# tum-vision/lsd_slam

Hardware: AMD Instinct MI355X
Metric: tracked frames/sec (full track+map loop) at 640x480, frames resident in HBM (8-bit upload excluded: value_pcie_inclusive has it) (higher is better)
Workload: dtype f32

## Files before the change

include/lsd_slam_hip.hpp:

```cpp
#ifndef LSD_SLAM_HIP_HPP
#define LSD_SLAM_HIP_HPP

#include <array>
#include <chrono>
#include <cmath>
#include <cstdint>
#include <cstring>
#include <deque>
#include <exception>
#include <functional>
#include <map>
#include <memory>
#include <mutex>
#include <stdexcept>
#include <string>
#include <tuple>
#include <utility>
#include <vector>

#include "lsdhip.h"
#include "lsd_slam_hip_pose.hpp"

namespace lsd_slam_hip {

// ... 279 lines not shown
    check(lsdhip_tracker_create(ctx_->handle(), &h_), "lsdhip_tracker_create");
  }
  SE3Tracker(const SE3Tracker&) = delete;
  SE3Tracker& operator=(const SE3Tracker&) = delete;
  ~SE3Tracker() { lsdhip_tracker_destroy(h_); }

  SE3 trackFrame(TrackingReference* reference, Frame* frame, const SE3& frameToReference_initialEstimate) {
    pushSettings();
    double init[7];
    frameToReference_initialEstimate.to7(init);
    lsdhip_track_result r;
    hookError_ = nullptr;
    if (!reference || !reference->keyframe || !frame) throw Error(LSDHIP_E_STATE, "SE3Tracker::trackFrame: the tracking reference holds no keyframe");
    check(lsdhip_tracker_track(h_, reference->keyframe->handle(), frame->handle(), init, &r), "lsdhip_tracker_track");
    publish(r);
    if (hookError_) std::rethrow_exception(hookError_);
    return SE3::from7(r.frameToReference);
  }
  std::vector<SE3> trackFrameBatch(const std::vector<TrackingReference*>& references, const std::vector<Frame*>& frames,
                                   const std::vector<SE3>& inits, std::vector<lsdhip_track_result>& results) {
    pushSettings();
    const int n = (int)frames.size();
    std::vector<lsdhip_frame*> kfs((size_t)n), frs((size_t)n);
    std::vector<double> init((size_t)n * 7);
    for (int j = 0; j < n; j++) {
      if (!references[j] || !references[j]->keyframe || !frames[j]) throw Error(LSDHIP_E_STATE, "SE3Tracker::trackFrameBatch: a tracking reference holds no keyframe");
      kfs[j] = references[j]->keyframe->handle();
      frs[j] = frames[j]->handle();
      inits[j].to7(&init[(size_t)j * 7]);
    }
    results.assign((size_t)n, lsdhip_track_result());
    hookError_ = nullptr;
    const int rc = lsdhip_tracker_track_batch(h_, n, kfs.data(), frs.data(), init.data(), results.data());
    if (rc != LSDHIP_OK && rc != LSDHIP_DIVERGED) check(rc, "lsdhip_tracker_track_batch");
    if (hookError_) std::rethrow_exception(hookError_);
    std::vector<SE3> out((size_t)n);
    for (int j = 0; j < n; j++) out[j] = SE3::from7(results[j].frameToReference);
    return out;
  }
  SE3 trackFrameOnPermaref(Frame* reference, Frame* frame, SE3 referenceToFrame) {
    pushSettings();
    double init[7];
    referenceToFrame.to7(init);
    lsdhip_track_result r;
    check(lsdhip_tracker_track_permaref(h_, reference->permaRef_posData.data(), reference->permaRef_colorAndVarData.data(),
                                        reference->permaRefNumPts, frame->handle(), init, &r), "lsdhip_tracker_track_permaref");
    publish(r);
    return SE3::from7(r.frameToReference);
  }
  void setEnqueueHook(std::function<void()> fn) {
    hook_ = std::move(fn);
    check(lsdhip_tracker_set_enqueue_hook(h_, hook_ ? &SE3Tracker::hookTrampoline : nullptr, this), "lsdhip_tracker_set_enqueue_hook");
  }
  float checkPermaRefOverlap(Frame* reference, SE3 referenceToFrame) {
    double init[7];
    referenceToFrame.to7(init);
    float usage = 0;
    check(lsdhip_tracker_check_overlap(h_, reference->permaRef_posData.data(), reference->permaRefNumPts, init, &usage), "lsdhip_tracker_check_overlap");
    pointUsage = usage;
    return usage;
  }

  float pointUsage = 0, lastGoodCount = 0, lastMeanRes = 0, lastBadCount = 0, lastResidual = 0;
  float affineEstimation_a = 1, affineEstimation_b = 0;
  bool diverged = false, trackingWasGood = false;
  int numEvaluations = 0, numWarpUpdates = 0;
  int levelEvaluations[LSDHIP_PYRAMID_LEVELS] = {0, 0, 0, 0, 0};
  int numLaunches = 0;
  void setSpeculation(int trials, int finestLevelWorkgroups = 0) { check(lsdhip_tracker_set_speculation(h_, trials, finestLevelWorkgroups), "lsdhip_tracker_set_speculation"); }
  void setBatchCoarseMinJobs(int minJobs) { check(lsdhip_tracker_set_batch_coarse_min_jobs(h_, minJobs), "lsdhip_tracker_set_batch_coarse_min_jobs"); }
  lsdhip_tracker* handle() const { return h_; }
  const std::shared_ptr<Context>& context() const { return ctx_; }

 private:
  void pushSettings() {
    lsdhip_tracker_settings st;
    st.lambdaSuccessFac = settings.lambdaSuccessFac; st.lambdaFailFac = settings.lambdaFailFac;
    for (int l = 0; l < LSDHIP_PYRAMID_LEVELS; l++) {
      st.lambdaInitial[l] = settings.lambdaInitial[l]; st.stepSizeMin[l] = settings.stepSizeMin[l];
      st.convergenceEps[l] = settings.convergenceEps[l]; st.maxItsPerLvl[l] = settings.maxItsPerLvl[l];
    }
    st.lambdaInitialTestTrack = settings.lambdaInitialTestTrack; st.stepSizeMinTestTrack = settings.stepSizeMinTestTrack;
    st.convergenceEpsTestTrack = settings.convergenceEpsTestTrack; st.maxItsTestTrack = settings.maxItsTestTrack;
    st.huber_d = settings.huber_d; st.var_weight = settings.var_weight;
    check(lsdhip_tracker_set_settings(h_, &st), "lsdhip_tracker_set_settings");
  }
  void publish(const lsdhip_track_result& r) {
    pointUsage = r.pointUsage; lastGoodCount = r.lastGoodCount; lastMeanRes = r.lastMeanRes; lastBadCount = r.lastBadCount;
    lastResidual = r.lastResidual; affineEstimation_a = r.affineEstimation_a; affineEstimation_b = r.affineEstimation_b;
    diverged = r.diverged != 0; trackingWasGood = r.trackingWasGood != 0;
    numEvaluations = r.numEvaluations; numWarpUpdates = r.numWarpUpdates;
    int st[8];
    if (lsdhip_tracker_exec_stats(h_, st) == 0) for (int l = 0; l < LSDHIP_PYRAMID_LEVELS; l++) levelEvaluations[l] = st[3 + l];
    int ls[2];
    if (lsdhip_tracker_launch_stats(h_, ls) == 0) numLaunches = ls[0];
  }
  static void hookTrampoline(void* self) {
    SE3Tracker* t = static_cast<SE3Tracker*>(self);
    try { if (t->hook_) t->hook_(); } catch (...) { t->hookError_ = std::current_exception(); }
  }
  std::function<void()> hook_;
  std::exception_ptr hookError_;
  std::shared_ptr<Context> ctx_;
  lsdhip_tracker* h_ = nullptr;
};

class KeyFrameBank {
 public:
  struct Info { int frameId, numPoints; float meanIdepth; Sim3 camToWorld; };
  KeyFrameBank(std::shared_ptr<Context> ctx, int maxKeyframes) : ctx_(std::move(ctx)) {
    check(lsdhip_kfbank_create(ctx_->handle(), maxKeyframes, &h_), "lsdhip_kfbank_create");
  }
  KeyFrameBank(const KeyFrameBank&) = delete;
  KeyFrameBank& operator=(const KeyFrameBank&) = delete;
  ~KeyFrameBank() { lsdhip_kfbank_destroy(h_); }
  int put(Frame& kf) {
    int slot = -1;
    check(lsdhip_kfbank_put(h_, kf.handle(), &slot), "lsdhip_kfbank_put");
    kf.idxInKeyframes = slot;
    return slot;
  }
  int put(Frame& kf, const Sim3& camToWorld, float meanIdepth = -1.0f) {
    const int slot = put(kf);
    setMeta(slot, camToWorld, meanIdepth);
    return slot;
  }
  void setMeta(int slot, const Sim3& camToWorld, float meanIdepth = -1.0f) {
    const double p[8] = {camToWorld.q[0], camToWorld.q[1], camToWorld.q[2], camToWorld.q[3], camToWorld.t[0], camToWorld.t[1], camToWorld.t[2], camToWorld.s};
    check(lsdhip_kfbank_set_meta(h_, slot, p, meanIdepth), "lsdhip_kfbank_set_meta");
  }
  int size() const { return check(lsdhip_kfbank_size(h_), "lsdhip_kfbank_size"); }
  Info info(int slot) const {
    Info o;
    double p[8];
    check(lsdhip_kfbank_info(h_, slot, &o.frameId, &o.numPoints, &o.meanIdepth, p), "lsdhip_kfbank_info");
    for (int i = 0; i < 4; i++) o.camToWorld.q[i] = p[i];
    for (int i = 0; i < 3; i++) o.camToWorld.t[i] = p[4 + i];
    o.camToWorld.s = p[7];
    return o;
  }
  int download(int slot, std::vector<float>* posData, std::vector<float>* colorAndVarData) const {
    const int n = info(slot).numPoints;
    std::vector<float> pos((size_t)n * 3 + 1), cv((size_t)n * 2 + 1);
    check(lsdhip_kfbank_download(h_, slot, pos.data(), cv.data()), "lsdhip_kfbank_download");
    if (posData) posData->assign(pos.begin(), pos.begin() + (size_t)n * 3);
    if (colorAndVarData) colorAndVarData->assign(cv.begin(), cv.begin() + (size_t)n * 2);
    return n;
  }
  lsdhip_kfbank* handle() const { return h_; }
  const std::shared_ptr<Context>& context() const { return ctx_; }

 private:
  std::shared_ptr<Context> ctx_;
  lsdhip_kfbank* h_ = nullptr;
// ... 164 lines not shown
    return v;
  }
  int debugPlotDepthMap(int debugDisplay = 0) {
    if (!isValid()) return 1;
    debugImageDepth.resize((size_t)ctx_->width() * ctx_->height() * 3);
    check(lsdhip_depth_debug_plot(h_, debugDisplay, debugImageDepth.data()), "lsdhip_depth_debug_plot");
    return 1;
  }
  void debugPlotDepthMapDevice(unsigned char* dev, int debugDisplay) { check(lsdhip_depth_debug_plot_dev(h_, debugDisplay, dev), "lsdhip_depth_debug_plot_dev"); }
  static void debugPlotDepthMapBatch(const std::vector<DepthMap*>& maps, const std::vector<unsigned char*>& devs, int debugDisplay) {
    if (maps.empty()) return;
    if (devs.size() != maps.size()) throw Error(LSDHIP_E_ARG, "DepthMap::debugPlotDepthMapBatch: one device buffer per map");
    std::vector<lsdhip_depthmap*> ms;
    for (DepthMap* m : maps) ms.push_back(m->h_);
    check(lsdhip_depth_debug_plot_batch((int)ms.size(), ms.data(), debugDisplay, devs.data()), "lsdhip_depth_debug_plot_batch");
  }
  std::vector<unsigned char> debugImageDepth;
  void copyPlanesToDevice(float* idepth_dev, float* idepthVar_dev) { check(lsdhip_depth_copy_planes_dev(h_, idepth_dev, idepthVar_dev), "lsdhip_depth_copy_planes_dev"); }

  float msUpdate = 0, msCreate = 0, msFinalize = 0, msObserve = 0, msRegularize = 0, msPropagate = 0, msFillHoles = 0, msSetDepth = 0;
  lsdhip_depthmap* handle() const { return h_; }

 private:
  void timings() {
    float t[8];
    if (lsdhip_depth_timings(h_, t) == 0) { msUpdate = t[0]; msCreate = t[1]; msFinalize = t[2]; msObserve = t[3]; msRegularize = t[4]; msPropagate = t[5]; msFillHoles = t[6]; msSetDepth = t[7]; }
  }
  std::shared_ptr<Context> ctx_;
  lsdhip_depthmap* h_ = nullptr;
};

class SlamLoop {
 public:
  SlamLoop(int w, int h, const Mat3f& K, const unsigned char* firstImage, bool imagesOnDevice, const float* gtDepth0, int kfEvery)
      : tracker(w, h, K), map(w, h, K), w_(w), h_(h), K_(K), onDevice_(imagesOnDevice), kfEvery_(kfEvery) {
    const int its[LSDHIP_PYRAMID_LEVELS] = {5, 20, 50, 100, 0};
    std::memcpy(tracker.settings.maxItsPerLvl, its, sizeof(its));
    keyframe = makeFrame(0, firstImage);
    if (gtDepth0) {
      keyframe->setDepthFromGroundTruth(gtDepth0);
      map.initializeFromGTDepth(keyframe.get());
    } else {
      map.initializeRandomly(keyframe.get());
    }
    trackKF_ = keyframe;
    reference.importFrame(keyframe.get());
    keyframe->clearDepthHasBeenUpdatedFlag();
    tracker.setEnqueueHook([this]() {
      flushDeferredMapping();
      if (!pendingNext_) return;
      prefetched_ = makeFrame(frameId_ + 1, pendingNext_, true);
      prefetchedSrc_ = pendingNext_;
    });
  }
  SlamLoop(const SlamLoop&) = delete;
  SlamLoop& operator=(const SlamLoop&) = delete;
  void setPipelined(bool on) {
    if (frameId_ != 0) throw Error(LSDHIP_E_STATE, "SlamLoop::setPipelined: switch before the first frame");
    Context::get(w_, h_, K_)->setPipeline(on);
    pipelined_ = on;
  }
  bool pipelined() const { return pipelined_; }
  void flushDeferredMapping() {
    if (!deferredMap_) return;
    std::shared_ptr<Frame> frame = std::move(deferredMap_);
    deferredMap_.reset();
    runUpdate(frame);
  }
  static float keyframeScore(float distanceSquared, float usage) {
    return distanceSquared * 4.0f * 4.0f + (1 - usage) * (1 - usage) * 3.0f * 3.0f;
  }
  std::function<void(Frame&, DepthMap&)> onKeyframeFinished;
  std::function<void(Frame&)> onKeyframeFinishedAsync;
  std::function<void(DepthMap&)> onMappingIteration;
  SE3 step(const unsigned char* image) { return step(image, [](double) {}); }
  template <typename F>
  SE3 step(const unsigned char* image, F&& onTrackEnd, const unsigned char* nextImage = nullptr) {
    if (trackingLost) throw Error(LSDHIP_E_STATE, "SlamLoop: tracking lost (no relocaliser here): create a new loop");
    lsdhip_host_mark(0);
    frameId_++;
    std::shared_ptr<Frame> frame;
    if (prefetched_ && prefetchedSrc_ == image) frame = std::move(prefetched_);
    else frame = makeFrame(frameId_, image);
    prefetched_.reset();
    pendingNext_ = nextImage;
    if (!pipelined_ && keyframe->depthHasBeenUpdatedFlag()) {
      reference.importFrame(keyframe.get());
      keyframe->clearDepthHasBeenUpdatedFlag();
    }
    lsdhip_host_mark(1);
    const std::shared_ptr<Frame> trackedOn = trackKF_;
    SE3 est = tracker.trackFrame(&reference, frame.get(), lastFrameToKF_);
    lsdhip_host_mark(8);
    pendingNext_ = nullptr;
    evaluations += tracker.numEvaluations;
    launches += tracker.numLaunches;
    for (int l = 0; l < LSDHIP_PYRAMID_LEVELS; l++) levelEvaluations[l] += tracker.levelEvaluations[l];
    if (tracker.trackingWasGood) numTrackedGood++;
    numTracked++;
    lastTrackEnd = std::chrono::duration<double>(std::chrono::steady_clock::now().time_since_epoch()).count();
    onTrackEnd(lastTrackEnd);
    if (tracker.diverged || (numKeyframesFinished_ > 5  && !tracker.trackingWasGood)) {
      trackingLost = true;
      reference.invalidate();
      if (map.isValid()) {
        if (mappedOnKF_ >= 5 ) {
          map.finalizeKeyFrame();
          numKeyframesFinished_++;
          if (onKeyframeFinished) onKeyframeFinished(*keyframe, map);
          if (onKeyframeFinishedAsync) onKeyframeFinishedAsync(*keyframe);
        }
        map.invalidate();
      }
      throw Error(LSDHIP_DIVERGED, std::string("SlamLoop: tracking lost at frame ") + std::to_string(frameId_) +
                                       (tracker.diverged ? " (diverged)" : " (trackingWasGood false)"));
    }
    if (pipelined_) {
      if (pendingKF_) {
        double p[7];
        if (pendingIsReactivated_) {
          double f2k[8], frameToWorld[8];
          est.to7(f2k); f2k[7] = 1;
          lsd_slam::pose::sim3_mul(worldPose(*trackKF_).data(), f2k, frameToWorld);
          lsd_slam::pose::relative_se3(worldPose(*pendingKF_).data(), frameToWorld, p);
          pendingIsReactivated_ = false;
        } else {
          check(lsdhip_frame_relative_pose(pendingKF_->handle(), frame->handle(), p), "lsdhip_frame_relative_pose");
        }
        lastFrameToKF_ = SE3::from7(p);
        trackKF_ = pendingKF_;
        pendingKF_.reset();
        reference.importFrame(trackKF_.get());
        trackKF_->clearDepthHasBeenUpdatedFlag();
      } else {
        lastFrameToKF_ = est;
        if (trackKF_->depthHasBeenUpdatedFlag()) {
          reference.importFrame(trackKF_.get());
          trackKF_->clearDepthHasBeenUpdatedFlag();
        }
      }
    }
    ++sinceKF_;
    newKeyframe = false;
    flushDeferredMapping();
    if (trackedOn != keyframe) {
      frame->clear_refPixelWasGood();
      numDropped++;
      return est;
    }
    bool createNewKeyFrame = kfEvery_ > 0 && sinceKF_ >= kfEvery_;
    if (kfEvery_ == 0 && mappedOnKF_ > 5 ) {
      const float mi = keyframe->meanIdepth();
      const float d0 = (float)est.t[0] * mi, d1 = (float)est.t[1] * mi, d2 = (float)est.t[2] * mi;
      float minVal = 0.2f * 0.7f;
      if (reactivateKeyframes) {
        const int size = bank_->size();
// ... 122 lines not shown
      map.changeKeyframe(frame.get());
    }
    bankFinishedKeyframe(finished);
    if (onKeyframeFinishedAsync) onKeyframeFinishedAsync(*finished);
    const lsdhip_reposition_result& r = search_->last;
    keyframeChanges.push_back(KeyframeChange{frame->id(), finished->id(), found ? found->id() : frame->id(), found != nullptr,
                                             r.numPotential, r.numChecked, r.numTracked});
    double nextEstimate[7] = {1, 0, 0, 0, 0, 0, 0};
    if (found) {
      numReactivations++;
      keyframe = found;
      keyframe->clearDepthHasBeenUpdatedFlag();
      lsd_slam::pose::relative_se3(worldPose(*keyframe).data(), cw, nextEstimate);
    } else {
      double raw[8];
      check(lsdhip_frame_get_pose(frame->handle(), raw), "lsdhip_frame_get_pose");
      std::array<double, 8> w;
      lsd_slam::pose::sim3_mul(worldPose(*finished).data(), raw, w.data());
      worldPoses_[frame->id()] = w;
      keyframe = frame;
      if (keepKeyframes) keyframeLog.push_back(frame);
    }
    liveQueue_.clear();
    if (pipelined_) {
      pendingKF_ = keyframe;
      pendingIsReactivated_ = found != nullptr;
    } else {
      trackKF_ = keyframe;
      reference.importFrame(keyframe.get());
      keyframe->clearDepthHasBeenUpdatedFlag();
      lastFrameToKF_ = SE3::from7(nextEstimate);
    }
    sinceKF_ = 0;
    newKeyframe = true;
    if (onMappingIteration) onMappingIteration(map);
  }
  std::unique_ptr<KeyFrameBank> bank_;
  std::unique_ptr<TrackableKeyFrameSearch> search_;
  std::vector<std::shared_ptr<Frame>> bankedBySlot_;
  std::map<int, std::array<double, 8>> worldPoses_;
  bool pendingIsReactivated_ = false;
  void runUpdate(const std::shared_ptr<Frame>& frame) {
    liveQueue_.push_back(frame);
    while ((int)liveQueue_.size() > (liveQueueLength > 1 ? liveQueueLength : 1)) liveQueue_.pop_front();
    std::deque<std::shared_ptr<Frame>> q(liveQueue_.begin(), liveQueue_.end());
    lsdhip_host_mark(9);
    map.updateKeyframe(q);
    lsdhip_host_mark(13);
    mappedOnKF_++;
    frame->clear_refPixelWasGood();
    numUpdates++;
    lsdhip_host_mark(14);
    if (onMappingIteration) onMappingIteration(map);
  }
  std::shared_ptr<Frame> deferredMap_;
  std::shared_ptr<Frame> makeFrame(int id, const unsigned char* img, bool mayDefer = false) {
    if (onDevice_) return std::make_shared<Frame>(id, w_, h_, K_, 0.0, Frame::DeviceImage{img});
    if (mayDefer && pipelined_) return std::make_shared<Frame>(id, w_, h_, K_, 0.0, Frame::HostImageAsync{img});
    return std::make_shared<Frame>(id, w_, h_, K_, 0.0, img);
  }
  int w_, h_;
  Mat3f K_;
  bool onDevice_;
  bool pipelined_ = false;
  int kfEvery_, sinceKF_ = 0, frameId_ = 0;
  int mappedOnKF_ = 0;
  int numKeyframesFinished_ = 0;
  SE3 lastFrameToKF_;
  std::shared_ptr<Frame> trackKF_;
  std::shared_ptr<Frame> pendingKF_;
  std::shared_ptr<Frame> prefetched_;
  const unsigned char* prefetchedSrc_ = nullptr;
  const unsigned char* pendingNext_ = nullptr;
  std::deque<std::shared_ptr<Frame>> liveQueue_;
};

class SlamLoopBatch {
 public:
  struct Sequence {
    Sequence(int w, int h, const Mat3f& K) : map(w, h, K) {}
    DepthMap map;
    TrackingReference reference;
    std::shared_ptr<Frame> keyframe;
    std::shared_ptr<Frame> trackKF;
    std::shared_ptr<Frame> pendingKF;
    SE3 lastFrameToKF;
    int sinceKF = 0, mappedOnKF = 0, numKeyframesFinished = 0;
    long numTracked = 0, numTrackedGood = 0, numUpdates = 0, evaluations = 0, numDropped = 0;
    bool trackingLost = false, newKeyframe = false;
    lsdhip_track_result last = lsdhip_track_result();
    std::vector<std::shared_ptr<Frame>> keyframeLog;
    std::shared_ptr<Frame> replacedFirst;
  };
  SlamLoopBatch(int w, int h, const Mat3f& K, int S, const unsigned char* const* firstImages, bool imagesOnDevice,
                const float* const* gtDepth0, int kfEvery)
      : tracker(w, h, K), w_(w), h_(h), K_(K), onDevice_(imagesOnDevice), kfEvery_(kfEvery) {
    if (S <= 0 || kfEvery <= 0) throw Error(LSDHIP_E_ARG, "SlamLoopBatch: S > 0 sequences, a fixed keyframe interval > 0");
    const int its[LSDHIP_PYRAMID_LEVELS] = {5, 20, 50, 100, 0};
    std::memcpy(tracker.settings.maxItsPerLvl, its, sizeof(its));
    tracker.setBatchCoarseMinJobs(coarseMinJobs(false));
    std::vector<int> ids((size_t)S);
    for (int s = 0; s < S; s++) ids[s] = idOf(s, 0);
    std::vector<std::shared_ptr<Frame>> first = Frame::createBatch(w, h, K, ids, firstImages, imagesOnDevice);
    for (int s = 0; s < S; s++) {
      seqs_.emplace_back(new Sequence(w, h, K));
      Sequence& q = *seqs_.back();
// ... 284 lines not shown
```

include/lsdhip.h:

```cpp
#ifndef LSDHIP_H
#define LSDHIP_H

#include <stddef.h>
#include <stdint.h>

#ifdef __cplusplus
extern "C" {
#endif

#define LSDHIP_PYRAMID_LEVELS 5

#define LSDHIP_OK 0
#define LSDHIP_DIVERGED 1
#define LSDHIP_E_ARG (-1)
#define LSDHIP_E_HIP (-2)
#define LSDHIP_E_STATE (-3)
#define LSDHIP_E_CAPACITY (-4)
#define LSDHIP_CLOUD_TABLE_FULL 2
#define LSDHIP_CLOUD_GUARD_POINTS 64

typedef struct lsdhip_ctx lsdhip_ctx;
typedef struct lsdhip_frame lsdhip_frame;
typedef struct lsdhip_tracker lsdhip_tracker;
typedef struct lsdhip_depthmap lsdhip_depthmap;
// ... 60 lines not shown
int lsdhip_frame_clear_wasgood(lsdhip_frame* f);
int lsdhip_frame_set_pose(lsdhip_frame* f, const double thisToParent_sim3[8], lsdhip_frame* trackingParent,
                          float initialTrackedResidual);
int lsdhip_frame_get_pose(lsdhip_frame* f, double thisToParent_sim3[8]);
int lsdhip_frame_relative_pose(lsdhip_frame* reference, lsdhip_frame* frame, double frameToReference[7]);
int lsdhip_frame_publish_depth(lsdhip_frame* f);
int lsdhip_frame_stats(lsdhip_frame* f, float out[8]);
int lsdhip_frame_set_counters(lsdhip_frame* f, int numFramesTrackedOnThis, int numMappedOnThis,
                              int numMappedOnThisTotal, int depthHasBeenUpdatedFlag);
int lsdhip_frame_depth_updated(lsdhip_frame* f);
int lsdhip_frame_clear_depth_updated(lsdhip_frame* f);
int lsdhip_ref_pointcloud(lsdhip_frame* kf, int level, float* pos3_host, float* colorAndVar2_host,
                          float* grad2_host, int* idx_host);

typedef struct lsdhip_track_result {
  double frameToReference[7];
  float pointUsage, lastGoodCount, lastBadCount, lastMeanRes, lastResidual;
  float affineEstimation_a, affineEstimation_b;
  int diverged, trackingWasGood;
  int numEvaluations, numWarpUpdates;
} lsdhip_track_result;

typedef struct lsdhip_residual_record {
  int warped_size;
  float goodCount, badCount, pointUsage, meanRes, retval;
  float affine_a_lastIt, affine_b_lastIt;
  float weightedError;
  float A[36], b[6], lsError;
  double num_constraints;
} lsdhip_residual_record;

int lsdhip_tracker_create(lsdhip_ctx* ctx, lsdhip_tracker** out);
void lsdhip_tracker_destroy(lsdhip_tracker* t);
int lsdhip_tracker_set_max_its(lsdhip_tracker* t, const int maxItsPerLvl[LSDHIP_PYRAMID_LEVELS]);
typedef struct lsdhip_tracker_settings {
  float lambdaSuccessFac, lambdaFailFac;
  float lambdaInitial[LSDHIP_PYRAMID_LEVELS], stepSizeMin[LSDHIP_PYRAMID_LEVELS], convergenceEps[LSDHIP_PYRAMID_LEVELS];
  int maxItsPerLvl[LSDHIP_PYRAMID_LEVELS];
  float lambdaInitialTestTrack, stepSizeMinTestTrack, convergenceEpsTestTrack, maxItsTestTrack;
  float huber_d, var_weight;
} lsdhip_tracker_settings;
int lsdhip_tracker_get_settings(const lsdhip_tracker* t, lsdhip_tracker_settings* out);
int lsdhip_tracker_set_settings(lsdhip_tracker* t, const lsdhip_tracker_settings* in);
int lsdhip_tracker_exec_stats(const lsdhip_tracker* t, int out[8]);
int lsdhip_tracker_set_speculation(lsdhip_tracker* t, int trials, int finestLevelWorkgroups);
int lsdhip_tracker_set_batch_coarse_min_jobs(lsdhip_tracker* t, int minJobs);
int lsdhip_tracker_launch_stats(const lsdhip_tracker* t, int out[2]);
int lsdhip_tracker_step_stats(const lsdhip_tracker* t, int out[4]);
int lsdhip_tracker_summary_stats(const lsdhip_tracker* t, long long out[6]);
int lsdhip_tracker_eval_throughput(lsdhip_tracker* t, int n, lsdhip_frame** keyframes, lsdhip_frame** frames, const float* refToFrame,
                                   int level, int repeats, double* ms_per_launch, double* bytes_per_launch);
typedef void (*lsdhip_enqueue_hook)(void* user);
int lsdhip_tracker_set_enqueue_hook(lsdhip_tracker* t, lsdhip_enqueue_hook fn, void* user);
int lsdhip_tracker_track(lsdhip_tracker* t, lsdhip_frame* keyframe, lsdhip_frame* frame,
                         const double frameToReference_initialEstimate[7], lsdhip_track_result* out);
int lsdhip_tracker_track_batch(lsdhip_tracker* t, int n, lsdhip_frame** keyframes, lsdhip_frame** frames,
                               const double* frameToReference_initialEstimates, lsdhip_track_result* results);
int lsdhip_tracker_evaluate(lsdhip_tracker* t, lsdhip_frame* keyframe, lsdhip_frame* frame,
                            const float referenceToFrame[7], int level, float affine_a, float affine_b,
                            lsdhip_residual_record* out);
int lsdhip_tracker_evaluate_batch(lsdhip_tracker* t, int n, lsdhip_frame** keyframes, lsdhip_frame** frames,
                                  const float* referenceToFrame, const float* affine, int level, lsdhip_residual_record* out,
                                  int* form);
int lsdhip_tracker_track_permaref(lsdhip_tracker* t, const float* pos3_host, const float* colorAndVar2_host, int n,
                                  lsdhip_frame* frame, const double referenceToFrame[7], lsdhip_track_result* out);
int lsdhip_tracker_track_permaref_batch(lsdhip_tracker* t, int n, const float* pos3_host, const float* colorAndVar2_host,
                                        const int* counts, lsdhip_frame** frames, const double* referenceToFrame,
                                        lsdhip_track_result* results);
int lsdhip_tracker_check_overlap(lsdhip_tracker* t, const float* pos3_host, int n, const double referenceToFrame[7],
                                 float* usage_out);

typedef struct lsdhip_kfbank lsdhip_kfbank;
int lsdhip_kfbank_create(lsdhip_ctx* ctx, int max_keyframes, lsdhip_kfbank** out);
void lsdhip_kfbank_destroy(lsdhip_kfbank* bank);
int lsdhip_kfbank_put(lsdhip_kfbank* bank, lsdhip_frame* keyframe, int* slot_out);
int lsdhip_kfbank_set_meta(lsdhip_kfbank* bank, int slot, const double camToWorld_sim3[8], float meanIdepth);
int lsdhip_kfbank_size(lsdhip_kfbank* bank);
int lsdhip_kfbank_info(lsdhip_kfbank* bank, int slot, int* frameId, int* numPoints, float* meanIdepth, double camToWorld_sim3[8]);
int lsdhip_kfbank_download(lsdhip_kfbank* bank, int slot, float* pos3_host, float* colorAndVar2_host);
int lsdhip_tracker_check_overlap_bank(lsdhip_tracker* t, lsdhip_kfbank* bank, int n, const int* slots, const double* refToFrame,
                                      float* usage_out);
int lsdhip_tracker_track_permaref_bank(lsdhip_tracker* t, lsdhip_kfbank* bank, int n, const int* slots, lsdhip_frame** frames,
                                       const double* refToFrame, lsdhip_track_result* results);
typedef struct lsdhip_reposition_result {
  int slot, frameId;
  int numPotential, numChecked, numTracked;
  int overlapLaunches, trackingBatches;
  float bestScore, bestDist, bestUsage, bestPoseDiscrepancy;
  double refToFrame[7], refToFrame_tracked[7];
} lsdhip_reposition_result;
#define LSDHIP_REPO_FAR 0
#define LSDHIP_REPO_ANGLE 1
#define LSDHIP_REPO_PARENT 2
#define LSDHIP_REPO_INIT_PHASE 3
#define LSDHIP_REPO_EMPTY 4
#define LSDHIP_REPO_SCORE 5
#define LSDHIP_REPO_REJECTED 6
#define LSDHIP_REPO_TAKEN 7
typedef struct lsdhip_reposition_record {
  int slot, frameId, stage;
  float dist2, angle;
  float usage, score;
  float usageTracked;
  float newScore, goodVal, poseDiscrepancy;
  int trackingWasGood, diverged;
  double refToFrame[7], refToFrame_tracked[7];
} lsdhip_reposition_record;
int lsdhip_tracker_find_reposition_candidate(lsdhip_tracker* t, lsdhip_kfbank* bank, lsdhip_frame* frame, const double frameCamToWorld_sim3[8],
                                             int trackingParentId, float maxScore, lsdhip_reposition_result* result);
int lsdhip_tracker_reposition_records(lsdhip_tracker* t, int max, lsdhip_reposition_record* records, int* n);
int lsdhip_tracker_set_relocalization_th(lsdhip_tracker* t, float relocalizationTH);

typedef struct lsdhip_sim3tracker lsdhip_sim3tracker;
typedef struct lsdhip_sim3_result {
  double frameToReference[8];
  float lastResidual, lastDepthResidual, lastPhotometricResidual;
  float pointUsage;
  float affineEstimation_a, affineEstimation_b;
  int diverged;
  int numEvaluations;
  float lastSim3Hessian[49];
} lsdhip_sim3_result;
typedef struct lsdhip_sim3_eval_record {
  int warped_size;
  float pointUsage, affine_a_lastIt, affine_b_lastIt;
  float sumResD, sumResP;
  int numTermsD, numTermsP;
  float meanD, meanP, mean;
  float A[49], b[7];
  double num_constraints;
} lsdhip_sim3_eval_record;
int lsdhip_sim3tracker_create(lsdhip_ctx* ctx, lsdhip_sim3tracker** out);
void lsdhip_sim3tracker_destroy(lsdhip_sim3tracker* t);
int lsdhip_sim3tracker_set_max_its(lsdhip_sim3tracker* t, const int maxItsPerLvl[5]);
int lsdhip_sim3tracker_track(lsdhip_sim3tracker* t, lsdhip_frame* keyframe, lsdhip_frame* frame, const double init_frameToReference[8],
                             int startLevel, int finalLevel, lsdhip_sim3_result* out);
int lsdhip_sim3tracker_track_batch(lsdhip_sim3tracker* t, int n, lsdhip_frame** keyframes, lsdhip_frame** frames,
                                   const double* init_frameToReference, int startLevel, int finalLevel, lsdhip_sim3_result* results);
int lsdhip_host_se3f_step(const float increment[6], const float referenceToFrame[7], float out[7]);
int lsdhip_host_ldlt6(const float A[36], const float b[6], float x[6]);
int lsdhip_host_sim3_step(const double increment[7], const double referenceToFrame[8], double out[8]);
int lsdhip_host_ldlt7(const float A[49], const float b[7], float x[7]);
int lsdhip_devtest_se3f_lm_step(lsdhip_ctx* ctx, int n, const float* A, const float* b, const float* damp, const float* T, float* inc, float* Tn);
int lsdhip_devtest_sim3_lm_step(lsdhip_ctx* ctx, int n, const float* A, const float* b, const double* nconstraints, const float* lambda,
                                const double* T, float* inc, double* Tn);
int lsdhip_sim3tracker_evaluate(lsdhip_sim3tracker* t, lsdhip_frame* keyframe, lsdhip_frame* frame, const double referenceToFrame[8],
                                int level, float aff_a, float aff_b, lsdhip_sim3_eval_record* out);

int lsdhip_depth_create(lsdhip_ctx* ctx, lsdhip_depthmap** out);
void lsdhip_depth_destroy(lsdhip_depthmap* dm);
int lsdhip_depth_is_valid(lsdhip_depthmap* dm);
int lsdhip_depth_invalidate(lsdhip_depthmap* dm);
int lsdhip_depth_reset(lsdhip_depthmap* dm);
int lsdhip_depth_init_gt(lsdhip_depthmap* dm, lsdhip_frame* kf);
int lsdhip_depth_init_random(lsdhip_depthmap* dm, lsdhip_frame* kf);
int lsdhip_depth_set_from_existing(lsdhip_depthmap* dm, lsdhip_frame* kf);
int lsdhip_depth_update(lsdhip_depthmap* dm, lsdhip_frame** refs, int n);
int lsdhip_depth_update_batch(int n, lsdhip_depthmap** maps, lsdhip_frame** refs);
int lsdhip_depth_create_keyframe(lsdhip_depthmap* dm, lsdhip_frame* new_keyframe, float* rescale_out);
int lsdhip_depth_finalize(lsdhip_depthmap* dm);
int lsdhip_depth_change_keyframe_batch(int n, lsdhip_depthmap** maps, lsdhip_frame** new_keyframes, float* rescale_out);
int lsdhip_depth_reactivate_keyframe_batch(int n, lsdhip_depthmap** maps, lsdhip_frame** old_keyframes);
int lsdhip_ctx_batch_form(lsdhip_ctx* ctx, int which, int out[8], int* queueCounts, int maxCounts);
int lsdhip_depth_download(lsdhip_depthmap* dm, lsdhip_hypothesis* out_host);
int lsdhip_depth_upload(lsdhip_depthmap* dm, lsdhip_frame* kf, const lsdhip_hypothesis* in_host, int reactivated);
int lsdhip_depth_debug_plot(lsdhip_depthmap* dm, int debugDisplay, uint8_t* out_host);
int lsdhip_depth_debug_plot_dev(lsdhip_depthmap* dm, int debugDisplay, uint8_t* out_dev);
int lsdhip_depth_debug_plot_batch(int n, lsdhip_depthmap** maps, int debugDisplay, uint8_t* const* out_dev);
int lsdhip_depth_stage(lsdhip_depthmap* dm, int stage, lsdhip_frame** refs, int n);
int lsdhip_depth_stage_rows(lsdhip_depthmap* dm, int stage, int tile_row0, int n_tile_rows, int last);
int lsdhip_depth_stage_rows_batch(lsdhip_ctx* c, int n, lsdhip_depthmap** maps, const int* tile_row0, const int* n_tile_rows);
int lsdhip_depth_copy_planes_dev(lsdhip_depthmap* dm, float* idepth_dev, float* idepthVar_dev);
int lsdhip_ctx_copy_dev(lsdhip_ctx* ctx, void* dst_dev, const void* src_dev, size_t bytes);
int lsdhip_ctx_alloc_dev(lsdhip_ctx* ctx, size_t bytes, void** out_dev);
int lsdhip_ctx_ipc_export(lsdhip_ctx* ctx, void* dev, unsigned char handle64[64]);
int lsdhip_ctx_ipc_open(lsdhip_ctx* ctx, const unsigned char handle64[64], void** out_dev);
int lsdhip_ctx_ipc_close(lsdhip_ctx* ctx, void* dev);
int lsdhip_ctx_flag_set(lsdhip_ctx* ctx, int* flag_dev, int value);
int lsdhip_ctx_flag_wait(lsdhip_ctx* ctx, const int* flag_dev, int value, int* fail_dev);
int lsdhip_ctx_memset_dev(lsdhip_ctx* ctx, void* dev, int byte, size_t bytes);
int lsdhip_ctx_read_dev(lsdhip_ctx* ctx, void* host, const void* dev, size_t bytes);
int lsdhip_ctx_aux_begin(lsdhip_ctx* ctx);
int lsdhip_ctx_aux_end(lsdhip_ctx* ctx);
int lsdhip_ctx_aux_join(lsdhip_ctx* ctx);
void* lsdhip_ctx_aux_stream(lsdhip_ctx* ctx);
void lsdhip_host_mark(int id);
int lsdhip_ctx_free_dev(lsdhip_ctx* ctx, void* dev);
int lsdhip_depth_copy_rows_dev(lsdhip_depthmap* dm, int row0, int nrows, void* packed_dev, int to_map);
typedef struct lsdhip_row_copy {
  lsdhip_depthmap* src_map; int src_row0; void* src_packed;
  lsdhip_depthmap* dst_map; int dst_row0; void* dst_packed;
  int nrows;
} lsdhip_row_copy;
// ... 28 lines not shown
```

include/lsdhip_driver.h:

```cpp
#ifndef LSDHIP_DRIVER_H
#define LSDHIP_DRIVER_H
#include <stdint.h>
#ifdef __cplusplus
extern "C" {
#endif
typedef struct lsdloop lsdloop;
typedef struct lsdloop_stats {
  double seconds_track;
  double seconds_map;
  double seconds_keyframe;
  long long frames;
  long long updates;
  long long keyframes;
  long long evaluations;
  long long tracked_good;
  long long level_evaluations[5];
  long long track_launches;
  long long dropped;
} lsdloop_stats;
int lsdloop_create(int device, int w, int h, const float K4[4], const uint8_t* first_image, int images_on_device,
                   const float* gt_depth0_host, int kf_every, lsdloop** out);
void lsdloop_destroy(lsdloop* l);
int lsdloop_run(lsdloop* l, const uint8_t* const* images, int n, int stop_at_keyframe, double* frameToKeyframe_out);
int lsdloop_get_stats(lsdloop* l, lsdloop_stats* out);
int lsdloop_reset_stats(lsdloop* l);
int lsdloop_copy_keyframe_planes(lsdloop* l, float* idepth_dev, float* idepthVar_dev);
int lsdloop_set_keyframe_ring(lsdloop* l, float* ring_dev, int slots);
long long lsdloop_keyframes_exported(lsdloop* l);
int lsdloop_keep_keyframes(lsdloop* l, int on);
int lsdloop_keyframe_log(lsdloop* l, double* scales_out, long long* points_out, int max);
int lsdloop_set_pipeline(lsdloop* l, int on);
int lsdloop_enable_reactivation(lsdloop* l, int max_keyframes);
int lsdloop_keyframe_changes(lsdloop* l, int* out, int max);
int lsdloop_reactivation_counts(lsdloop* l, long long out2[2]);
int lsdloop_download_map(lsdloop* l, lsdhip_hypothesis* out);
int lsdloop_set_live_queue(lsdloop* l, int frames);
int lsdloop_set_speculation(lsdloop* l, int trials, int finest_level_workgroups);
int lsdloop_observe_time(lsdloop* l, double* ms_out, long long* calls_out);
int lsdloop_observe_work(lsdloop* l, double out3[3]);
int lsdloop_comm_unique_id(unsigned char out128[128]);
int lsdloop_comm_init(lsdloop* l, const unsigned char id128[128], int rank, int world);
int lsdloop_comm_destroy(lsdloop* l);
int lsdloop_gather_keyframes(lsdloop* l, int count, int root, float* recv_dev, long long stride_floats);
int lsdloop_gather_counts(lsdloop* l, int* counts_out, int cap);
int lsdloop_ipc_init(lsdloop* l, int rank, int world, int root, unsigned char handle64_out[64]);
int lsdloop_ipc_connect(lsdloop* l, const unsigned char root_handle64[64]);
int lsdloop_ipc_result(lsdloop* l, int* counts_out, float** data_out);
void* lsdloop_ctx(lsdloop* l);
typedef struct lsdloopbatch lsdloopbatch;
int lsdloopbatch_create(int device, int w, int h, const float K4[4], int S, const uint8_t* const* first_images, int images_on_device,
                        const float* const* gt_depth0_host, int kf_every, lsdloopbatch** out);
void lsdloopbatch_destroy(lsdloopbatch* l);
int lsdloopbatch_run(lsdloopbatch* l, const uint8_t* const* images, int n, double* frameToKeyframe_out);
int lsdloopbatch_get_stats(lsdloopbatch* l, long long* out6_per_sequence);
void* lsdloopbatch_ctx(lsdloopbatch* l);
int lsdloopbatch_set_keyframe_phases(lsdloopbatch* l, const int* phase);
int lsdloopbatch_set_pipeline(lsdloopbatch* l, int on);
int lsdloopbatch_set_coarse_min_jobs(lsdloopbatch* l, int min_jobs);
long long lsdloopbatch_dropped(lsdloopbatch* l, int sequence);
int lsdloopbatch_keep_keyframes(lsdloopbatch* l, int on);
int lsdloopbatch_keyframe_log(lsdloopbatch* l, int sequence, double* scales_out, long long* points_out, int max);
int lsdloopbatch_last_result(lsdloopbatch* l, int sequence, lsdhip_track_result* out);
int lsdloopbatch_download_map(lsdloopbatch* l, int sequence, lsdhip_hypothesis* out);
int lsdloopbatch_set_cloud_sinks(lsdloopbatch* l, long long capacity_points, int max_keyframes);
void* lsdloopbatch_cloud(lsdloopbatch* l, int sequence);
int lsdloopbatch_cloud_pose(lsdloopbatch* l, int sequence, int frame_id, float out7[7]);
void* lsdloopbatch_keyframe_handle(lsdloopbatch* l, int sequence, int k);
const char* lsdloop_last_error(void);
typedef struct lsdband lsdband;
int lsdband_create(int device, int w, int H, int world, int first_band, int n_local, lsdband** out);
int lsdband_plan(int H, int world, int* window_rows_out, int* layout4, int* segments4, int cap);
void lsdband_destroy(lsdband* b);
int lsdband_window_rows(const lsdband* b);
int lsdband_layout(const lsdband* b, int band, int out4[4]);
int lsdband_load(lsdband* b, int local, const void* hyp_window, const float* maxgrad_window);
int lsdband_get(lsdband* b, int local, void* hyp_window_out);
int lsdband_comm_init(lsdband* b, const void* unique_id128, int nprocs, int proc, const int* proc_of_band);
int lsdband_run(lsdband* b, int passes);
int lsdband_synchronize(lsdband* b);
long long lsdband_halo_bytes_per_pass(const lsdband* b);
int lsdband_ipc_init(lsdband* b, int nprocs, int proc, const int* proc_of_band, unsigned char handle64_out[64]);
int lsdband_ipc_connect(lsdband* b, const unsigned char* handles);
int lsdband_ipc_failed(lsdband* b);
int lsdband_tile_runs(int H, int world, int band, int* runs3, int cap);
int lsdband_set_packed_exchange(lsdband* b, int on);
int lsdband_set_overlap(lsdband* b, int on);

#ifdef __cplusplus
}
#endif
// ... 2 lines not shown
```

lsd_slam_amd/capi.py:

```python
import ctypes as C
import os

import numpy as np

_HERE = os.path.dirname(os.path.abspath(__file__))
LIB_PATH = os.environ.get("LSDHIP_LIB") or os.path.join(_HERE, "liblsdhip.so")
_lib = None

HYP_DTYPE = np.dtype(
    [("isValid", np.uint8), ("_pad", np.uint8, 3), ("blacklisted", np.int32), ("nextStereoFrameMinID", np.float32),
     ("validity_counter", np.int32), ("idepth", np.float32), ("idepth_var", np.float32),
     ("idepth_smoothed", np.float32), ("idepth_var_smoothed", np.float32)])
assert HYP_DTYPE.itemsize == 32


class BuildDefaults(C.Structure):
    _fields_ = [(k, C.c_int) for k in ("ctx_async", "ctx_pipeline", "spec_trials_small", "spec_small_pixels", "spec_trials_mid", "spec_mid_pixels",
                                         "spec_workgroups", "spec_workgroups_above_pixels", "spec_trials_max", "batch_throughput_min_jobs",
                                         "batch_strip_workgroups", "batch_coarse_min_jobs", "batch_coarse_max_pixels",
                                         "batch_coarse_max_points")]


class Params(C.Structure):
    _fields_ = [("minUseGrad", C.c_float), ("cameraPixelNoise2", C.c_float), ("depthSmoothingFactor", C.c_float),
# ... 74 lines not shown
        "lsdhip_frame_create_batch": (i, [vp, i, vp, pvp, i, pvp]),
        "lsdhip_ctx_reserve_frames": (i, [vp, i]),
        "lsdhip_frame_relative_pose": (i, [vp, vp, vp]),
        "lsdhip_frame_publish_depth": (i, [vp]),
        "lsdhip_last_error": (C.c_char_p, []),
        "lsdhip_ctx_intrinsics": (i, [vp, i, vp]),
        "lsdhip_frame_create": (i, [vp, i, vp, pvp]),
        "lsdhip_frame_create_from_device": (i, [vp, i, vp, pvp]),
        "lsdhip_frame_destroy": (None, [vp]),
        "lsdhip_frame_id": (i, [vp]),
        "lsdhip_frame_download": (i, [vp, i, i, vp]),
        "lsdhip_frame_set_depth_gt": (i, [vp, vp, f]),
        "lsdhip_frame_set_depth_planes": (i, [vp, vp, vp]),
        "lsdhip_frame_set_maxgrad": (i, [vp, vp]),
        "lsdhip_frame_get_wasgood": (i, [vp, vp]),
        "lsdhip_frame_set_wasgood": (i, [vp, vp]),
        "lsdhip_frame_clear_wasgood": (i, [vp]),
        "lsdhip_frame_set_pose": (i, [vp, vp, vp, f]),
        "lsdhip_frame_get_pose": (i, [vp, vp]),
        "lsdhip_frame_stats": (i, [vp, vp]),
        "lsdhip_frame_set_counters": (i, [vp, i, i, i, i]),
        "lsdhip_frame_depth_updated": (i, [vp]),
        "lsdhip_frame_clear_depth_updated": (i, [vp]),
        "lsdhip_ref_pointcloud": (i, [vp, i, vp, vp, vp, vp]),
        "lsdhip_tracker_create": (i, [vp, pvp]),
        "lsdhip_tracker_destroy": (None, [vp]),
        "lsdhip_tracker_set_max_its": (i, [vp, vp]),
        "lsdhip_tracker_get_settings": (i, [vp, C.POINTER(TrackerSettings)]),
        "lsdhip_tracker_set_settings": (i, [vp, C.POINTER(TrackerSettings)]),
        "lsdhip_depth_copy_rows_batch": (i, [vp, i, vp]),
        "lsdhip_ctx_alloc_dev": (i, [vp, C.c_size_t, vp]),
        "lsdhip_ctx_ipc_export": (i, [vp, vp, vp]),
        "lsdhip_ctx_ipc_open": (i, [vp, vp, vp]),
        "lsdhip_ctx_ipc_close": (i, [vp, vp]),
        "lsdhip_ctx_flag_set": (i, [vp, vp, i]),
        "lsdhip_ctx_flag_wait": (i, [vp, vp, i, vp]),
        "lsdhip_ctx_memset_dev": (i, [vp, vp, i, C.c_size_t]),
        "lsdhip_ctx_read_dev": (i, [vp, vp, vp, C.c_size_t]),
        "lsdhip_ctx_free_dev": (i, [vp, vp]),
        "lsdhip_host_mark": (None, [i]),
        "lsdhip_ctx_aux_begin": (i, [vp]),
        "lsdhip_ctx_aux_end": (i, [vp]),
        "lsdhip_ctx_aux_join": (i, [vp]),
        "lsdhip_ctx_aux_stream": (vp, [vp]),
        "lsdhip_depth_stage_rows": (i, [vp, i, i, i, i]),
        "lsdhip_depth_stage_rows_batch": (i, [vp, i, pvp, C.POINTER(C.c_int), C.POINTER(C.c_int)]),
        "lsdhip_tracker_exec_stats": (i, [vp, vp]),
        "lsdhip_tracker_set_speculation": (i, [vp, i, i]),
        "lsdhip_tracker_set_batch_coarse_min_jobs": (i, [vp, i]),
        "lsdhip_tracker_launch_stats": (i, [vp, vp]),
        "lsdhip_tracker_summary_stats": (i, [vp, vp]),
        "lsdhip_tracker_step_stats": (i, [vp, vp]),
        "lsdhip_tracker_set_enqueue_hook": (i, [vp, vp, vp]),
        "lsdhip_tracker_track": (i, [vp, vp, vp, vp, C.POINTER(TrackResult)]),
        "lsdhip_tracker_track_batch": (i, [vp, i, pvp, pvp, vp, C.POINTER(TrackResult)]),
        "lsdhip_tracker_eval_throughput": (i, [vp, i, pvp, pvp, vp, i, i, C.POINTER(C.c_double), C.POINTER(C.c_double)]),
        "lsdhip_tracker_evaluate": (i, [vp, vp, vp, vp, i, f, f, C.POINTER(ResidualRecord)]),
        "lsdhip_tracker_evaluate_batch": (i, [vp, i, pvp, pvp, vp, vp, i, C.POINTER(ResidualRecord), vp]),
        "lsdhip_tracker_track_permaref": (i, [vp, vp, vp, i, vp, vp, C.POINTER(TrackResult)]),
        "lsdhip_tracker_track_permaref_batch": (i, [vp, i, vp, vp, vp, pvp, vp, C.POINTER(TrackResult)]),
        "lsdhip_tracker_check_overlap": (i, [vp, vp, i, vp, C.POINTER(C.c_float)]),
        "lsdhip_kfbank_create": (i, [vp, i, pvp]),
        "lsdhip_kfbank_destroy": (None, [vp]),
        "lsdhip_kfbank_put": (i, [vp, vp, C.POINTER(C.c_int)]),
        "lsdhip_kfbank_set_meta": (i, [vp, i, vp, f]),
        "lsdhip_kfbank_size": (i, [vp]),
        "lsdhip_kfbank_info": (i, [vp, i, C.POINTER(C.c_int), C.POINTER(C.c_int), C.POINTER(C.c_float), vp]),
        "lsdhip_kfbank_download": (i, [vp, i, vp, vp]),
        "lsdhip_tracker_check_overlap_bank": (i, [vp, vp, i, vp, vp, vp]),
        "lsdhip_tracker_track_permaref_bank": (i, [vp, vp, i, vp, pvp, vp, C.POINTER(TrackResult)]),
        "lsdhip_tracker_find_reposition_candidate": (i, [vp, vp, vp, vp, i, f, C.POINTER(RepositionResult)]),
        "lsdhip_tracker_reposition_records": (i, [vp, i, C.POINTER(RepositionRecord), C.POINTER(C.c_int)]),
        "lsdhip_tracker_set_relocalization_th": (i, [vp, f]),
        "lsdhip_sim3tracker_create": (i, [vp, pvp]),
        "lsdhip_sim3tracker_destroy": (None, [vp]),
        "lsdhip_sim3tracker_set_max_its": (i, [vp, vp]),
        "lsdhip_sim3tracker_track": (i, [vp, vp, vp, vp, i, i, C.POINTER(Sim3Result)]),
        "lsdhip_sim3tracker_track_batch": (i, [vp, i, pvp, pvp, vp, i, i, C.POINTER(Sim3Result)]),
        "lsdhip_host_se3f_step": (i, [vp, vp, vp]),
        "lsdhip_host_ldlt6": (i, [vp, vp, vp]),
        "lsdhip_host_sim3_step": (i, [vp, vp, vp]),
        "lsdhip_host_ldlt7": (i, [vp, vp, vp]),
        "lsdhip_devtest_se3f_lm_step": (i, [vp, i, vp, vp, vp, vp, vp, vp]),
        "lsdhip_devtest_sim3_lm_step": (i, [vp, i, vp, vp, vp, vp, vp, vp, vp]),
        "lsdhip_sim3tracker_evaluate": (i, [vp, vp, vp, vp, i, f, f, C.POINTER(Sim3EvalRecord)]),
        "lsdhip_depth_create": (i, [vp, pvp]),
        "lsdhip_depth_destroy": (None, [vp]),
        "lsdhip_depth_is_valid": (i, [vp]),
        "lsdhip_depth_invalidate": (i, [vp]),
        "lsdhip_depth_reset": (i, [vp]),
        "lsdhip_depth_init_gt": (i, [vp, vp]),
        "lsdhip_depth_init_random": (i, [vp, vp]),
        "lsdhip_depth_set_from_existing": (i, [vp, vp]),
        "lsdhip_depth_update": (i, [vp, pvp, i]),
        "lsdhip_depth_observe_work": (i, [vp, vp]),
        "lsdhip_depth_update_batch": (i, [i, pvp, pvp]),
        "lsdhip_depth_create_keyframe": (i, [vp, vp, C.POINTER(C.c_float)]),
        "lsdhip_depth_change_keyframe_batch": (i, [i, pvp, pvp, C.POINTER(C.c_float)]),
        "lsdhip_depth_reactivate_keyframe_batch": (i, [i, pvp, pvp]),
        "lsdhip_ctx_batch_form": (i, [vp, i, vp, vp, i]),
        "lsdhip_depth_finalize": (i, [vp]),
        "lsdhip_depth_download": (i, [vp, vp]),
        "lsdhip_depth_upload": (i, [vp, vp, vp, i]),
        "lsdhip_depth_debug_plot": (i, [vp, i, vp]),
        "lsdhip_depth_debug_plot_dev": (i, [vp, i, vp]),
        "lsdhip_depth_debug_plot_batch": (i, [i, pvp, i, pvp]),
# ... 52 lines not shown
```

lsd_slam_amd/csrc/host_math.cpp:

```cpp
#include <cstdarg>
#include "lsdhip_internal.hpp"

static thread_local std::string g_last_error;
void lsd_set_error(const char* fmt, ...) {
  char buf[1024];
  va_list ap;
  va_start(ap, fmt);
  vsnprintf(buf, sizeof(buf), fmt, ap);
  va_end(ap);
  g_last_error = buf;
}
extern "C" const char* lsdhip_last_error(void) { return g_last_error.c_str(); }


extern "C" int lsdhip_host_se3f_step(const float increment[6], const float referenceToFrame[7], float out[7]) {
  if (!increment || !referenceToFrame || !out) return LSDHIP_E_ARG;
  lsdm::SE3fH T;
  T.q = {referenceToFrame[0], referenceToFrame[1], referenceToFrame[2], referenceToFrame[3]};
  T.t[0] = referenceToFrame[4]; T.t[1] = referenceToFrame[5]; T.t[2] = referenceToFrame[6];
  const lsdm::SE3fH r = lsdm::se3f_mul(lsdm::se3f_exp(increment), T);
  out[0] = r.q.w; out[1] = r.q.x; out[2] = r.q.y; out[3] = r.q.z; out[4] = r.t[0]; out[5] = r.t[1]; out[6] = r.t[2];
  return LSDHIP_OK;
}
extern "C" int lsdhip_host_ldlt6(const float A[36], const float b[6], float x[6]) {
  if (!A || !b || !x) return LSDHIP_E_ARG;
  lsdm::ldlt6_solve(A, b, x);
  return LSDHIP_OK;
}
```

lsd_slam_amd/csrc/lsdhip_internal.hpp:

```cpp
#pragma once
#include <hip/hip_runtime.h>
#include <atomic>
#include <chrono>
#include <cmath>
#include <cstddef>
#include <cstdint>
#include <cstdio>
#include <cstring>
#include <mutex>
#include <string>
#include <vector>
#include "../../include/lsdhip.h"

#define LSD_LEVELS LSDHIP_PYRAMID_LEVELS
#define LSD_TRACK_MIN_LEVEL 1
#define LSD_TRACK_MAX_LEVEL 5
#define LSD_QUICK_KF_CHECK_LVL 4

void lsd_set_error(const char* fmt, ...);
#define HIPCHK(expr)                                                                       \
  do {                                                                                     \
    hipError_t e_ = (expr);                                                                \
    if (e_ != hipSuccess) {                                                                \
      lsd_set_error("%s failed: %s (%s:%d)", #expr, hipGetErrorString(e_), __FILE__, __LINE__); \
// ... 45 lines not shown
  int evalBatch;
};

struct TrackJob {
  TrackLevel lv[LSD_LEVELS];
  uint8_t* wasGood;
  float cameraPixelNoise2, var_weight, huber_half;
  float lambdaSuccessFac, lambdaFailFac;
  int useAffine;
  int lastLevel;
  int topLevel;
  lsdm::SE3fH T0;
  float aff_a0, aff_b0;
  int evalOnly;
  int trackFrameSemantics;
};
struct TrackSpec {
  int specC;
  int specGrid;
  int trials[LSD_LEVELS];
  uint8_t* wasGoodSide;
  unsigned maskStride;
  int seq;
  int copyMask;
  unsigned long long dbgCum;
  unsigned long long* dbgCounters;
  int last;
#ifdef LSD_PHASE_TRACE
  int traceWg;
#endif
#ifdef LSD_DEVTOOLS
  int* dbgLog;
#endif
};

struct TrackState {
  lsdm::SE3fH T;
  lsdm::SE3fH Tn;
  float R[9], t[3];
  float aff_a, aff_b, aff_a_lastIt, aff_b_lastIt;
  float lastErr, LM_lambda, last_residual;
  int level, iteration, incTry, phase;
  int pending;
  float A[36], b[6];
  float inc[6];
  float bytes;
  int done, diverged;
  int numEvaluations, numWarpUpdates;
  float pointUsage, goodCount, badCount, meanRes;
  int levelEvals[LSD_LEVELS];
  int ncand;
  int lastCand;
  int numLaunches;
};

struct TrackSummary {
  int done;
  int diverged, level, numEvaluations, numWarpUpdates, pad_[3];
  float q[4], t[3];
  float lastResidual, pointUsage, goodCount, badCount, meanRes, aff_a, aff_b, aff_a_lastIt, aff_b_lastIt;
  float sums[RS_NUM];
  double bytes;
  int levelEvals[LSD_LEVELS];
  int numLaunches;
  int lastCand;
  int seq;
  int exhausted;
  unsigned check;
};
#define LSD_SUMMARY_CHECK_WORDS (offsetof(TrackSummary, seq) / 4)
__host__ __device__ static inline unsigned lsd_summary_term(unsigned i, unsigned bits) { return bits * (2u * i + 1u); }

struct DeferredSlot { double sum, count, flag, pad; };
#define LSD_NUM_SLOTS 256
#define LSD_DEFAULT_ASYNC 0
#define LSD_DEFAULT_PIPELINE 0
#ifndef LSD_OBS_SPLIT_MIN_MAPS
#define LSD_OBS_SPLIT_MIN_MAPS 4
#endif
#define LSD_OBS_WALK_WAVES 4096
struct lsdhip_frame;

#define LSD_CTX_LOCK(c) std::lock_guard<std::recursive_mutex> lsd_ctx_lock_((c)->mtx)
struct lsdhip_ctx {
  std::recursive_mutex mtx;
  int device = 0;
  bool async = LSD_DEFAULT_ASYNC != 0;
  DeferredSlot* h_slots = nullptr;
  lsdhip_frame* slot_stats_owner[LSD_NUM_SLOTS] = {};
  lsdhip_frame* slot_rescale_owner[LSD_NUM_SLOTS] = {};
  int slot_next = 0;
  long long enqEpoch = 0, doneEpoch = 0;
  long long slot_epoch[LSD_NUM_SLOTS] = {};
  int w = 0, h = 0;
  bool refBlocksWanted = false;
  int wl[LSD_LEVELS], hl[LSD_LEVELS];
  LevelIntr intr[LSD_LEVELS];
  float K0[9], K0inv[9];
  lsdhip_params params;
  hipStream_t stream = nullptr;
#define LSD_EVR 64
  bool pipeline = LSD_DEFAULT_PIPELINE != 0;
  hipStream_t mstream = nullptr;
  hipEvent_t mEv[LSD_EVR] = {};
  long long mSeq = 0;
  long long mDoneSeq = 0;
// ... 100 lines not shown
};

struct lsdhip_tracker {
  lsdhip_ctx* ctx = nullptr;
  float lambdaSuccessFac = 0.5f, lambdaFailFac = 2.0f;
  float lambdaInitial[LSD_LEVELS], stepSizeMin[LSD_LEVELS], convergenceEps[LSD_LEVELS];
  int maxItsPerLvl[LSD_LEVELS];
  float lambdaInitialTestTrack = 0, stepSizeMinTestTrack = 1e-3, convergenceEpsTestTrack = 0.98, maxItsTestTrack = 5;
  float huber_d = 3, var_weight = 1.0;
  float pointUsage = 0, lastGoodCount = 0, lastMeanRes = 0, lastBadCount = 0, lastResidual = 0;
  float affineEstimation_a = 1, affineEstimation_b = 0, affineEstimation_a_lastIt = 1, affineEstimation_b_lastIt = 0;
  bool diverged = false, trackingWasGood = false;
  int numEvaluations = 0, numWarpUpdates = 0;
  void (*enqueueHook)(void*) = nullptr;
  void* enqueueHookUser = nullptr;
  bool spinWait = true;
  bool hostLM = false;
  float* d_partials = nullptr;
  int max_blocks = 0;
  TrackState* d_state = nullptr;
  int levelEvaluations[LSD_LEVELS] = {};
  int block = 256;
  int grid_cap = 304;
  bool evalBatch = true;
  LaunchHistory recent;
  int specC = 6;
  int soloMinJobs = -1;
  bool specAuto = true;
  int specCaps[LSD_LEVELS] = {0, 0, 0, 0, 0};
  int specLevel[LSD_LEVELS] = {0, 0, 0, 0, 0};
  int specCap = LSD_SPEC_CAP_WORKGROUPS;
  uint8_t* d_maskSide = nullptr;
  int maskSet = 0;
  long long maskMergeSeq[2] = {0, 0};
  size_t maskStride = 0;
  int numLaunches = 0;
  long long sumPolled = 0, sumLate = 0, sumLateMaxNs = 0, sumLateWords = 0;
  int sumLateFirstWord = -1, sumLateLastWord = -1;
  unsigned long long dbgCum = 0;
  std::vector<unsigned> dumpL0;
  unsigned long long* d_dbg = nullptr;
#ifdef LSD_DEVTOOLS
  int* d_log = nullptr;
  std::vector<int> lastLog;
#endif
  const lsdhip_frame* jobKf = nullptr;
  unsigned jobKfVersion = 0;
  int jobTag = 0, launchOrdinal = 0;
  int budgetExtra = 2;
  int budgetFixed = 0;
  long long dbgJobs = 0, dbgEnqueued = 0, dbgMisses = 0, dbgWaitNs = 0, dbgLaunchNs = 0;
  TrackSummary* h_summary = nullptr;
  TrackSummary* d_summary = nullptr;
  unsigned long long* d_trace = nullptr;
  int batch_capacity = 0;
  TrackJob* d_bjobs = nullptr;
  TrackJob* h_bjobs = nullptr;
  TrackState* d_bstate = nullptr;
  float* d_bscratch = nullptr;
  LaunchHistory batchRecent;
  int batchTag = 1;
  TrackSummary* h_bsummary = nullptr;
  float* d_pts = nullptr;
  int pts_capacity = 0;
  float relocalizationTH = 0.7f;
  float* h_overlapSums = nullptr;
  int overlapSumsCapacity = 0;
  std::vector<lsdhip_reposition_record> repoRecords;
};

struct lsdhip_kfbank {
  lsdhip_ctx* ctx = nullptr;
  int maxSlots = 0, capacity = 0;
  size_t slotFloats = 0;
  float* d_base = nullptr;
  int* d_count = nullptr;
  struct Slot { int frameId; int numPoints; float meanIdepth; double camToWorld[8]; };
  std::vector<Slot> slots;
  float* pos(int slot) const { return d_base + (size_t)slot * slotFloats; }
  float* colvar(int slot) const { return pos(slot) + (size_t)capacity * 3; }
};

#ifdef __HIP_DEVICE_COMPILE__
#define LSD_G __attribute__((address_space(1)))
#else
#define LSD_G
#endif
template <typename T> __host__ __device__ inline LSD_G T* lsd_g(T* p) { return (LSD_G T*)p; }
struct HypPlanes {
  LSD_G uint8_t* valid;
  LSD_G int32_t* blacklisted;
  LSD_G float* nextID;
  LSD_G int32_t* validity;
  LSD_G float* idepth;
  LSD_G float* var;
  LSD_G float* idepth_s;
  LSD_G float* var_s;
};

struct StereoRef {
  LSD_G const float* image;
  LSD_G const uint8_t* wasGood;
  int parentIsKF;
  int id;
  float initialTrackedResidual;
  float K_otherToThis_R[9];
// ... 152 lines not shown
```

lsd_slam_amd/csrc/pose_math.hpp:

```cpp
#pragma once
#include <hip/hip_runtime.h>
#include <cmath>

#define LSDM_HD __host__ __device__ inline

namespace lsdm {
struct Quatd { double w, x, y, z; };
struct Quatf { float w, x, y, z; };
struct SE3dH { Quatd q; double t[3]; };
struct SE3fH { Quatf q; float t[3]; };
struct Sim3dH { Quatd q; double t[3]; double s; };

template <typename Q> LSDM_HD Q q_conj(const Q& a) { Q r = {a.w, -a.x, -a.y, -a.z}; return r; }
template <typename Q> LSDM_HD Q q_mul(const Q& a, const Q& b) {
  Q r;
  r.w = a.w * b.w - a.x * b.x - a.y * b.y - a.z * b.z;
  r.x = a.w * b.x + a.x * b.w + a.y * b.z - a.z * b.y;
  r.y = a.w * b.y + a.y * b.w + a.z * b.x - a.x * b.z;
  r.z = a.w * b.z + a.z * b.w + a.x * b.y - a.y * b.x;
  return r;
}
LSDM_HD void q_normalize(Quatf& q) {
  float n = sqrtf(q.x * q.x + q.y * q.y + q.z * q.z + q.w * q.w);
  q.w /= n; q.x /= n; q.y /= n; q.z /= n;
// ... 1 lines not shown
LSDM_HD void q_normalize(Quatd& q) {
  double n = sqrt(q.x * q.x + q.y * q.y + q.z * q.z + q.w * q.w);
  q.w /= n; q.x /= n; q.y /= n; q.z /= n;
}
template <typename Q, typename T> LSDM_HD void q_rotate(const Q& q, const T v[3], T out[3]) {
  T ux = q.y * v[2] - q.z * v[1], uy = q.z * v[0] - q.x * v[2], uz = q.x * v[1] - q.y * v[0];
  ux += ux; uy += uy; uz += uz;
  T cx = q.y * uz - q.z * uy, cy = q.z * ux - q.x * uz, cz = q.x * uy - q.y * ux;
  out[0] = v[0] + q.w * ux + cx;
  out[1] = v[1] + q.w * uy + cy;
  out[2] = v[2] + q.w * uz + cz;
}
template <typename Q, typename T> LSDM_HD void q_to_rot(const Q& q, T R[9]) {
  T tx = T(2) * q.x, ty = T(2) * q.y, tz = T(2) * q.z;
  T twx = tx * q.w, twy = ty * q.w, twz = tz * q.w;
  T txx = tx * q.x, txy = ty * q.x, txz = tz * q.x;
  T tyy = ty * q.y, tyz = tz * q.y, tzz = tz * q.z;
  R[0] = T(1) - (tyy + tzz); R[1] = txy - twz;          R[2] = txz + twy;
  R[3] = txy + twz;          R[4] = T(1) - (txx + tzz); R[5] = tyz - twx;
  R[6] = txz - twy;          R[7] = tyz + twx;          R[8] = T(1) - (txx + tyy);
}
LSDM_HD void quatf_to_rot(const Quatf& q, float R[9]) { q_to_rot<Quatf, float>(q, R); }
LSDM_HD void quatd_to_rot(const Quatd& q, double R[9]) { q_to_rot<Quatd, double>(q, R); }

LSDM_HD SE3dH se3d_from7(const double p[7]) { SE3dH T; T.q = {p[0], p[1], p[2], p[3]}; T.t[0] = p[4]; T.t[1] = p[5]; T.t[2] = p[6]; return T; }
LSDM_HD void se3d_to7(const SE3dH& T, double p[7]) { p[0] = T.q.w; p[1] = T.q.x; p[2] = T.q.y; p[3] = T.q.z; p[4] = T.t[0]; p[5] = T.t[1]; p[6] = T.t[2]; }
LSDM_HD SE3dH se3d_inverse(const SE3dH& T) {
  SE3dH r;
  r.q = q_conj(T.q);
  double nt[3] = {T.t[0] * -1.0, T.t[1] * -1.0, T.t[2] * -1.0};
  q_rotate<Quatd, double>(r.q, nt, r.t);
  return r;
}
LSDM_HD SE3fH se3f_from_d(const SE3dH& T) {
  SE3fH r;
  r.q = {(float)T.q.w, (float)T.q.x, (float)T.q.y, (float)T.q.z};
  q_normalize(r.q);
  for (int i = 0; i < 3; i++) r.t[i] = (float)T.t[i];
  return r;
}
LSDM_HD SE3dH se3d_from_f(const SE3fH& T) {
  SE3dH r;
  r.q = {(double)T.q.w, (double)T.q.x, (double)T.q.y, (double)T.q.z};
  q_normalize(r.q);
  for (int i = 0; i < 3; i++) r.t[i] = (double)T.t[i];
  return r;
}
LSDM_HD SE3fH se3f_inverse(const SE3fH& T) {
  SE3fH r;
  r.q = q_conj(T.q);
  float nt[3] = {T.t[0] * -1.0f, T.t[1] * -1.0f, T.t[2] * -1.0f};
  q_rotate<Quatf, float>(r.q, nt, r.t);
  return r;
}
LSDM_HD SE3fH se3f_mul(const SE3fH& a, const SE3fH& b) {
  SE3fH r = a;
  float rt[3];
  q_rotate<Quatf, float>(a.q, b.t, rt);
  for (int i = 0; i < 3; i++) r.t[i] = a.t[i] + rt[i];
  r.q = q_mul(a.q, b.q);
  q_normalize(r.q);
  return r;
}
LSDM_HD SE3fH se3f_exp(const float a[6]) {
  const float eps = static_cast<float>(1e-5);
  float ox = a[3], oy = a[4], oz = a[5];
  float theta_sq = ox * ox + (oy * oy + oz * oz);
  float theta = sqrtf(theta_sq);
  float half_theta = 0.5f * theta;
  float imag, real;
  if (theta < eps) {
    float theta_po4 = theta_sq * theta_sq;
    imag = 0.5f - static_cast<float>(1.0 / 48.0) * theta_sq + static_cast<float>(1.0 / 3840.0) * theta_po4;
    real = 1.0f - 0.5f * theta_sq + static_cast<float>(1.0 / 384.0) * theta_po4;
  } else {
    float s = sinf(half_theta);
    imag = s / theta;
    real = cosf(half_theta);
  }
  SE3fH r;
  r.q = {real, imag * ox, imag * oy, imag * oz};
  q_normalize(r.q);
  float Om[9] = {0, -oz, oy, oz, 0, -ox, -oy, ox, 0};
  float Om2[9];
  for (int i = 0; i < 3; i++)
    for (int j = 0; j < 3; j++) {
      float acc = Om[i * 3 + 0] * Om[0 * 3 + j];
      acc += Om[i * 3 + 1] * Om[1 * 3 + j];
      acc += Om[i * 3 + 2] * Om[2 * 3 + j];
      Om2[i * 3 + j] = acc;
    }
  float V[9];
  if (theta < eps) {
    q_to_rot<Quatf, float>(r.q, V);
  } else {
    float tsq = theta * theta;
    float ca = (1.0f - cosf(theta)) / tsq;
    float cb = (theta - sinf(theta)) / (tsq * theta);
    for (int i = 0; i < 9; i++) V[i] = (((i % 4) == 0 ? 1.0f : 0.0f) + ca * Om[i]) + cb * Om2[i];
  }
  for (int i = 0; i < 3; i++) {
    float acc = V[i * 3 + 0] * a[0];
    acc += V[i * 3 + 1] * a[1];
    acc += V[i * 3 + 2] * a[2];
    r.t[i] = acc;
  }
// ... 61 lines not shown
```

lsd_slam_amd/csrc/tracker.hip:

```cpp
#include <atomic>
#include <chrono>
#include "track_device.hpp"
#include "reposition_plan.hpp"

#ifdef LSD_PHASE_TRACE
#define PHASE_MARK(k) do { if (trOn_ && threadIdx.x == 0) tr_[k] = clock64(); } while (0)
#define LSD_TRACE_WORDS 32
#define TRACE_PARAMS , const bool trOn_, unsigned long long* const tr_
#define TRACE_ARGS , trOn_, tr_
#define TRACE_PUT(rec, who, k, v) do { if (trOn_ && threadIdx.x == (who)) (rec)[k] = (unsigned long long)(v); } while (0)
#define TRACE_LM_REC (trOn_ ? tr_ : nullptr)
__device__ __forceinline__ unsigned long long* trace_open(unsigned long long* trace, const bool mine, unsigned long long** s_trp) {
  if (!mine) return trace;
  const unsigned long long n = trace[0];
  trace[0] = n + 1;
  unsigned long long* tr_ = trace + 1 + (n % 4096) * LSD_TRACE_WORDS;
  for (int k = 0; k < LSD_TRACE_WORDS; k++) tr_[k] = 0;
  tr_[8] = wall_clock64();
  tr_[24] = (unsigned long long)gridDim.x; tr_[25] = (unsigned long long)gridDim.y;
  *s_trp = tr_;
  return tr_;
}
#else
#define PHASE_MARK(k) do { } while (0)
#define TRACE_PARAMS
#define TRACE_ARGS
#define TRACE_PUT(rec, who, k, v) do { } while (0)
#define TRACE_LM_REC nullptr
#endif

#ifdef LSD_DEVTOOLS
#define LAUNCH_LOG(exitCode, pendingIn, ncandIn, pcUsed) do { \
    if (!BATCH && MODE == TS_FUSED && blockIdx.x == 0 && threadIdx.x == 0 && spec.dbgLog && spec.seq != 0) { \
      int* lg_ = spec.dbgLog + ((spec.seq & 0xFFF) * 16); \
      lg_[0] = spec.seq; lg_[1] = (exitCode); lg_[2] = parity | (first << 1) | (spec.last << 2); lg_[3] = lvlIn_; lg_[4] = (pendingIn); lg_[5] = (ncandIn); \
      lg_[6] = (pcUsed); lg_[7] = S.level; lg_[8] = S.numEvaluations; lg_[9] = S.numLaunches; lg_[10] = S.done; lg_[11] = S.phase; lg_[12] = S.incTry; \
      lg_[13] = S.ncand; lg_[14] = S.pending; lg_[15] = numLaunchesIn_; } } while (0)
#else
#define LAUNCH_LOG(exitCode, pendingIn, ncandIn, pcUsed) do { } while (0)
#endif

enum { TS_FUSED = 0, TS_LM = 1, TS_EVAL = 2 };
__device__ __forceinline__ void track_state_begin(TrackState& S, const TrackJob& job, const int tid) {
  if (tid == 0) {
    S.T = job.T0;
    set_eval_pose(S, job.T0);
    S.aff_a = job.aff_a0; S.aff_b = job.aff_b0; S.aff_a_lastIt = job.aff_a0; S.aff_b_lastIt = job.aff_b0;
    S.lastErr = 0; S.LM_lambda = 0; S.last_residual = 0;
    S.level = job.topLevel; S.iteration = 0; S.incTry = 0; S.phase = 0; S.pending = 0;
    S.done = 0; S.diverged = 0; S.numEvaluations = 0; S.numWarpUpdates = 0;
    S.pointUsage = 0; S.goodCount = 0; S.badCount = 0; S.meanRes = 0;
    S.bytes = 0;
    for (int l = 0; l < LSD_LEVELS; l++) S.levelEvals[l] = 0;
    S.ncand = 1; S.lastCand = 0; S.numLaunches = 0;
  }
  if (tid < 36) S.A[tid] = 0;
  if (tid < 6) { S.b[tid] = 0; S.inc[tid] = 0; }
}

struct StepAddr {
  const float *sums_in, *topval_in;
  float *sums_out, *topval_out;
  const int4* topkey_in; int4* topkey_out;
  const TrialRecord* recs_in;
  TrialRecord* recs_out;
  int max_rows, cmax;
};
template <bool BATCH, int MODE>
__device__ __forceinline__ StepAddr step_addr(const TrackScratch& sc, const int parity) {
  const size_t rows = (size_t)sc.max_rows, cm = (size_t)sc.cmax, job0 = BATCH ? (size_t)blockIdx.y * 2 * cm : 0;
  const size_t in = job0 + (size_t)parity * cm, out = job0 + (size_t)(MODE == TS_EVAL ? parity : 1 - parity) * cm;
  constexpr size_t TAIL = TAIL_ROWS * TAIL_STRIDE;
  return {sc.sums + in * RS_COLS * rows, sc.topval + in * rows * TAIL, sc.sums + out * RS_COLS * rows, sc.topval + out * rows * TAIL,
          sc.topkey + in * rows, sc.topkey + out * rows, sc.recs + in, sc.recs + out, sc.max_rows, sc.cmax};
}

struct StepRole { int cand, bx; bool leader, leaves; };
template <bool BATCH, int MODE>
__device__ __forceinline__ void step_role(StepRole& r, const TrackJob& job, const TrackSpec& spec, const TrackState& S) {
  const int lvlPending = S.level;
  if (MODE == TS_FUSED) {
    const int nbl = job.lv[lvlPending].nblocks;
    const int tr = trials_at(spec, lvlPending);
    r.cand = (int)blockIdx.x / nbl; r.bx = (int)blockIdx.x - r.cand * nbl;
    const bool needTrial = S.pending ? r.cand < tr : r.cand == 0;
    const bool needNext = S.pending && lvlPending > job.lastLevel && (int)blockIdx.x < job.lv[lvlPending - 1].nblocks;
    r.leaves = !r.leader && !needTrial && !needNext;
  }
  if (BATCH && MODE == TS_LM) {
    r.cand = (int)blockIdx.x; r.bx = 0;
    r.leaves = !r.leader && !(S.pending && r.cand < trials_at(spec, lvlPending));
  }
  if (BATCH && MODE == TS_EVAL) {
    const int nbl = job.lv[lvlPending].nblocks;
    r.cand = (int)blockIdx.x / nbl; r.bx = (int)blockIdx.x - r.cand * nbl;
  }
}

constexpr int STRIP_CHMAX = 8;
__device__ __forceinline__ void strip_request(const TrackLevel& L, const int tile_, const int wave, const int lane, int& cntv, unsigned (&ow)[STRIP_CHMAX]) {
  const int px = L.w * L.h;
  const int base_ = tile_ * L.tilePx;
  const int b0_ = base_ >> 8;
  const int mblk_ = (min(base_ + L.tilePx, px) - base_ + 255) >> 8;
  const gbyte* offs = (const gbyte*)L.kf_refBlk;
  const __attribute__((address_space(1))) int* cnts = (const __attribute__((address_space(1))) int*)(offs + ((size_t)((px + 255) >> 8) << 8));
  cntv = lane < mblk_ ? cnts[b0_ + lane] : 0;
#pragma unroll
  for (int c = 0; c < STRIP_CHMAX; c++) {
    const int blk = c * 4 + wave;
    ow[c] = blk < mblk_ ? *(const __attribute__((address_space(1))) unsigned*)(offs + ((size_t)(b0_ + blk) << 8) + (lane << 2)) : 0u;
// ... 396 lines not shown
#pragma unroll
    for (int k = 0; k < CPP; k++)
      if (hp * CPP + k < RS_END) s_red[k * (BLOCK + 1) + tid] = acc[hp * CPP + k];
    __syncthreads();
    if (MODE == TS_FUSED && hp == 0 && tid == 0) { S.pending = 1; S.numLaunches = S.numLaunches + 1; }
    if (stripRows && hp == 0 && candLane && c.key >= 0) {
      float px, py;
      ref_point_at(a, c.x, c.y, c.id, px, py, cPz);
      eval_warp(a, px, py, cPz, cq);
      eval_fetch(a, cq, cq.in_image, ct);
    }
    {
      const int slice = tid / CPP, k = tid - slice * CPP;
      if (slice < RSLICE) s_sum[slice][k] = slice_sum<BLOCK + 1, RRUN>(s_red, k, slice);
    }
    __syncthreads();
    if (stripRows && hp == 0 && candLane) {
      float* row = topval_out + (size_t)(tile * TAIL_ROWS + (tid - (BLOCK - 64))) * TAIL_STRIDE;
      if (c.key >= 0) {
        PointOut o;
        eval_finish(a, cq, ct, cPz, c.img, c.var, o);
        tail_row(o, row);
      }
      ((int*)row)[TAIL_KEY] = c.key;
    }
    if (tid < CPP && hp * CPP + tid < RS_END) {
      float s = s_sum[0][tid];
#pragma unroll
      for (int sl = 1; sl < RSLICE; sl++) s += s_sum[sl][tid];
      sums_out[(size_t)tile * RS_COLS + (hp * CPP + tid)] = s;
    }
  }
  if (!stripRows) block_top3(key0, key1, key2, s_wtop, s_top);
  if (tid == 0) topkey_out[tile] = make_int4(s_top[0], s_top[1], s_top[2], -1);
  if (L.singlePass && key0 >= 0) {
    const int r = key0 == s_top[0] ? 0 : (key0 == s_top[1] ? 1 : (key0 == s_top[2] ? 2 : -1));
    if (r >= 0) tail_row_from_sums(acc, topval_out + (size_t)(tile * TAIL_ROWS + r) * TAIL_STRIDE);
  }
}

#ifdef LSD_ORDER_CHECK
__device__ __forceinline__ void order_check_totals(const TrackSpec& spec, const float s, const int pc, const int tid) {
  unsigned hv = tid < RS_END ? __float_as_uint(s) * (2654435761u * (unsigned)(tid + 1)) : 0u;
  hv += (unsigned)pc * 97u;
  for (int off = 32; off > 0; off >>= 1) hv += __shfl_xor(hv, off);
  if (tid == 0) {
    const unsigned long long slot = 8 + 2 * ((spec.dbgCum / 400ull) % 8192ull);
    __hip_atomic_fetch_min(&spec.dbgCounters[slot], (unsigned long long)hv, __ATOMIC_RELAXED, __HIP_MEMORY_SCOPE_AGENT);
    __hip_atomic_fetch_max(&spec.dbgCounters[slot + 1], (unsigned long long)hv, __ATOMIC_RELAXED, __HIP_MEMORY_SCOPE_AGENT);
  }
}
#endif

__device__ __forceinline__ void warm_job_arguments() {
  typedef const unsigned __attribute__((address_space(4))) cuint;
  cuint* ka = (cuint*)__builtin_amdgcn_kernarg_segment_ptr();
  unsigned warm = 0;
#pragma unroll
  for (int i = 0; i < (int)(sizeof(TrackJob) / 4); i += 32) warm ^= ka[i];
  asm volatile("" ::"s"(warm));
}

template <int BLOCK, bool BATCH, int MODE>
__device__ __forceinline__ void track_step_impl(const TrackJob& jobv, const TrackJob* __restrict__ jobs, TrackState* __restrict__ st2,
                                                TrackScratch sc, TrackSummary* __restrict__ out, int parity, int first, const TrackSpec& spec) {
  const TrackJob& job = BATCH ? jobs[blockIdx.y] : jobv;
  if (!BATCH) warm_job_arguments();
  if (BATCH) { st2 += 2 * (size_t)blockIdx.y; out += blockIdx.y; }
  const StepAddr A = step_addr<BATCH, MODE>(sc, parity);
  constexpr int WAVES = BLOCK / 64, SUMW = WAVES - 1;
  constexpr int NSLICE = (SUMW * 64) / RS_END, CPP = RED_CPP, RSLICE_ = BLOCK / CPP;
  __shared__ TrackState S;
  __shared__ LmShared sh;
  __shared__ LmPar s_par;
  __shared__ float s_sum[(NSLICE > RSLICE_ ? NSLICE : RSLICE_)][64];
  __shared__ __attribute__((aligned(16))) float s_red[CPP * (BLOCK + 1) + 8];
  __shared__ int s_wtop[WAVES][3];
  __shared__ int s_top[3];
  const int tid = threadIdx.x, wave = tid >> 6, lane = tid & 63;
  StepRole role = {0, (int)blockIdx.x, blockIdx.x == 0, false};
  const bool leader = role.leader;
  TrackState* next = st2 + (1 - parity);
  constexpr int TRIALS_MAX = BATCH ? (MODE == TS_EVAL ? 1 : LSD_BATCH_SPEC_MAX) : LSD_SPEC_MAX;
  constexpr bool SPEC_LM = MODE != TS_EVAL;
  static_assert(FinishTables<TRIALS_MAX>::WORDS <= CPP * (BLOCK + 1) + 8, "the finishing phase's tables must fit the reduction buffer");
  const FinishTables<TRIALS_MAX> ft(s_red);
  __shared__ TrialRecord s_rec[TRIALS_MAX];
#ifdef LSD_PHASE_TRACE
  __shared__ unsigned long long* s_trp;
  const bool trOn_ = sc.trace != nullptr && (int)blockIdx.x == (BATCH ? spec.traceWg : 0) && (!BATCH || blockIdx.y == 0);
  unsigned long long* const tr_ = trace_open(sc.trace, trOn_ && tid == 0, &s_trp);
#endif
  PHASE_MARK(0);
  if (!BATCH && MODE == TS_FUSED && !first && !leader && st2[parity].done) return;
  if (!BATCH && MODE == TS_FUSED && leader && tid == 0 && spec.seq != 0) out->seq = spec.seq;
  if (first) {
    track_state_begin(S, job, tid);
  } else {
    copy_words<sizeof(TrackState) / 4>(&S, st2 + parity, tid, BLOCK);
    if (SPEC_LM && A.cmax > 1 && tid < (int)(sizeof(s_rec) / 4)) ((float*)s_rec)[tid] = ((const float*)A.recs_in)[tid < (int)(sizeof(TrialRecord) / 4) * A.cmax ? tid : 0];
  }
  __syncthreads();
  PHASE_MARK(1);
#ifdef LSD_DEVTOOLS
  const int lvlIn_ = S.level, numLaunchesIn_ = S.numLaunches, pendingIn_ = S.pending, ncandIn_ = S.ncand;
#endif
  if (S.done) {
    LAUNCH_LOG(1, pendingIn_, ncandIn_, -1);
    if (MODE != TS_EVAL && leader) { copy_words<sizeof(TrackState) / 4>(next, &S, tid, BLOCK); }
    return;
  }
  const int lvlPending = S.level;
  const int doneWord = (MODE == TS_FUSED && spec.seq != 0) ? (BATCH ? spec.seq : (spec.seq >> 12)) : 1;
  step_role<BATCH, MODE>(role, job, spec, S);
  if (role.leaves) return;
  int cand = role.cand, bx = role.bx;

  int cntv = 0;
  unsigned ow[STRIP_CHMAX];
  bool havePre = false;
  if (BATCH && MODE == TS_FUSED && S.pending && job.lv[lvlPending].tilePx > 0) {
    havePre = cand < trials_at(spec, lvlPending);
    if (havePre) strip_request(job.lv[lvlPending], xcd_tile(bx, job.lv[lvlPending].nblocks), wave, lane, cntv, ow);
  }

  if (MODE != TS_EVAL && S.pending) {
    const int ncandPending = S.ncand < 1 ? 1 : (S.ncand > TRIALS_MAX ? TRIALS_MAX : S.ncand);
    const int level = S.level;
    const int nb = job.lv[level].nblocks;
    if (tid == SUMW * 64 - 1) stage_lm_par(job, level, s_par, trials_at(spec, level));
    if (wave < SUMW) {
      column_sums<TRIALS_MAX>(A, nb, ncandPending, tid, ft.sum);
      TRACE_PUT(tr_, 0, 17, clock64());
    }
    gather_tails<BATCH, WAVES>(job, S, level, nb, ncandPending, A, s_rec, ft.sub, ft.nsub, wave, lane);
    TRACE_PUT(s_trp, SUMW * 64, 18, clock64());
    __syncthreads();
    PHASE_MARK(2);
    if (wave == 0) {
      const int pc = pick_trial(S, s_par, level, ncandPending, ft.sum, ft.sub, ft.nsub, s_rec, tid);
      const float s = finish_totals(ft.sum, ft.sub, ft.nsub, pc, tid);
      if (tid < RS_NUM) sh.tot[tid] = s;
#ifdef LSD_ORDER_CHECK
      if (!BATCH && spec.dbgCounters) order_check_totals(spec, s, pc, tid);
#endif
      PHASE_MARK(3);
      TRACE_PUT(tr_, 0, 19, ncandPending); TRACE_PUT(tr_, 0, 7, pc);
      lm_wave<SPEC_LM>(s_par, S, s, sh, tid, leader ? out : nullptr, TRACE_LM_REC, pc, cand, doneWord);
    }
    __syncthreads();
    PHASE_MARK(4);
    if (S.done) {
      if (!BATCH && MODE == TS_FUSED && S.lastCand > 0 && spec.copyMask != 0 && job.lv[level].writeMask && cand == 0 && bx < nb)
        copy_side_mask<BLOCK>(job, S, spec, level, bx, nb, tid);
      if (leader) copy_words<sizeof(TrackState) / 4>(next, &S, tid, BLOCK);
      LAUNCH_LOG(2, pendingIn_, ncandIn_, S.lastCand);
      return;
    }
    if (cand > 0 && bx == 0 && S.phase == 1 && cand < S.ncand && tid < TRIAL_RECORD_WORDS) ((float*)&A.recs_out[cand])[tid] = trial_record_word(S, tid);
  }

  if (MODE == TS_LM) {
    __syncthreads();
    if (tid == 0) { S.pending = 1; S.numLaunches = S.numLaunches + 1; }
    __syncthreads();
    if (leader) copy_words<sizeof(TrackState) / 4>(next, &S, tid, BLOCK);
    return;
  }

  const int level = S.level;
  const TrackLevel& L = job.lv[level];
  const int nb = L.nblocks;
  if (MODE == TS_FUSED && level != lvlPending) { cand = 0; bx = (int)blockIdx.x; }
  if (bx >= nb || cand >= S.ncand) return;
  const int tile = xcd_tile(bx, nb);
  EvalCtx a;
  make_ctx_dev(job, S, level, a);
  if (BATCH && MODE == TS_EVAL && cand > 0) ctx_set_pose(a, A.recs_in[cand]);
  gbyte* wasGood = (gbyte*)(L.writeMask ? (cand == 0 ? job.wasGood : spec.wasGoodSide + (size_t)(cand - 1) * spec.maskStride) : nullptr);
  const int work = a.npts >= 0 ? a.npts : a.w * a.h;
  float acc[RS_END];
#pragma unroll
  for (int k = 0; k < RS_END; k++) acc[k] = 0.f;
  int key0 = -1, key1 = -1, key2 = -1;
  if (BATCH && L.tilePx > 0) {
    if (!(havePre && level == lvlPending)) strip_request(L, tile, wave, lane, cntv, ow);
    eval_strip<BLOCK>(a, L.tilePx, tile, work, cntv, ow, (unsigned*)s_red , wasGood, acc, key0, key1, key2, tid TRACE_ARGS);
  } else if (!BATCH && L.evalBatch != 0) {
    eval_groups_of_four(a, tile * BLOCK + tid, nb * BLOCK, work, wasGood, acc, key0, key1, key2);
  } else {
    eval_plain(a, tile * BLOCK + tid, nb * BLOCK, work, wasGood, acc, key0, key1, key2);
  }
  PHASE_MARK(5);
  TRACE_PUT(tr_, 0, 10, level); TRACE_PUT(tr_, 0, 11, nb); TRACE_PUT(tr_, 0, 26, lvlPending);
  reduce_and_store<BLOCK, BATCH, MODE>(a, L, S, tile, acc, key0, key1, key2, s_red, s_sum, s_wtop, s_top, A.sums_out + (size_t)cand * RS_COLS * A.max_rows,
                                       A.topkey_out + (size_t)cand * A.max_rows, A.topval_out + (size_t)cand * A.max_rows * (TAIL_ROWS * TAIL_STRIDE), tid);
  if (MODE == TS_FUSED && leader) copy_words<sizeof(TrackState) / 4>(next, &S, tid, BLOCK);
  if (MODE == TS_FUSED && leader && tid == 0 && spec.last != 0) out->exhausted = spec.seq;
  LAUNCH_LOG(3, pendingIn_, ncandIn_, S.lastCand);
  PHASE_MARK(6);
  TRACE_PUT(tr_, 0, 9, wall_clock64());
}

template <int BLOCK, bool BATCH, int MODE = TS_FUSED>
__global__ __launch_bounds__(BLOCK) void k_track_step(TrackJob jobv, const TrackJob* __restrict__ jobs, TrackState* __restrict__ st2,
                                                       TrackScratch sc, TrackSummary* __restrict__ out, int parity, int first, TrackSpec spec) {
#ifdef LSD_ORDER_CHECK
  if (!BATCH && spec.dbgCounters && threadIdx.x == 0) {
    const unsigned long long fin = __hip_atomic_load(&spec.dbgCounters[0], __ATOMIC_RELAXED, __HIP_MEMORY_SCOPE_AGENT);
    if (fin < spec.dbgCum) {
      __hip_atomic_fetch_add(&spec.dbgCounters[1], 1ull, __ATOMIC_RELAXED, __HIP_MEMORY_SCOPE_AGENT);
      __hip_atomic_fetch_max(&spec.dbgCounters[2], spec.dbgCum - fin, __ATOMIC_RELAXED, __HIP_MEMORY_SCOPE_AGENT);
    }
  }
#endif
  track_step_impl<BLOCK, BATCH, MODE>(jobv, jobs, st2, sc, out, parity, first, spec);
#ifdef LSD_ORDER_CHECK
  __syncthreads();
  if (!BATCH && spec.dbgCounters && threadIdx.x == 0) __hip_atomic_fetch_add(&spec.dbgCounters[0], 1ull, __ATOMIC_RELEASE, __HIP_MEMORY_SCOPE_AGENT);
#endif
}

#define LSD_SOLO_TRIPS 9
#define LSD_SOLO_MAX_PTS (LSD_SOLO_TRIPS * 512)
#define LSD_SOLO_LDS_PTS 4544
static_assert(LSD_SOLO_LDS_PTS <= LSD_SOLO_MAX_PTS, "every point of the LDS lists has a register slot");
constexpr int lsd_solo_max_interior() {
  int best = 0;
  for (int w = 3; w <= LSD_SOLO_MAX_PX / 3; w++) {
    const int h = LSD_SOLO_MAX_PX / w;
    if ((w - 2) * (h - 2) > best) best = (w - 2) * (h - 2);
  }
  return best;
}
static_assert(lsd_solo_max_interior() <= LSD_SOLO_LDS_PTS, "the dense interior of any level k_track_solo takes fits its LDS lists");
__device__ __forceinline__ void solo_taps(const v4f* s_tex, const int w, const PointWarp& q, const bool fetch, PointTexels& t) {
  const int ix = fetch ? (int)q.u_new : 0;
  const int iy = fetch ? (int)q.v_new : 0;
  const v4f* bp = s_tex + (ix + __mul24(iy, w));
  const v4f v00 = bp[0], v10 = bp[1], v01 = bp[w], v11 = bp[w + 1];
  t.t00 = Texel3{v00.x, v00.y, v00.z}; t.t10 = Texel3{v10.x, v10.y, v10.z};
  t.t01 = Texel3{v01.x, v01.y, v01.z}; t.t11 = Texel3{v11.x, v11.y, v11.z};
}
template <int BLOCK>
__global__ __launch_bounds__(BLOCK) void k_track_solo(const TrackJob* __restrict__ jobs, TrackState* __restrict__ st2, TrackSummary* __restrict__ outs,
                                                          const int parity, const int doneWord) {
  const TrackJob& job = jobs[blockIdx.x];
  st2 += 2 * (size_t)blockIdx.x;
  TrackSummary* out = outs + blockIdx.x;
  constexpr int WAVES = BLOCK / 64;
  constexpr int HALF = BLOCK / 2;
  constexpr int CPP = RS_END;
  constexpr int RSLICE = BLOCK / CPP;
  constexpr int RRUN = (HALF + RSLICE - 1) / RSLICE;
  constexpr int TRIPS = LSD_SOLO_TRIPS;
  static_assert(WAVES * 3 <= 64, "top-3 merge in one wave");
  static_assert((size_t)TRIPS * BLOCK * 4 <= sizeof(float) * (CPP * (HALF + 1) + RRUN), "the level's list borrows the reduction buffer");
  __shared__ TrackState S;
  __shared__ LmShared sh;
  __shared__ LmPar s_par;
  __shared__ __attribute__((aligned(16))) float s_red[CPP * (HALF + 1) + RRUN];
  __shared__ float s_sum[RSLICE][64];
  __shared__ float s_sub[TAIL_ROWS][TAIL_STRIDE];
  __shared__ int s_wtop[WAVES][3];
  __shared__ v4f s_tex[LSD_SOLO_MAX_PX];
  __shared__ float s_var[LSD_SOLO_LDS_PTS], s_img[LSD_SOLO_LDS_PTS];
  const int tid = threadIdx.x, wave = tid >> 6, lane = tid & 63;
  track_state_begin(S, job, tid);
  __syncthreads();
  int listLevel = -1, total = 0;
  EvalCtx a;
  unsigned pXY[TRIPS];
  float pZ[TRIPS];
// ... 209 lines not shown
  T.q = {p[0], p[1], p[2], p[3]};
  T.t[0] = p[4]; T.t[1] = p[5]; T.t[2] = p[6];
  float inc[6];
  gj6_solve_wave(S.A, S.b, damp[c], sh.gj, lane, inc);
  const lsdm::SE3fH Tn = se3f_mul_wave(se3f_exp_wave(inc, lane), T, lane);
  if (lane == 0) {
#pragma unroll
    for (int i = 0; i < 6; i++) inc6[c * 6 + i] = inc[i];
    float* o = Tn7 + c * 7;
    o[0] = Tn.q.w; o[1] = Tn.q.x; o[2] = Tn.q.y; o[3] = Tn.q.z; o[4] = Tn.t[0]; o[5] = Tn.t[1]; o[6] = Tn.t[2];
  }
}

struct ScratchLayout { size_t topkey, topval, recs, end; };
static constexpr ScratchLayout scratch_layout(size_t jobs, size_t trials, size_t rows) {
  const size_t slots = jobs * 2 * trials;
  const size_t topkey = slots * RS_COLS * rows, topval = topkey + slots * 4 * rows, recs = topval + slots * 96 * rows;
  return {topkey, topval, recs, recs + slots * 32};
}
static_assert(scratch_layout(1, LSD_SPEC_MAX, 304).end * 4 == (size_t)LSD_SPEC_MAX * (2 * RS_COLS * 304 * 4 + 2 * 304 * 16 + 2 * 304 * 96 * 4 + 2 * 32 * 4) &&
              scratch_layout(8, LSD_BATCH_SPEC_MAX, 304).end * 4 == 8 * (size_t)LSD_BATCH_SPEC_MAX * (2 * RS_COLS * 304 * 4 + 2 * 304 * 16 + 2 * 304 * 96 * 4 + 2 * 32 * 4) &&
              scratch_layout(8, LSD_BATCH_SPEC_MAX, 304).recs == 8 * (size_t)LSD_BATCH_SPEC_MAX * (2 * RS_COLS * 304 + 2 * 4 * 304 + 2 * 96 * 304),
              "scratch arena: byte count and offsets");
static TrackScratch scratch_at(const lsdhip_tracker* t, float* base, size_t jobs, size_t trials, int cmax) {
  const ScratchLayout lay = scratch_layout(jobs, trials, (size_t)t->max_blocks);
  TrackScratch sc;
  sc.sums = base;
  sc.topkey = (int4*)(base + lay.topkey);
  sc.topval = base + lay.topval;
  sc.recs = cmax > 1 ? (TrialRecord*)(base + lay.recs) : nullptr;
  sc.max_rows = t->max_blocks;
  sc.cmax = cmax;
#ifdef LSD_PHASE_TRACE
  sc.trace = t->d_trace;
#endif
  return sc;
}

extern "C" int lsdhip_tracker_create(lsdhip_ctx* c, lsdhip_tracker** out) {
  if (!c || !out) return LSDHIP_E_ARG;
  HIPCHK(hipSetDevice(c->device));
  lsdhip_tracker* t = new lsdhip_tracker();
  t->ctx = c;
  const int maxIterations[6] = {5, 20, 50, 100, 100, 100};
  for (int l = 0; l < LSD_LEVELS; l++) {
    t->lambdaInitial[l] = 0;
    t->stepSizeMin[l] = 1e-8;
    t->convergenceEps[l] = 0.999f;
    t->maxItsPerLvl[l] = maxIterations[l];
  }
  if (const char* e = getenv("LSDHIP_TRACK_BLOCK")) t->block = atoi(e);
  if (const char* e = getenv("LSDHIP_TRACK_CAP")) t->grid_cap = atoi(e);
  if (const char* e = getenv("LSDHIP_EVAL_BATCH")) t->evalBatch = atoi(e) != 0;
  if (t->block != 256) { lsd_set_error("LSDHIP_TRACK_BLOCK must be 256"); delete t; return LSDHIP_E_ARG; }
  t->grid_cap = lsd_grid_cap(t->grid_cap, t->block, RS_END);
  t->max_blocks = t->grid_cap;
  const size_t partials_bytes = scratch_layout(1, LSD_SPEC_MAX, (size_t)t->max_blocks).end * sizeof(float);
  if (const char* e = getenv("LSDHIP_SPEC")) t->specC = atoi(e);
  if (t->specC < 1) t->specC = 1;
  if (t->specC > LSD_SPEC_MAX) t->specC = LSD_SPEC_MAX;
  if (const char* e = getenv("LSDHIP_SPEC_CAP")) t->specCap = atoi(e) & ~7;
  if (const char* e = getenv("LSDHIP_SPEC_CAPS")) {
    int v[LSD_LEVELS] = {0, 0, 0, 0, 0};
    sscanf(e, "%d,%d,%d,%d,%d", &v[0], &v[1], &v[2], &v[3], &v[4]);
    for (int l = 0; l < LSD_LEVELS; l++) t->specCaps[l] = v[l] < 0 ? 0 : (v[l] & ~7);
  }
  if (const char* e = getenv("LSDHIP_SPEC_LEVELS")) {
    int v[LSD_LEVELS] = {0, 0, 0, 0, 0};
    sscanf(e, "%d,%d,%d,%d,%d", &v[0], &v[1], &v[2], &v[3], &v[4]);
    for (int l = 0; l < LSD_LEVELS; l++) t->specLevel[l] = v[l] < 0 ? 0 : (v[l] > LSD_SPEC_MAX ? LSD_SPEC_MAX : v[l]);
  }
  t->maskStride = (((size_t)c->wl[LSD_TRACK_MIN_LEVEL] * c->hl[LSD_TRACK_MIN_LEVEL]) + 255) & ~(size_t)255;
  HIPCHK(hipMalloc((void**)&t->d_maskSide, 2 * t->maskStride * (LSD_SPEC_MAX - 1)));
  HIPCHK(hipMemsetAsync(t->d_maskSide, 0, 2 * t->maskStride * (LSD_SPEC_MAX - 1), c->stream));
  HIPCHK(hipMalloc((void**)&t->d_partials, partials_bytes));
  HIPCHK(hipMemsetAsync(t->d_partials, 0, partials_bytes, c->stream));
#ifdef LSD_ORDER_CHECK
  {
    const size_t nd = 8 + 2 * 8192;
    HIPCHK(hipMalloc((void**)&t->d_dbg, nd * 8));
    std::vector<unsigned long long> init(nd, 0);
    for (size_t i = 8; i < nd; i += 2) init[i] = ~0ull;
    HIPCHK(hipMemcpy(t->d_dbg, init.data(), nd * 8, hipMemcpyHostToDevice));
  }
#endif
#ifdef LSD_DEVTOOLS
  HIPCHK(hipMalloc((void**)&t->d_log, 4096 * 16 * 4));
  HIPCHK(hipMemset(t->d_log, 0, 4096 * 16 * 4));
#endif
  HIPCHK(hipMalloc((void**)&t->d_state, 2 * sizeof(TrackState)));
  HIPCHK(hipMemsetAsync(t->d_state, 0, 2 * sizeof(TrackState), c->stream));
#ifdef LSD_PHASE_TRACE
  HIPCHK(hipMalloc((void**)&t->d_trace, (1 + 4096 * LSD_TRACE_WORDS) * 8));
  HIPCHK(hipMemsetAsync(t->d_trace, 0, (1 + 4096 * LSD_TRACE_WORDS) * 8, c->stream));
#endif
  HIPCHK(hipHostMalloc((void**)&t->h_summary, sizeof(TrackSummary), hipHostMallocMapped));
  HIPCHK(hipHostGetDevicePointer((void**)&t->d_summary, t->h_summary, 0));
  memset(t->h_summary, 0, sizeof(TrackSummary));
  const char* env = getenv("LSDHIP_HOST_LM");
  t->hostLM = env && env[0] == '1';
  if (const char* e = getenv("LSDHIP_SPIN")) t->spinWait = e[0] != '0';
  if (const char* e = getenv("LSDHIP_BUDGET_EXTRA")) { t->budgetExtra = atoi(e); if (t->budgetExtra < 1) t->budgetExtra = 1; }
  if (const char* e = getenv("LSDHIP_BUDGET_FIXED")) { t->budgetFixed = atoi(e); if (t->budgetFixed < 1) t->budgetFixed = 0; }
  *out = t;
  return LSDHIP_OK;
}
// ... 5 lines not shown
    for (size_t i = 0; i < c->pendingMerges.size();)
      if (c->pendingMerges[i].doneSeq == &t->maskMergeSeq[0] || c->pendingMerges[i].doneSeq == &t->maskMergeSeq[1]) c->pendingMerges.erase(c->pendingMerges.begin() + i);
      else i++;
  }
#ifdef LSD_DEVTOOLS
  if (getenv("LSDHIP_TRACK_DEBUG") && t->dbgJobs > 0)
    fprintf(stderr, "TRACKDBG jobs %lld launches enqueued %.2f/job, budget misses %lld, host launch %.1f us/job, host wait %.1f us/job\n", t->dbgJobs,
            (double)t->dbgEnqueued / t->dbgJobs, t->dbgMisses, t->dbgLaunchNs / 1e3 / t->dbgJobs, t->dbgWaitNs / 1e3 / t->dbgJobs);
#endif
  (void)hipSetDevice(t->ctx->device);
  (void)hipStreamSynchronize(t->ctx->stream);
  if (t->h_overlapSums) (void)hipHostFree(t->h_overlapSums);
#ifdef LSD_ORDER_CHECK
  {
    std::vector<unsigned long long> h(8 + 2 * 8192, 0);
    (void)hipMemcpy(h.data(), t->d_dbg, h.size() * 8, hipMemcpyDeviceToHost);
    int used = 0, split = 0;
    for (size_t i = 8; i < h.size(); i += 2) if (h[i] != ~0ull) { used++; if (h[i] != h[i + 1]) split++; }
    if (const char* path = getenv("LSDHIP_ORDER_DUMP")) {
      if (FILE* f = fopen(path, "w")) {
        for (size_t i = 8; i < h.size(); i += 2) if (h[i] != ~0ull) fprintf(f, "%zu %llx %llx\n", (i - 8) / 2, h[i], h[i + 1]);
        fclose(f);
      }
    }
    fprintf(stderr, "ORDERCHECK: %llu workgroups finished (%llu launched), %llu started before every earlier workgroup had finished (largest deficit %llu); "
                    "%d launch slots hashed, %d in which the workgroups did NOT all see the same totals\n", h[0], t->dbgCum, h[1], h[2], used, split);
  }
#endif
  if (t->d_dbg) (void)hipFree(t->d_dbg);
#ifdef LSD_PHASE_TRACE
  if (const char* path = getenv("LSDHIP_TRACE_FILE")) {
    std::vector<unsigned long long> h(1 + 4096 * LSD_TRACE_WORDS);
    if (hipMemcpy(h.data(), t->d_trace, h.size() * 8, hipMemcpyDeviceToHost) == hipSuccess) {
      if (FILE* f = fopen(path, "w")) {
        unsigned long long n = h[0] < 4096 ? h[0] : 4096;
        for (unsigned long long i = 0; i < n; i++) {
          for (int k = 0; k < LSD_TRACE_WORDS; k++) fprintf(f, "%llu ", h[1 + i * LSD_TRACE_WORDS + k]);
          fprintf(f, "\n");
        }
        fclose(f);
      }
    }
  }
  (void)hipFree(t->d_trace);
#endif
  if (t->d_bjobs) { (void)hipFree(t->d_bjobs); (void)hipFree(t->d_bstate); (void)hipFree(t->d_bscratch); (void)hipHostFree(t->h_bjobs); (void)hipHostFree(t->h_bsummary); }
  (void)hipFree(t->d_partials);
  (void)hipFree(t->d_maskSide);
  (void)hipFree(t->d_state);
#ifdef LSD_DEVTOOLS
  (void)hipFree(t->d_log);
#endif
  (void)hipHostFree(t->h_summary);
  if (t->d_pts) (void)hipFree(t->d_pts);
  delete t;
}
extern "C" int lsdhip_tracker_set_enqueue_hook(lsdhip_tracker* t, lsdhip_enqueue_hook fn, void* user) {
  if (!t) return LSDHIP_E_ARG;
  t->enqueueHook = fn;
  t->enqueueHookUser = user;
  return LSDHIP_OK;
}
extern "C" int lsdhip_tracker_get_settings(const lsdhip_tracker* t, lsdhip_tracker_settings* o) {
  if (!t || !o) return LSDHIP_E_ARG;
  o->lambdaSuccessFac = t->lambdaSuccessFac; o->lambdaFailFac = t->lambdaFailFac;
  for (int l = 0; l < LSD_LEVELS; l++) {
    o->lambdaInitial[l] = t->lambdaInitial[l]; o->stepSizeMin[l] = t->stepSizeMin[l]; o->convergenceEps[l] = t->convergenceEps[l];
    o->maxItsPerLvl[l] = t->maxItsPerLvl[l];
  }
  o->lambdaInitialTestTrack = t->lambdaInitialTestTrack; o->stepSizeMinTestTrack = t->stepSizeMinTestTrack;
  o->convergenceEpsTestTrack = t->convergenceEpsTestTrack; o->maxItsTestTrack = t->maxItsTestTrack;
  o->huber_d = t->huber_d; o->var_weight = t->var_weight;
  return LSDHIP_OK;
}
extern "C" int lsdhip_tracker_set_settings(lsdhip_tracker* t, const lsdhip_tracker_settings* in) {
  if (!t || !in) return LSDHIP_E_ARG;
  t->lambdaSuccessFac = in->lambdaSuccessFac; t->lambdaFailFac = in->lambdaFailFac;
  for (int l = 0; l < LSD_LEVELS; l++) {
    t->lambdaInitial[l] = in->lambdaInitial[l]; t->stepSizeMin[l] = in->stepSizeMin[l]; t->convergenceEps[l] = in->convergenceEps[l];
    t->maxItsPerLvl[l] = in->maxItsPerLvl[l];
  }
  t->lambdaInitialTestTrack = in->lambdaInitialTestTrack; t->stepSizeMinTestTrack = in->stepSizeMinTestTrack;
  t->convergenceEpsTestTrack = in->convergenceEpsTestTrack; t->maxItsTestTrack = in->maxItsTestTrack;
  t->huber_d = in->huber_d; t->var_weight = in->var_weight;
  return LSDHIP_OK;
}
extern "C" int lsdhip_tracker_exec_stats(const lsdhip_tracker* t, int out[8]) {
  if (!t || !out) return LSDHIP_E_ARG;
  out[0] = 0; out[1] = 0; out[2] = 0;
  for (int l = 0; l < LSD_LEVELS; l++) out[3 + l] = t->levelEvaluations[l];
  return LSDHIP_OK;
}
extern "C" int lsdhip_tracker_set_speculation(lsdhip_tracker* t, int trials, int finestLevelWorkgroups) {
  if (!t || trials < 1 || trials > LSD_SPEC_MAX || finestLevelWorkgroups < 0) { lsd_set_error("lsdhip_tracker_set_speculation: trials must be 1..%d", LSD_SPEC_MAX); return LSDHIP_E_ARG; }
  LSD_CTX_LOCK(t->ctx);
  t->specC = trials;
  t->specAuto = false;
  if (finestLevelWorkgroups > 0) t->specCap = finestLevelWorkgroups < 8 ? 8 : (finestLevelWorkgroups & ~7);
  for (int l = 0; l < LSD_LEVELS; l++) t->specLevel[l] = 0;
  t->recent = LaunchHistory{};
  return LSDHIP_OK;
}
extern "C" int lsdhip_tracker_set_batch_coarse_min_jobs(lsdhip_tracker* t, int minJobs) {
  if (!t || minJobs < 0) { lsd_set_error("lsdhip_tracker_set_batch_coarse_min_jobs: minJobs must be >= 0"); return LSDHIP_E_ARG; }
  LSD_CTX_LOCK(t->ctx);
  t->soloMinJobs = minJobs;
// ... 249 lines not shown
  TrackScratch sc = scratch_of(t);
  t->launchOrdinal++;
  spec.seq = launch_seq(t);
  spec.last = last;
  dev_log_pointer(t, spec);
#ifdef LSD_ORDER_CHECK
  spec.dbgCum = t->dbgCum;
  spec.dbgCounters = t->d_dbg;
  t->dbgCum += (unsigned long long)grid;
#endif
  hipLaunchKernelGGL((k_track_step<256, false>), dim3(grid), dim3(256), 0, c->stream, job, (const TrackJob*)nullptr, t->d_state, sc,
                     t->d_summary, parity, first, spec);
}
static int launch_steps(lsdhip_tracker* t, const TrackJob& job, const TrackSpec& spec, int grid, int steps, int* parity, int* first) {
  const DevTime tl0 = dev_now();
  for (int i = 0; i < steps; i++) {
    launch_step(t, job, spec, grid, *parity, *first, i + 1 == steps);
    lsdhip_host_mark(20);
    *first = 0;
    *parity ^= 1;
  }
  dev_launches_queued(t, steps, tl0);
  HIPCHK(hipGetLastError());
  return LSDHIP_OK;
}
struct EvalOut {
  int warped_size;
  float retval;
  float weightedError;
  float A[36], b[6], lsError;
  double num_constraints;
};

static void eval_out_of(const TrackSummary* S, EvalOut* eo) {
  const float* r = S->sums;
  int M = (int)r[RS_M];
  eo->warped_size = M;
  eo->retval = r[RS_SUMRES2] / r[RS_GOOD];
  eo->weightedError = r[RS_WERR] / ((M >> 2) << 2);
  size_t num_constraints = (size_t)6 * (size_t)(M >> 2);
  float n = (float)num_constraints;
  int k = RS_A0;
  for (int i = 0; i < 6; i++)
    for (int j = i; j < 6; j++, k++) {
      float v = (0.0f + r[k]) / n;
      eo->A[i * 6 + j] = v;
      eo->A[j * 6 + i] = v;
    }
  for (int i = 0; i < 6; i++) eo->b[i] = (0.0f - r[RS_B0 + i]) / n;
  eo->lsError = (0.0f + r[RS_ERR]) / n;
  eo->num_constraints = (double)num_constraints;
}

static int evaluate_pose(lsdhip_tracker* t, TrackJob& job, const lsdm::SE3fH& T, int level, EvalOut* eo) {
  lsdhip_ctx* c = t->ctx;
  LSD_CTX_LOCK(c);
  job.evalOnly = 1;
  job.lastLevel = level;
  job.topLevel = level;
  job.T0 = T;
  job.aff_a0 = t->affineEstimation_a; job.aff_b0 = t->affineEstimation_b;
  t->h_summary->done = 0;
  t->jobTag = 0;
  const TrackSpec spec = TrackSpec{};
  if (int rcp = prof_collect(c)) return rcp;
  if (c->prof_on) HIPCHK(hipEventRecord(c->ev_a, c->stream));
  launch_step(t, job, spec, job.lv[level].nblocks, 0, 1, 0);
  if (c->prof_on) HIPCHK(hipEventRecord(c->ev_b, c->stream));
  launch_step(t, job, spec, 1, 1, 0, 0);
  HIPCHK(hipGetLastError());
  HIPCHK(hipStreamSynchronize(c->stream));
  const TrackSummary* S = t->h_summary;
  if (c->prof_on) {
    float ms = 0;
    HIPCHK(hipEventElapsedTime(&ms, c->ev_a, c->ev_b));
    c->prof_ms += ms;
    c->prof_launches++;
    c->prof_bytes += S->bytes;
  }
  t->numEvaluations++;
  t->pointUsage = S->pointUsage; t->lastGoodCount = S->goodCount; t->lastBadCount = S->badCount; t->lastMeanRes = S->meanRes;
  t->affineEstimation_a_lastIt = S->aff_a_lastIt; t->affineEstimation_b_lastIt = S->aff_b_lastIt;
  eval_out_of(S, eo);
  return LSDHIP_OK;
}

static void record_of(const TrackSummary* S, lsdhip_residual_record* out) {
  EvalOut ev;
  eval_out_of(S, &ev);
  out->warped_size = ev.warped_size;
  out->goodCount = S->goodCount; out->badCount = S->badCount; out->pointUsage = S->pointUsage;
  out->meanRes = S->meanRes; out->retval = ev.retval;
  out->affine_a_lastIt = S->aff_a_lastIt; out->affine_b_lastIt = S->aff_b_lastIt;
  out->weightedError = ev.weightedError;
  memcpy(out->A, ev.A, sizeof(ev.A)); memcpy(out->b, ev.b, sizeof(ev.b));
  out->lsError = ev.lsError; out->num_constraints = ev.num_constraints;
}

static int lm_level_host(lsdhip_tracker* t, TrackJob& job, int lvl, lsdm::SE3fH& referenceToFrame, float* lastResidualOut) {
  lsdhip_ctx* c = t->ctx;
  LSD_CTX_LOCK(c);
  const TrackLevel& L = job.lv[lvl];
  EvalOut ev;
  int rc = evaluate_pose(t, job, referenceToFrame, lvl, &ev);
  if (rc) return rc;
  if (ev.warped_size < L.minWarped) return LSDHIP_DIVERGED;
  if (c->params.useAffineLightningEstimation) {
    t->affineEstimation_a = t->affineEstimation_a_lastIt;
    t->affineEstimation_b = t->affineEstimation_b_lastIt;
// ... 86 lines not shown
    if (sample) { HIPCHK(hipEventRecord(c->ev_b, c->stream)); c->prof_pending = true; }
    if (guard == 0 && hook && t->enqueueHook) t->enqueueHook(t->enqueueHookUser);
    bool finished = false;
    if (int rc = wait(guard, &finished)) return rc;
    if (finished) return LSDHIP_OK;
    if (int rc = prof_collect(c)) return rc;
    budget = topUp(guard);
  }
  lsd_set_error("%s did not terminate", what);
  return LSDHIP_E_STATE;
}

static uint8_t* side_planes(const lsdhip_tracker* t) { return t->d_maskSide + (size_t)t->maskSet * t->maskStride * (LSD_SPEC_MAX - 1); }
static int claim_side_planes(lsdhip_tracker* t) {
  lsdhip_ctx* c = t->ctx;
  t->maskSet ^= 1;
  if (c->pipeline && t->maskMergeSeq[t->maskSet] != 0) {
    if (t->maskMergeSeq[t->maskSet] < 0) { if (int rcf = lsd_flush_merges(c)) return rcf; }
    if (t->maskMergeSeq[t->maskSet] > c->mSeq && lsd_m_record(c) < 0) return LSDHIP_E_HIP;
    if (int rcw = lsd_t_wait_m(c, t->maskMergeSeq[t->maskSet])) return rcw;
    t->maskMergeSeq[t->maskSet] = 0;
  }
  return LSDHIP_OK;
}
static SinglePlan plan_job(const lsdhip_tracker* t, TrackJob& job) {
  LevelWork lv[LSD_LEVELS];
  SpecPolicy p;
  p.specC = t->specC; p.specAuto = t->specAuto; p.specCap = t->specCap; p.grid_cap = t->grid_cap; p.block = t->block;
  for (int l = 0; l < LSD_LEVELS; l++) {
    const TrackLevel& L = job.lv[l];
    lv[l] = {L.npts >= 0 ? (long long)L.npts : (long long)L.w * L.h, {L.nblocks, L.singlePass, L.tilePx}};
    p.specLevel[l] = t->specLevel[l]; p.specCaps[l] = t->specCaps[l];
  }
  const SinglePlan P = lsd_single_plan(lv, p, job.lastLevel, job.topLevel);
  for (int l = 0; l < LSD_LEVELS; l++) {
    job.lv[l].nblocks = P.tiling[l].nblocks; job.lv[l].singlePass = P.tiling[l].singlePass;
    job.lv[l].evalBatch = eval_batch_level(t, job.lv[l]);
  }
  return P;
}
static TrackSpec job_spec(const lsdhip_tracker* t, const SinglePlan& P) {
  TrackSpec spec = TrackSpec{};
  spec.specC = t->specC;
  spec.specGrid = P.specGrid;
  for (int l = 0; l < LSD_LEVELS; l++) spec.trials[l] = P.trials[l];
  spec.wasGoodSide = side_planes(t);
  spec.maskStride = (unsigned)t->maskStride;
  spec.copyMask = t->ctx->pipeline ? 0 : 1;
  return spec;
}

static int track_device(lsdhip_tracker* t, TrackJob& job, int topLevel, const lsdm::SE3fH& T0, lsdm::SE3fH* Tout) {
  lsdhip_ctx* c = t->ctx;
  job.evalOnly = 0;
  job.topLevel = topLevel;
  job.T0 = T0;
  job.aff_a0 = 1.0f; job.aff_b0 = 0.0f;
  if (int rc = claim_side_planes(t)) return rc;
  const SinglePlan plan = plan_job(t, job);
  const TrackSpec spec = job_spec(t, plan);
  TrackSummary* S = t->h_summary;
  volatile const int* done = &S->done;
  S->done = 0;
  const long long myEpoch = ++c->enqEpoch;
  const bool sample = c->prof_on && ((c->prof_tick++ & 7) == 0);
  dev_job_begins(t);
  t->jobTag = (t->jobTag % 0x7FFFF) + 1;
  t->launchOrdinal = 0;
  S->seq = 0;
  S->exhausted = 0;
  int parity = 0, first = 1;
  if (int rc = prof_collect(c)) return rc;
  lsdhip_host_mark(2);
  auto enqueue = [&](int budget) {
    const int rc = launch_steps(t, job, spec, plan.grid, budget, &parity, &first);
    lsdhip_host_mark(3);
    return rc;
  };
  auto wait = [&](int guard, bool* finished) -> int {
    lsdhip_host_mark(4);
    DevWaitClock waitClock_(t);
    {
      LsdCtxUnlocked unlocked_(c);
      if (t->spinWait) {
        volatile const int* exhausted = &S->exhausted;
        const int tag = t->jobTag, lastSeq = launch_seq(t);
        if (int rc = lsd_spin_until(c, [=]() { return *done == tag || *exhausted == lastSeq; }, lsd_deadline(LSD_JOB_WAIT_S), LSD_WAIT_JOB)) return rc;
      } else {
        HIPCHK(hipStreamSynchronize(c->stream));
      }
    }
    lsdhip_host_mark(5);
    if (*done != t->jobTag) {
      dev_budget_missed(t);
      HIPCHK(hipStreamSynchronize(c->stream));
      if (int rc = dev_dump_first_launch(t, job, topLevel, guard)) return rc;
    }
    *finished = *done == t->jobTag;
    return LSDHIP_OK;
  };
  auto topUp = [&](int guard) {
    if (t->jobKf && t->jobKf->depthVersion != t->jobKfVersion && guard < 8) {
      t->jobKfVersion = t->jobKf->depthVersion;
      S->done = 0;
      parity = 0; first = 1;
      return 12;
// ... 54 lines not shown
    job.wasGood = frame->d_wasGood;
    job.lv[level].writeMask = 1;
  }
  job.trackFrameSemantics = 1;
  job.evalOnly = 1;
  job.lastLevel = level;
  job.topLevel = level;
  job.T0 = pose_from7(T7);
  job.aff_a0 = aff_a; job.aff_b0 = aff_b;
  return LSDHIP_OK;
}
static int fill_permaref_job(lsdhip_tracker* t, TrackJob& job, BatchShape shape, const float* pts_pos, const float* pts_colvar, int npts,
                             lsdhip_frame* frame, const lsdm::SE3fH& T0) {
  const int L = LSD_QUICK_KF_CHECK_LVL;
  fill_job_common(t, job);
  if (int rcl = fill_level(t, job, shape, L, nullptr, frame, pts_pos, pts_colvar, npts)) return rcl;
  job.lv[L].lambdaInitial = t->lambdaInitialTestTrack; job.lv[L].stepSizeMin = t->stepSizeMinTestTrack;
  job.lv[L].convergenceEps = t->convergenceEpsTestTrack; job.lv[L].maxIts = (int)t->maxItsTestTrack;
  job.lastLevel = L;
  job.topLevel = L;
  job.trackFrameSemantics = 0;
  job.evalOnly = 0;
  job.T0 = T0;
  job.aff_a0 = 1.0f; job.aff_b0 = 0.0f;
  return LSDHIP_OK;
}
static int finish_permaref(lsdhip_tracker* t, bool diverged, const lsdm::SE3fH& referenceToFrame, lsdhip_track_result* out) {
  if (diverged) return finish_diverged(t, out);
  t->diverged = false;
  t->trackingWasGood = tracking_was_good(t, LSD_QUICK_KF_CHECK_LVL);
  fill_result(t, lsdm::se3d_from_f(referenceToFrame), out);
  return LSDHIP_OK;
}
static int finish_trackframe(lsdhip_tracker* t, const TrackSummary* S, lsdhip_frame* kf, lsdhip_frame* frame, lsdhip_track_result* out) {
  lsdhip_ctx* c = t->ctx;
  LSD_CTX_LOCK(c);
  take_summary(t, S);
  if (S->diverged) return finish_diverged(t, out);
  t->diverged = false;
  t->trackingWasGood = tracking_was_good(t, LSD_TRACK_MIN_LEVEL);
  if (t->trackingWasGood) kf->numFramesTrackedOnThis++;
  frame->initialTrackedResidual = t->lastResidual / t->pointUsage;
  lsdm::SE3dH f2r = lsdm::se3d_from_f(lsdm::se3f_inverse(pose_of(S)));
  frame->thisToParent_raw.q = f2r.q;
  lsdm::q_normalize(frame->thisToParent_raw.q);
  frame->thisToParent_raw.t[0] = f2r.t[0]; frame->thisToParent_raw.t[1] = f2r.t[1]; frame->thisToParent_raw.t[2] = f2r.t[2];
  frame->thisToParent_raw.s = 1;
  frame->trackingParent = kf;
  frame->trackingParentID = kf->id;
  fill_result(t, f2r, out);
  return LSDHIP_OK;
}

extern "C" int lsdhip_tracker_track(lsdhip_tracker* t, lsdhip_frame* kf, lsdhip_frame* frame, const double init[7],
                                    lsdhip_track_result* out) {
  if (!t || !kf || !frame || !init || !out) return LSDHIP_E_ARG;
  if (!kf->hasIDepth) { lsd_set_error("lsdhip_tracker_track: keyframe %d has no depth", kf->id); return LSDHIP_E_STATE; }
  lsdhip_ctx* c = t->ctx;
  LSD_CTX_LOCK(c);
  HIPCHK(hipSetDevice(c->device));
  t->diverged = false;
  t->trackingWasGood = true;
  t->affineEstimation_a = 1; t->affineEstimation_b = 0;
  t->numEvaluations = 0; t->numWarpUpdates = 0;
  TrackJob job;
  LsdTrackJobScope tjob_(c, false);
  if (c->pipeline) {
    long long need = frame->readySeq > kf->readySeq ? frame->readySeq : kf->readySeq;
    if (kf->depthSeq > need) need = kf->depthSeq;
    if (int rcw = lsd_t_wait_m(c, need)) return rcw;
  }
  int rc = fill_trackframe_job(t, job, BatchShape{}, kf, frame);
  if (rc) return rc;
  if (int rcg = lsd_gate_open(c)) return rcg;
  if (int rcd = lsd_pipe_dummy(c)) return rcd;
  dev_trace_job(c, kf, frame, init);
  lsdm::SE3fH referenceToFrame = lsdm::se3f_from_d(lsdm::se3d_inverse(lsdm::se3d_from7(init)));

  if (t->hostLM) {
    float last_residual = 0;
    rc = LSDHIP_OK;
    for (int lvl = LSD_TRACK_MAX_LEVEL - 1; lvl >= LSD_TRACK_MIN_LEVEL && rc == LSDHIP_OK; lvl--)
      rc = lm_level_host(t, job, lvl, referenceToFrame, &last_residual);
    t->lastResidual = last_residual;
    if (rc == LSDHIP_DIVERGED) return finish_diverged(t, out);
    if (rc) return rc;
    const TrackSummary S = host_lm_summary(t, referenceToFrame, last_residual);
    return finish_trackframe(t, &S, kf, frame, out);
  }
  t->jobKf = kf;
  t->jobKfVersion = kf->depthVersion;
  const lsdm::SE3fH T0 = referenceToFrame;
  dev_trace_launched(t, 26, frame);
  rc = track_device(t, job, LSD_TRACK_MAX_LEVEL - 1, T0, &referenceToFrame);
  if (rc == LSDHIP_OK || rc == LSDHIP_DIVERGED) rc = dev_replay_check(t, job, kf, frame, T0, &referenceToFrame, rc);
  t->jobKf = nullptr;
  if (rc != LSDHIP_OK && rc != LSDHIP_DIVERGED) return rc;
  lsdhip_host_mark(6);
  dev_trace_result(t, 20, frame);
  if (c->pipeline && rc == LSDHIP_OK && t->h_summary->lastCand > 0 && t->h_summary->level == LSD_TRACK_MIN_LEVEL) {
    const uint8_t* side = side_planes(t) + (size_t)(t->h_summary->lastCand - 1) * t->maskStride;
    t->maskMergeSeq[t->maskSet] = -1;
    c->pendingMerges.push_back({frame->d_wasGood, side, &t->maskMergeSeq[t->maskSet]});
  }
  rc = finish_trackframe(t, t->h_summary, kf, frame, out);
  lsdhip_host_mark(7);
  return rc;
}

static int batch_reserve(lsdhip_tracker* t, int n) {
  lsdhip_ctx* c = t->ctx;
  LSD_CTX_LOCK(c);
  if (n <= t->batch_capacity) return LSDHIP_OK;
  HIPCHK(hipStreamSynchronize(c->stream));
  if (t->d_bjobs) { (void)hipFree(t->d_bjobs); (void)hipFree(t->d_bstate); (void)hipFree(t->d_bscratch); (void)hipHostFree(t->h_bjobs); (void)hipHostFree(t->h_bsummary); }
  t->batch_capacity = n < 8 ? 8 : n;
  const size_t B = (size_t)t->batch_capacity, bytes = scratch_layout(B, LSD_BATCH_SPEC_MAX, (size_t)t->max_blocks).end * sizeof(float);
  HIPCHK(hipMalloc((void**)&t->d_bjobs, B * sizeof(TrackJob)));
  HIPCHK(hipMalloc((void**)&t->d_bstate, B * 2 * sizeof(TrackState)));
  HIPCHK(hipMalloc((void**)&t->d_bscratch, bytes));
  HIPCHK(hipMemsetAsync(t->d_bscratch, 0, bytes, c->stream));
  HIPCHK(hipHostMalloc((void**)&t->h_bjobs, B * sizeof(TrackJob), hipHostMallocDefault));
  HIPCHK(hipHostMalloc((void**)&t->h_bsummary, B * sizeof(TrackSummary), hipHostMallocMapped));
  return LSDHIP_OK;
}
struct BatchLaunch { TrackScratch sc; TrackSummary* d_sum; };
static int batch_launch_record(lsdhip_tracker* t, int cmax, BatchLaunch* out) {
  out->sc = scratch_at(t, t->d_bscratch, (size_t)t->batch_capacity, LSD_BATCH_SPEC_MAX, cmax);
  HIPCHK(hipHostGetDevicePointer((void**)&out->d_sum, t->h_bsummary, 0));
  return LSDHIP_OK;
}
template <int MODE>
static void launch_batch_step(lsdhip_tracker* t, const BatchLaunch& r, int grid, int n, int parity, int first, const TrackSpec& spec) {
  hipLaunchKernelGGL((k_track_step<256, true, MODE>), dim3(grid, n), dim3(256), 0, t->ctx->stream, t->h_bjobs[0], (const TrackJob*)t->d_bjobs, t->d_bstate,
                     r.sc, r.d_sum, parity, first, spec);
}
static BatchPlan plan_batch(const lsdhip_tracker* t, int n) {
  const BatchEnv& env = batch_env();
  BatchPolicy p;
  p.specC = t->specC; p.specMax = env.specMax; p.specPixels = env.specPixels; p.fused = env.fused;
  p.spinWait = t->spinWait; p.poll = env.poll;
  p.soloMin = t->soloMinJobs >= 0 ? t->soloMinJobs : env.soloMin;
  return lsd_batch_plan(n, p, [t](int j, int l) {
    const TrackJob& job = t->h_bjobs[j];
    const TrackLevel& L = job.lv[l];
    return BatchLevel{(long long)L.w * L.h, L.nblocks, L.tilePx, L.writeMask, job.lastLevel <= l && l <= job.topLevel};
  });
}
static int batch_run(lsdhip_tracker* t, int n, bool callHook, bool record) {
  lsdhip_ctx* c = t->ctx;
  LSD_CTX_LOCK(c);
  const BatchEnv& env = batch_env();
  const BatchPlan plan = plan_batch(t, n);
  TrackSpec spec = TrackSpec{};
#ifdef LSD_PHASE_TRACE
  spec.traceWg = env.traceWg;
#endif
  if (plan.speculates) {
// ... 497 lines not shown
```

lsd_slam_amd/driver.py:

```python
import ctypes as C
import os

import numpy as np

from . import capi

_HERE = os.path.dirname(os.path.abspath(__file__))
DRIVER_PATH = os.path.join(_HERE, "liblsdhip_driver.so")
_lib = None


class LoopStats(C.Structure):
    _fields_ = [("seconds_track", C.c_double), ("seconds_map", C.c_double), ("seconds_keyframe", C.c_double), ("frames", C.c_longlong),
                ("updates", C.c_longlong), ("keyframes", C.c_longlong), ("evaluations", C.c_longlong), ("tracked_good", C.c_longlong),
                ("level_evaluations", C.c_longlong * 5), ("track_launches", C.c_longlong), ("dropped", C.c_longlong)]


EXPORTED_SYMBOLS = ["lsdloop_create", "lsdloop_destroy", "lsdloop_run", "lsdloop_get_stats", "lsdloop_reset_stats",
                    "lsdloop_copy_keyframe_planes", "lsdloop_set_keyframe_ring", "lsdloop_keyframes_exported", "lsdloop_ctx",
                    "lsdloop_last_error", "lsdloop_keep_keyframes", "lsdloop_keyframe_log", "lsdloop_set_live_queue", "lsdloop_set_pipeline", "lsdloop_enable_reactivation", "lsdloop_keyframe_changes", "lsdloop_reactivation_counts", "lsdloop_download_map", "lsdloop_set_speculation", "lsdloop_observe_time", "lsdloop_comm_unique_id", "lsdloop_comm_init", "lsdloop_comm_destroy",
                    "lsdloop_gather_keyframes", "lsdband_create", "lsdband_destroy", "lsdband_window_rows", "lsdband_layout", "lsdband_load",
                    "lsdband_get", "lsdband_comm_init", "lsdband_run", "lsdband_synchronize", "lsdband_halo_bytes_per_pass", "lsdband_set_packed_exchange", "lsdband_set_overlap", "lsdband_tile_runs", "lsdband_plan", "lsdband_ipc_init", "lsdband_ipc_connect", "lsdband_ipc_failed", "lsdloop_gather_counts", "lsdloop_ipc_init", "lsdloop_ipc_connect", "lsdloop_ipc_result", "lsdloop_observe_work",
                    "lsdloopbatch_create", "lsdloopbatch_destroy", "lsdloopbatch_run", "lsdloopbatch_get_stats", "lsdloopbatch_ctx", "lsdloopbatch_set_keyframe_phases", "lsdloopbatch_set_pipeline", "lsdloopbatch_set_coarse_min_jobs", "lsdloopbatch_dropped",
                    "lsdloopbatch_keep_keyframes", "lsdloopbatch_keyframe_log", "lsdloopbatch_last_result", "lsdloopbatch_download_map",
                    "lsdloopbatch_set_cloud_sinks", "lsdloopbatch_cloud", "lsdloopbatch_cloud_pose", "lsdloopbatch_keyframe_handle"]


def lib():
    global _lib
    if _lib is None:
        capi.lib()
        if not os.path.exists(DRIVER_PATH):
            raise RuntimeError("liblsdhip_driver.so is missing (%s): run __graft_entry__.build()" % DRIVER_PATH)
        L = C.CDLL(DRIVER_PATH)
        vp, i = C.c_void_p, C.c_int
        L.lsdloop_create.restype = i
        L.lsdloop_create.argtypes = [i, i, i, vp, vp, i, vp, i, C.POINTER(vp)]
        L.lsdloop_destroy.restype = None
        L.lsdloop_destroy.argtypes = [vp]
        L.lsdloop_run.restype = i
        L.lsdloop_run.argtypes = [vp, vp, i, i, vp]
        L.lsdloop_get_stats.restype = i
        L.lsdloop_get_stats.argtypes = [vp, C.POINTER(LoopStats)]
        L.lsdloop_reset_stats.restype = i
        L.lsdloop_reset_stats.argtypes = [vp]
        L.lsdloop_copy_keyframe_planes.restype = i
        L.lsdloop_copy_keyframe_planes.argtypes = [vp, vp, vp]
        L.lsdloop_set_keyframe_ring.restype = i
        L.lsdloop_set_keyframe_ring.argtypes = [vp, vp, i]
        L.lsdloop_keyframes_exported.restype = C.c_longlong
        L.lsdloop_keyframes_exported.argtypes = [vp]
        L.lsdloop_keep_keyframes.restype = i
        L.lsdloop_keep_keyframes.argtypes = [vp, i]
        L.lsdloop_keyframe_log.restype = i
        L.lsdloop_keyframe_log.argtypes = [vp, vp, vp, i]
        L.lsdloop_enable_reactivation.restype = i
        L.lsdloop_enable_reactivation.argtypes = [vp, i]
        L.lsdloop_keyframe_changes.restype = i
        L.lsdloop_keyframe_changes.argtypes = [vp, vp, i]
        L.lsdloop_reactivation_counts.restype = i
        L.lsdloop_reactivation_counts.argtypes = [vp, vp]
        L.lsdloop_download_map.restype = i
        L.lsdloop_download_map.argtypes = [vp, vp]
        L.lsdloop_set_live_queue.restype = i
        L.lsdloop_set_live_queue.argtypes = [vp, i]
        L.lsdloop_set_pipeline.restype = i
        L.lsdloop_set_pipeline.argtypes = [vp, i]
        L.lsdloop_set_speculation.restype = i
        L.lsdloop_set_speculation.argtypes = [vp, i, i]
        L.lsdloop_observe_time.restype = i
        L.lsdloop_observe_time.argtypes = [vp, vp, vp]
        L.lsdloop_observe_work.restype = i
        L.lsdloop_observe_work.argtypes = [vp, vp]
        L.lsdloop_comm_unique_id.restype = i
        L.lsdloop_comm_unique_id.argtypes = [vp]
        for name, args in (("lsdband_create", [i, i, i, i, i, i, C.POINTER(vp)]), ("lsdband_window_rows", [vp]), ("lsdband_layout", [vp, i, vp]),
                           ("lsdband_load", [vp, i, vp, vp]), ("lsdband_get", [vp, i, vp]), ("lsdband_comm_init", [vp, vp, i, i, vp]),
                           ("lsdband_run", [vp, i]), ("lsdband_synchronize", [vp]), ("lsdband_set_packed_exchange", [vp, i]), ("lsdband_set_overlap", [vp, i]), ("lsdband_tile_runs", [i, i, i, vp, i]), ("lsdband_plan", [i, i, vp, vp, vp, i]),
                           ("lsdband_ipc_init", [vp, i, i, vp, vp]), ("lsdband_ipc_connect", [vp, vp]), ("lsdband_ipc_failed", [vp])):
            getattr(L, name).restype = i
            getattr(L, name).argtypes = args
        L.lsdband_destroy.restype = None
        L.lsdband_destroy.argtypes = [vp]
        L.lsdband_halo_bytes_per_pass.restype = C.c_longlong
        L.lsdband_halo_bytes_per_pass.argtypes = [vp]
        L.lsdloop_comm_init.restype = i
        L.lsdloop_comm_init.argtypes = [vp, vp, i, i]
        L.lsdloop_comm_destroy.restype = i
        L.lsdloop_comm_destroy.argtypes = [vp]
        L.lsdloop_gather_keyframes.restype = i
        L.lsdloop_gather_keyframes.argtypes = [vp, i, i, vp, C.c_longlong]
        for name, args in (("lsdloop_gather_counts", [vp, vp, i]), ("lsdloop_ipc_init", [vp, i, i, i, vp]), ("lsdloop_ipc_connect", [vp, vp]),
                           ("lsdloop_ipc_result", [vp, vp, vp])):
            getattr(L, name).restype = i
            getattr(L, name).argtypes = args
        L.lsdloop_ctx.restype = vp
        L.lsdloop_ctx.argtypes = [vp]
        L.lsdloopbatch_create.restype = i
        L.lsdloopbatch_create.argtypes = [i, i, i, vp, i, vp, i, vp, i, C.POINTER(vp)]
        L.lsdloopbatch_destroy.restype = None
        L.lsdloopbatch_destroy.argtypes = [vp]
        L.lsdloopbatch_run.restype = i
        L.lsdloopbatch_run.argtypes = [vp, vp, i, vp]
        L.lsdloopbatch_get_stats.restype = i
        L.lsdloopbatch_get_stats.argtypes = [vp, vp]
        L.lsdloopbatch_ctx.restype = vp
        L.lsdloopbatch_ctx.argtypes = [vp]
        L.lsdloopbatch_set_keyframe_phases.restype = i
        L.lsdloopbatch_set_keyframe_phases.argtypes = [vp, vp]
        L.lsdloopbatch_set_pipeline.restype = i
        L.lsdloopbatch_set_pipeline.argtypes = [vp, i]
        L.lsdloopbatch_set_coarse_min_jobs.restype = i
        L.lsdloopbatch_set_coarse_min_jobs.argtypes = [vp, i]
        L.lsdloopbatch_dropped.restype = C.c_longlong
        L.lsdloopbatch_dropped.argtypes = [vp, i]
        L.lsdloopbatch_keep_keyframes.restype = i
        L.lsdloopbatch_keep_keyframes.argtypes = [vp, i]
        L.lsdloopbatch_keyframe_log.restype = i
        L.lsdloopbatch_keyframe_log.argtypes = [vp, i, vp, vp, i]
        L.lsdloopbatch_last_result.restype = i
        L.lsdloopbatch_last_result.argtypes = [vp, i, vp]
        L.lsdloopbatch_download_map.restype = i
# ... 138 lines not shown
    def stats(self):
        s = LoopStats()
        _check(self.L.lsdloop_get_stats(self.h_, C.byref(s)))
        return s

    def reset_stats(self):
        _check(self.L.lsdloop_reset_stats(self.h_))

    def copy_keyframe_planes(self, idepth_ptr, var_ptr):
        _check(self.L.lsdloop_copy_keyframe_planes(self.h_, C.c_void_p(idepth_ptr), C.c_void_p(var_ptr)))

    def set_keyframe_ring(self, ring_ptr, slots):
        _check(self.L.lsdloop_set_keyframe_ring(self.h_, C.c_void_p(ring_ptr) if ring_ptr else None, slots))

    def gather_counts(self, world):
        out = (C.c_int * world)()
        n = _check(self.L.lsdloop_gather_counts(self.h_, out, world))
        return list(out)[:n]

    def ipc_init(self, rank, world, root=0):
        out = (C.c_ubyte * 64)()
        _check(self.L.lsdloop_ipc_init(self.h_, rank, world, root, out))
        self._ipc_world = world
        return bytes(out)

    def ipc_connect(self, root_handle):
        buf = (C.c_ubyte * 64).from_buffer_copy(root_handle)
        _check(self.L.lsdloop_ipc_connect(self.h_, buf))

    def ipc_result(self):
        counts = (C.c_int * self._ipc_world)()
        ptr = C.c_void_p()
        fail = self.L.lsdloop_ipc_result(self.h_, counts, C.byref(ptr))
        if fail < 0:
            _check(fail)
        return fail, list(counts), ptr.value

    def keep_keyframes(self, on=True):
        _check(self.L.lsdloop_keep_keyframes(self.h_, int(on)))

    def keyframe_log(self, max_entries=4096):
        sc = np.zeros(max_entries, np.float64)
        pts = np.zeros(max_entries, np.int64)
        n = _check(self.L.lsdloop_keyframe_log(self.h_, sc.ctypes.data, pts.ctypes.data, max_entries))
        n = min(n, max_entries)
        return sc[:n], pts[:n]

    def set_live_queue(self, frames):
        _check(self.L.lsdloop_set_live_queue(self.h_, int(frames)))

    def set_speculation(self, trials, finest_level_workgroups=0):
        _check(self.L.lsdloop_set_speculation(self.h_, int(trials), int(finest_level_workgroups)))

    def set_pipeline(self, on=True):
        _check(self.L.lsdloop_set_pipeline(self.h_, int(bool(on))))

    def enable_reactivation(self, max_keyframes):
        _check(self.L.lsdloop_enable_reactivation(self.h_, int(max_keyframes)))

    def keyframe_changes(self, max_entries=4096):
        out = np.zeros((max_entries, 7), np.int32)
        n = _check(self.L.lsdloop_keyframe_changes(self.h_, out.ctypes.data, max_entries))
        return out[:min(n, max_entries)].copy()

    def download_map(self):
        out = np.zeros(self.w * self.h, dtype=capi.HYP_DTYPE)
        _check(self.L.lsdloop_download_map(self.h_, out.ctypes.data))
        return out.reshape(self.h, self.w)

    def reactivation_counts(self):
        out = np.zeros(2, np.int64)
        _check(self.L.lsdloop_reactivation_counts(self.h_, out.ctypes.data))
        return int(out[0]), int(out[1])

    def observe_time(self):
        ms, n = C.c_double(), C.c_longlong()
        _check(self.L.lsdloop_observe_time(self.h_, C.byref(ms), C.byref(n)))
        return ms.value, n.value

    def observe_work(self):
        out = np.zeros(3, np.float64)
        _check(self.L.lsdloop_observe_work(self.h_, out.ctypes.data))
        return float(out[0]), float(out[1]), float(out[2])

    @staticmethod
    def comm_unique_id():
        buf = (C.c_ubyte * 128)()
        _check(lib().lsdloop_comm_unique_id(buf))
        return bytes(buf)

    def comm_init(self, unique_id, rank, world):
        buf = (C.c_ubyte * 128).from_buffer_copy(unique_id)
        _check(self.L.lsdloop_comm_init(self.h_, buf, rank, world))

    def comm_destroy(self):
        _check(self.L.lsdloop_comm_destroy(self.h_))

    def gather_keyframes(self, count, root, recv_ptr, stride_floats):
        _check(self.L.lsdloop_gather_keyframes(self.h_, int(count), int(root), C.c_void_p(recv_ptr) if recv_ptr else None, int(stride_floats)))

    def keyframes_exported(self):
        return int(self.L.lsdloop_keyframes_exported(self.h_))

    def ctx_handle(self):
        return self.L.lsdloop_ctx(self.h_)
```

lsd_slam_amd/driver/slam_loop.cpp:

```cpp
#include <chrono>
#include <cstdlib>
#include <cstring>
#include <dlfcn.h>
#include <string>

#include "../../include/lsd_slam_hip.hpp"
#include "../../include/lsdhip_driver.h"

using namespace lsd_slam_hip;

static thread_local std::string g_err;
typedef void* NcclComm;

struct lsdloop {
  std::unique_ptr<SlamLoop> loop;
  std::shared_ptr<Context> ctx;
  lsdloop_stats st{};
  double wall = 0;
  double gpu0[3] = {0, 0, 0};
  long long calls0[3] = {0, 0, 0};
  float* ring = nullptr;
  int ring_slots = 0;
  long long ring_count = 0;
  NcclComm comm = nullptr;
  int comm_rank = 0, comm_world = 1;
  std::vector<int> last_counts;
  int* counts_dev = nullptr;
  bool ipc = false;
  int ipc_root = 0;
  char* mailbox = nullptr;
  int* ipc_fail = nullptr;
  long long gathers = 0;
  float* ipc_data() const { return (float*)(mailbox + 4096); }
  int* ipc_flag(int rank, int which) const { return (int*)(mailbox + 64 + (size_t)rank * 16 + (size_t)which * 4); }
};

namespace {
struct NcclId { char internal[128]; };
struct Rccl {
  int (*GetUniqueId)(NcclId*) = nullptr;
  int (*CommInitRank)(NcclComm*, int, NcclId, int) = nullptr;
  int (*CommDestroy)(NcclComm) = nullptr;
  int (*GroupStart)() = nullptr;
  int (*GroupEnd)() = nullptr;
  int (*Send)(const void*, size_t, int, int, NcclComm, void*) = nullptr;
  int (*Recv)(void*, size_t, int, int, NcclComm, void*) = nullptr;
  int (*AllGather)(const void*, void*, size_t, int, NcclComm, void*) = nullptr;
  const char* (*GetErrorString)(int) = nullptr;
  bool ok = false;
  std::string why;
};
Rccl& rccl() {
  static Rccl r;
  static bool tried = false;
  if (tried) return r;
  tried = true;
  void* h = RTLD_DEFAULT;
  if (!dlsym(h, "ncclCommInitRank")) {
    h = dlopen("librccl.so", RTLD_NOW | RTLD_GLOBAL);
    if (!h) h = dlopen("/opt/rocm/lib/librccl.so", RTLD_NOW | RTLD_GLOBAL);
    if (!h) { r.why = "no RCCL in the process and librccl.so not found"; return r; }
  }
  auto sym = [&](const char* n) { void* p = dlsym(h, n); if (!p) r.why = std::string("RCCL symbol missing: ") + n; return p; };
  r.GetUniqueId = (int (*)(NcclId*))sym("ncclGetUniqueId");
  r.CommInitRank = (int (*)(NcclComm*, int, NcclId, int))sym("ncclCommInitRank");
  r.CommDestroy = (int (*)(NcclComm))sym("ncclCommDestroy");
  r.GroupStart = (int (*)())sym("ncclGroupStart");
  r.GroupEnd = (int (*)())sym("ncclGroupEnd");
  r.Send = (int (*)(const void*, size_t, int, int, NcclComm, void*))sym("ncclSend");
  r.Recv = (int (*)(void*, size_t, int, int, NcclComm, void*))sym("ncclRecv");
  r.AllGather = (int (*)(const void*, void*, size_t, int, NcclComm, void*))sym("ncclAllGather");
  r.GetErrorString = (const char* (*)(int))sym("ncclGetErrorString");
  r.ok = r.GetUniqueId && r.CommInitRank && r.CommDestroy && r.GroupStart && r.GroupEnd && r.Send && r.Recv && r.AllGather;
  return r;
}
}

static double now_s() { return std::chrono::duration<double>(std::chrono::steady_clock::now().time_since_epoch()).count(); }

// ... 177 lines not shown
    return (int)log.size();
  } catch (const Error& e) { g_err = e.what(); return e.status < 0 ? e.status : LSDHIP_E_STATE; }
}
extern "C" int lsdloopbatch_last_result(lsdloopbatch* l, int s, lsdhip_track_result* out) {
  if (!l || !out || s < 0 || s >= l->loop->size()) return LSDHIP_E_ARG;
  *out = l->loop->sequence(s).last;
  return LSDHIP_OK;
}
extern "C" int lsdloopbatch_download_map(lsdloopbatch* l, int s, lsdhip_hypothesis* out) {
  if (!l || !out || s < 0 || s >= l->loop->size()) return LSDHIP_E_ARG;
  try {
    const std::vector<lsdhip_hypothesis> m = l->loop->sequence(s).map.currentDepthMap();
    std::memcpy(out, m.data(), m.size() * sizeof(lsdhip_hypothesis));
    return LSDHIP_OK;
  } catch (const Error& e) { g_err = e.what(); return e.status < 0 ? e.status : LSDHIP_E_STATE; }
}
extern "C" int lsdloopbatch_set_keyframe_phases(lsdloopbatch* l, const int* phase) {
  if (!l || !phase) return LSDHIP_E_ARG;
  try {
    l->loop->setKeyframePhases(std::vector<int>(phase, phase + l->loop->size()));
    return LSDHIP_OK;
  } catch (const Error& e) {
    g_err = e.what();
    return e.status < 0 ? e.status : LSDHIP_E_STATE;
  }
}

extern "C" int lsdloop_run(lsdloop* l, const uint8_t* const* images, int n, int stop_at_keyframe, double* out7) {
  if (!l || !images || n < 0) return LSDHIP_E_ARG;
  try {
    int done = 0;
    long updSeen = l->loop->numUpdates;
    static const bool prefetch = !std::getenv("LSDHIP_NO_PREFETCH");
    const double t0 = now_s();
    for (int i = 0; i < n; i++) {
      SlamLoop& L = *l->loop;
      const long ev0 = L.evaluations;
      const long la0 = L.launches;
      const long good0 = L.numTrackedGood;
      const long drop0 = L.numDropped;
      long lev0[5];
      for (int k = 0; k < 5; k++) lev0[k] = L.levelEvaluations[k];
      SE3 est = L.step(images[i], [](double) {}, (prefetch && i + 1 < n) ? images[i + 1] : nullptr);
      l->st.frames++;
      l->st.updates += L.numUpdates - updSeen;
      updSeen = L.numUpdates;
      l->st.evaluations += L.evaluations - ev0;
      l->st.track_launches += L.launches - la0;
      l->st.tracked_good += L.numTrackedGood - good0;
      l->st.dropped += L.numDropped - drop0;
      for (int k = 0; k < 5; k++) l->st.level_evaluations[k] += L.levelEvaluations[k] - lev0[k];
      if (L.newKeyframe) l->st.keyframes++;
      if (out7) est.to7(out7 + 7 * (size_t)i);
      done++;
      if (stop_at_keyframe && L.newKeyframe) break;
    }
    l->loop->flushDeferredMapping();
    {
      const long upd = l->loop->numUpdates - updSeen;
      l->st.updates += upd;
    }
    l->ctx->synchronize();
    l->wall += now_s() - t0;
    return done;
  } catch (const Error& e) {
    g_err = e.what();
    return e.status > 0 ? -100 - e.status : e.status;
  } catch (const std::exception& e) {
    g_err = e.what();
    return LSDHIP_E_STATE;
  }
}
extern "C" int lsdloop_get_stats(lsdloop* l, lsdloop_stats* out) {
  if (!l || !out) return LSDHIP_E_ARG;
  try {
    double ms[3];
    long long calls[3];
    l->loop->map.gpuTimes(ms, calls);
    auto scaled = [&](int k, long n) {
      const long long sampled = calls[k] - l->calls0[k];
      if (sampled > 0) return (ms[k] - l->gpu0[k]) / (double)sampled * (double)n * 1e-3;
      return calls[k] > 0 ? ms[k] / (double)calls[k] * (double)n * 1e-3 : 0.0;
    };
    l->st.seconds_map = scaled(0, l->st.updates);
    l->st.seconds_keyframe = scaled(1, l->st.keyframes) + scaled(2, l->st.keyframes);
    l->st.seconds_track = l->loop->pipelined() ? l->wall : l->wall - l->st.seconds_map - l->st.seconds_keyframe;
    *out = l->st;
    return LSDHIP_OK;
  } catch (const Error& e) { g_err = e.what(); return e.status; }
}
extern "C" int lsdloop_reset_stats(lsdloop* l) {
  if (!l) return LSDHIP_E_ARG;
  try {
    l->loop->map.gpuTimes(l->gpu0, l->calls0);
    l->st = lsdloop_stats{};
    l->wall = 0;
    return LSDHIP_OK;
  } catch (const Error& e) { g_err = e.what(); return e.status; }
}
extern "C" int lsdloop_copy_keyframe_planes(lsdloop* l, float* idepth_dev, float* var_dev) {
  if (!l) return LSDHIP_E_ARG;
  try { l->loop->map.copyPlanesToDevice(idepth_dev, var_dev); return LSDHIP_OK; }
  catch (const Error& e) { g_err = e.what(); return e.status; }
}
extern "C" int lsdloop_set_keyframe_ring(lsdloop* l, float* ring_dev, int slots) {
  if (!l || (ring_dev && slots < 1)) return LSDHIP_E_ARG;
// ... 20 lines not shown
  try {
    const auto& log = l->loop->keyframeLog;
    for (int i = 0; i < (int)log.size() && i < max; i++) {
      if (scales_out) scales_out[i] = log[i]->thisToParent_raw().s;
      if (points_out) points_out[i] = log[i]->stats().numPoints;
    }
    return (int)log.size();
  } catch (const Error& e) { g_err = e.what(); return e.status; }
}
extern "C" int lsdloop_set_pipeline(lsdloop* l, int on) {
  if (!l) return LSDHIP_E_ARG;
  try { l->loop->setPipelined(on != 0); return LSDHIP_OK; }
  catch (const Error& e) { g_err = e.what(); return e.status; }
}
extern "C" int lsdloop_enable_reactivation(lsdloop* l, int max_keyframes) {
  if (!l) return LSDHIP_E_ARG;
  try { l->loop->enableReactivation(max_keyframes); return LSDHIP_OK; }
  catch (const Error& e) { g_err = e.what(); return e.status; }
}
extern "C" int lsdloop_keyframe_changes(lsdloop* l, int* out, int max) {
  if (!l || (max > 0 && !out)) return LSDHIP_E_ARG;
  const auto& log = l->loop->keyframeChanges;
  for (int i = 0; i < (int)log.size() && i < max; i++) {
    const SlamLoop::KeyframeChange& c = log[(size_t)i];
    int* o = out + 7 * (size_t)i;
    o[0] = c.frameId; o[1] = c.previousKfId; o[2] = c.newKfId; o[3] = c.reactivated ? 1 : 0;
    o[4] = c.numPotential; o[5] = c.numChecked; o[6] = c.numTracked;
  }
  return (int)log.size();
}
extern "C" int lsdloop_download_map(lsdloop* l, lsdhip_hypothesis* out) {
  if (!l || !out) return LSDHIP_E_ARG;
  try {
    l->loop->flushDeferredMapping();
    const std::vector<lsdhip_hypothesis> m = l->loop->map.currentDepthMap();
    std::memcpy(out, m.data(), m.size() * sizeof(lsdhip_hypothesis));
    return LSDHIP_OK;
  } catch (const Error& e) { g_err = e.what(); return e.status < 0 ? e.status : LSDHIP_E_STATE; }
}
extern "C" int lsdloop_reactivation_counts(lsdloop* l, long long out2[2]) {
  if (!l || !out2) return LSDHIP_E_ARG;
  out2[0] = l->loop->numReactivations; out2[1] = l->loop->numUnbanked;
  return LSDHIP_OK;
}
extern "C" int lsdloop_set_live_queue(lsdloop* l, int frames) {
  if (!l || frames < 1) return LSDHIP_E_ARG;
  l->loop->liveQueueLength = frames;
  return LSDHIP_OK;
}
extern "C" int lsdloop_set_speculation(lsdloop* l, int trials, int finest_level_workgroups) {
  if (!l) return LSDHIP_E_ARG;
  try { l->loop->tracker.setSpeculation(trials, finest_level_workgroups); return LSDHIP_OK; }
  catch (const Error& e) { g_err = e.what(); return e.status; }
}
extern "C" int lsdloop_observe_time(lsdloop* l, double* ms_out, long long* calls_out) {
  if (!l) return LSDHIP_E_ARG;
  return lsdhip_depth_observe_time(l->loop->map.handle(), ms_out, calls_out);
}
extern "C" int lsdloop_observe_work(lsdloop* l, double out3[3]) {
  if (!l) return LSDHIP_E_ARG;
  return lsdhip_depth_observe_work(l->loop->map.handle(), out3);
}
extern "C" int lsdloop_comm_unique_id(unsigned char out128[128]) {
  Rccl& R = rccl();
  if (!R.ok) { g_err = "RCCL unavailable: " + R.why; return LSDHIP_E_STATE; }
  NcclId id;
  const int rc = R.GetUniqueId(&id);
  if (rc != 0) { g_err = std::string("ncclGetUniqueId: ") + (R.GetErrorString ? R.GetErrorString(rc) : "?"); return LSDHIP_E_HIP; }
  std::memcpy(out128, id.internal, 128);
  return LSDHIP_OK;
}
extern "C" int lsdloop_comm_init(lsdloop* l, const unsigned char id128[128], int rank, int world) {
  if (!l || !id128 || rank < 0 || rank >= world) return LSDHIP_E_ARG;
  Rccl& R = rccl();
  if (!R.ok) { g_err = "RCCL unavailable: " + R.why; return LSDHIP_E_STATE; }
  if (l->comm) { R.CommDestroy(l->comm); l->comm = nullptr; }
  NcclId id;
  std::memcpy(id.internal, id128, 128);
  const int rc = R.CommInitRank(&l->comm, world, id, rank);
  if (rc != 0) { l->comm = nullptr; g_err = std::string("ncclCommInitRank: ") + (R.GetErrorString ? R.GetErrorString(rc) : "?"); return LSDHIP_E_HIP; }
  l->comm_rank = rank;
  l->comm_world = world;
  return LSDHIP_OK;
}
extern "C" int lsdloop_comm_destroy(lsdloop* l) {
  if (!l) return LSDHIP_E_ARG;
  if (l->comm) { rccl().CommDestroy(l->comm); l->comm = nullptr; }
  return LSDHIP_OK;
}
static int gather_ipc(lsdloop* l, int count) {
  const size_t plane2 = (size_t)2 * l->ctx->width() * l->ctx->height();
  const size_t slot_floats = (size_t)l->ring_slots * plane2;
  const long long g = l->gathers;
  try {
    lsdhip_ctx* c = l->ctx->handle();
    if (l->comm_rank == l->ipc_root) {
      for (int r = 0; r < l->comm_world; r++) if (r != l->ipc_root) check(lsdhip_ctx_flag_set(c, l->ipc_flag(r, 1), (int)g), "lsdhip_ctx_flag_set");
      if (count > 0) check(lsdhip_ctx_copy_dev(c, l->ipc_data() + (size_t)l->ipc_root * slot_floats, l->ring, (size_t)count * plane2 * sizeof(float)), "lsdhip_ctx_copy_dev");
      check(lsdhip_ctx_flag_set(c, l->ipc_flag(l->ipc_root, 2), count), "lsdhip_ctx_flag_set");
      for (int r = 0; r < l->comm_world; r++) if (r != l->ipc_root) check(lsdhip_ctx_flag_wait(c, l->ipc_flag(r, 0), (int)(g + 1), (int*)l->mailbox), "lsdhip_ctx_flag_wait");
    } else {
      if (g >= 1) check(lsdhip_ctx_flag_wait(c, l->ipc_flag(l->comm_rank, 1), (int)g, l->ipc_fail), "lsdhip_ctx_flag_wait");
      if (count > 0) check(lsdhip_ctx_copy_dev(c, l->ipc_data() + (size_t)l->comm_rank * slot_floats, l->ring, (size_t)count * plane2 * sizeof(float)), "lsdhip_ctx_copy_dev");
      check(lsdhip_ctx_flag_set(c, l->ipc_flag(l->comm_rank, 2), count), "lsdhip_ctx_flag_set");
      check(lsdhip_ctx_flag_set(c, l->ipc_flag(l->comm_rank, 0), (int)(g + 1)), "lsdhip_ctx_flag_set");
    }
// ... 512 lines not shown
```

Measured before the change: 5683.

## Link consecutive frame tracking jobs so the next frame starts in the same launch

Adds a linked-job mode to the fused tracker kernel. The kernel receives two job descriptions, and once the current frame's tracking converges it starts tracking the prefetched next frame from the derived pose, without waiting for a new host round trip. The goal is to hide per-frame launch and host synchronisation gaps between consecutive tracks. The cost is heavy bookkeeping: tags, a second summary buffer, paths for abandoning the linked job, and keyframe-version checks. Any mismatch could cause wasted work or rerunning the linked frame.

```diff
diff --git a/include/lsd_slam_hip.hpp b/include/lsd_slam_hip.hpp
--- a/include/lsd_slam_hip.hpp
+++ b/include/lsd_slam_hip.hpp
@@ -355,6 +355,18 @@
     hook_ = std::move(fn);
     check(lsdhip_tracker_set_enqueue_hook(h_, hook_ ? &SE3Tracker::hookTrampoline : nullptr, this), "lsdhip_tracker_set_enqueue_hook");
   }
+  void setLinkHook(std::function<Frame*()> fn) {
+    linkHook_ = std::move(fn);
+    check(lsdhip_tracker_set_link_hook(h_, linkHook_ ? &SE3Tracker::linkTrampoline : nullptr, this), "lsdhip_tracker_set_link_hook");
+  }
+  void setLinkJobs(bool on) { check(lsdhip_tracker_set_link_jobs(h_, on ? 1 : 0), "lsdhip_tracker_set_link_jobs"); }
+  void setLinkFrom(int launchIndex) { check(lsdhip_tracker_set_link_from(h_, launchIndex), "lsdhip_tracker_set_link_from"); }
+  void abandonLinked() { check(lsdhip_tracker_abandon_linked(h_), "lsdhip_tracker_abandon_linked"); }
+  std::array<long long, 4> linkStats() const {
+    std::array<long long, 4> o{};
+    check(lsdhip_tracker_link_stats(h_, o.data()), "lsdhip_tracker_link_stats");
+    return o;
+  }
   float checkPermaRefOverlap(Frame* reference, SE3 referenceToFrame) {
     double init[7];
     referenceToFrame.to7(init);
@@ -402,7 +414,15 @@
     SE3Tracker* t = static_cast<SE3Tracker*>(self);
     try { if (t->hook_) t->hook_(); } catch (...) { t->hookError_ = std::current_exception(); }
   }
+  static lsdhip_frame* linkTrampoline(void* self) {
+    SE3Tracker* t = static_cast<SE3Tracker*>(self);
+    try {
+      Frame* f = t->linkHook_ ? t->linkHook_() : nullptr;
+      return f ? f->handle() : nullptr;
+    } catch (...) { if (!t->hookError_) t->hookError_ = std::current_exception(); return nullptr; }
+  }
   std::function<void()> hook_;
+  std::function<Frame*()> linkHook_;
   std::exception_ptr hookError_;
   std::shared_ptr<Context> ctx_;
   lsdhip_tracker* h_ = nullptr;
@@ -673,7 +693,9 @@
       prefetched_ = makeFrame(frameId_ + 1, pendingNext_, true);
       prefetchedSrc_ = pendingNext_;
     });
-  }
+    tracker.setLinkHook([this]() -> Frame* { return linkableNext(); });
+  }
+  ~SlamLoop() { (void)lsdhip_tracker_abandon_linked(tracker.handle()); }
   SlamLoop(const SlamLoop&) = delete;
   SlamLoop& operator=(const SlamLoop&) = delete;
   void setPipelined(bool on) {
@@ -723,6 +745,7 @@
     onTrackEnd(lastTrackEnd);
     if (tracker.diverged || (numKeyframesFinished_ > 5  && !tracker.trackingWasGood)) {
       trackingLost = true;
+      tracker.abandonLinked();
       reference.invalidate();
       if (map.isValid()) {
         if (mappedOnKF_ >= 5 ) {
@@ -951,6 +974,15 @@
     numUpdates++;
     lsdhip_host_mark(14);
     if (onMappingIteration) onMappingIteration(map);
+  }
+  Frame* linkableNext() {
+    if (!pipelined_ || !prefetched_ || pendingKF_ || trackKF_ != keyframe) return nullptr;
+    if (kfEvery_ > 0 ? sinceKF_ + 1 >= kfEvery_ : mappedOnKF_ > 5 ) return nullptr;
+    if (trackKF_->depthHasBeenUpdatedFlag()) {
+      reference.importFrame(trackKF_.get());
+      trackKF_->clearDepthHasBeenUpdatedFlag();
+    }
+    return prefetched_.get();
   }
   std::shared_ptr<Frame> deferredMap_;
   std::shared_ptr<Frame> makeFrame(int id, const unsigned char* img, bool mayDefer = false) {
diff --git a/include/lsdhip.h b/include/lsdhip.h
--- a/include/lsdhip.h
+++ b/include/lsdhip.h
@@ -136,6 +136,12 @@
                                    int level, int repeats, double* ms_per_launch, double* bytes_per_launch);
 typedef void (*lsdhip_enqueue_hook)(void* user);
 int lsdhip_tracker_set_enqueue_hook(lsdhip_tracker* t, lsdhip_enqueue_hook fn, void* user);
+typedef lsdhip_frame* (*lsdhip_link_hook)(void* user);
+int lsdhip_tracker_set_link_hook(lsdhip_tracker* t, lsdhip_link_hook fn, void* user);
+int lsdhip_tracker_set_link_jobs(lsdhip_tracker* t, int on);
+int lsdhip_tracker_set_link_from(lsdhip_tracker* t, int launchIndex);
+int lsdhip_tracker_abandon_linked(lsdhip_tracker* t);
+int lsdhip_tracker_link_stats(const lsdhip_tracker* t, long long out[4]);
 int lsdhip_tracker_track(lsdhip_tracker* t, lsdhip_frame* keyframe, lsdhip_frame* frame,
                          const double frameToReference_initialEstimate[7], lsdhip_track_result* out);
 int lsdhip_tracker_track_batch(lsdhip_tracker* t, int n, lsdhip_frame** keyframes, lsdhip_frame** frames,
@@ -223,6 +229,7 @@
                                    const double* init_frameToReference, int startLevel, int finalLevel, lsdhip_sim3_result* results);
 int lsdhip_host_se3f_step(const float increment[6], const float referenceToFrame[7], float out[7]);
 int lsdhip_host_ldlt6(const float A[36], const float b[6], float x[6]);
+int lsdhip_host_next_start(const float referenceToFrame[7], float out[7], float twoStep[7]);
 int lsdhip_host_sim3_step(const double increment[7], const double referenceToFrame[8], double out[8]);
 int lsdhip_host_ldlt7(const float A[49], const float b[7], float x[7]);
 int lsdhip_devtest_se3f_lm_step(lsdhip_ctx* ctx, int n, const float* A, const float* b, const float* damp, const float* T, float* inc, float* Tn);
diff --git a/include/lsdhip_driver.h b/include/lsdhip_driver.h
--- a/include/lsdhip_driver.h
+++ b/include/lsdhip_driver.h
@@ -36,6 +36,11 @@
 int lsdloop_download_map(lsdloop* l, lsdhip_hypothesis* out);
 int lsdloop_set_live_queue(lsdloop* l, int frames);
 int lsdloop_set_speculation(lsdloop* l, int trials, int finest_level_workgroups);
+int lsdloop_set_link_jobs(lsdloop* l, int on, int from_launch);
+typedef struct lsdloop_frame_record { int numEvaluations, numWarpUpdates, numLaunches; float lastResidual, pointUsage; } lsdloop_frame_record;
+int lsdloop_keep_frame_log(lsdloop* l, int on);
+int lsdloop_frame_log(lsdloop* l, int max, lsdloop_frame_record* out);
+int lsdloop_link_stats(lsdloop* l, long long out4[4]);
 int lsdloop_observe_time(lsdloop* l, double* ms_out, long long* calls_out);
 int lsdloop_observe_work(lsdloop* l, double out3[3]);
 int lsdloop_comm_unique_id(unsigned char out128[128]);
diff --git a/lsd_slam_amd/capi.py b/lsd_slam_amd/capi.py
--- a/lsd_slam_amd/capi.py
+++ b/lsd_slam_amd/capi.py
@@ -150,6 +150,12 @@
         "lsdhip_tracker_summary_stats": (i, [vp, vp]),
         "lsdhip_tracker_step_stats": (i, [vp, vp]),
         "lsdhip_tracker_set_enqueue_hook": (i, [vp, vp, vp]),
+        "lsdhip_host_next_start": (i, [vp, vp, vp]),
+        "lsdhip_tracker_set_link_hook": (i, [vp, vp, vp]),
+        "lsdhip_tracker_set_link_jobs": (i, [vp, i]),
+        "lsdhip_tracker_set_link_from": (i, [vp, i]),
+        "lsdhip_tracker_abandon_linked": (i, [vp]),
+        "lsdhip_tracker_link_stats": (i, [vp, vp]),
         "lsdhip_tracker_track": (i, [vp, vp, vp, vp, C.POINTER(TrackResult)]),
         "lsdhip_tracker_track_batch": (i, [vp, i, pvp, pvp, vp, C.POINTER(TrackResult)]),
         "lsdhip_tracker_eval_throughput": (i, [vp, i, pvp, pvp, vp, i, i, C.POINTER(C.c_double), C.POINTER(C.c_double)]),
diff --git a/lsd_slam_amd/csrc/host_math.cpp b/lsd_slam_amd/csrc/host_math.cpp
--- a/lsd_slam_amd/csrc/host_math.cpp
+++ b/lsd_slam_amd/csrc/host_math.cpp
@@ -22,6 +22,18 @@
   out[0] = r.q.w; out[1] = r.q.x; out[2] = r.q.y; out[3] = r.q.z; out[4] = r.t[0]; out[5] = r.t[1]; out[6] = r.t[2];
   return LSDHIP_OK;
 }
+extern "C" int lsdhip_host_next_start(const float referenceToFrame[7], float out[7], float twoStep[7]) {
+  if (!referenceToFrame || !out || !twoStep) return LSDHIP_E_ARG;
+  lsdm::SE3fH T;
+  T.q = {referenceToFrame[0], referenceToFrame[1], referenceToFrame[2], referenceToFrame[3]};
+  T.t[0] = referenceToFrame[4]; T.t[1] = referenceToFrame[5]; T.t[2] = referenceToFrame[6];
+  auto put = [](const lsdm::SE3fH& P, float* o) { o[0] = P.q.w; o[1] = P.q.x; o[2] = P.q.y; o[3] = P.q.z; o[4] = P.t[0]; o[5] = P.t[1]; o[6] = P.t[2]; };
+  put(lsdm::se3f_next_start(T), out);
+  double result7[7];
+  lsdm::se3d_to7(lsdm::se3d_from_f(lsdm::se3f_inverse(T)), result7);
+  put(lsdm::se3f_from_d(lsdm::se3d_inverse(lsdm::se3d_from7(result7))), twoStep);
+  return LSDHIP_OK;
+}
 extern "C" int lsdhip_host_ldlt6(const float A[36], const float b[6], float x[6]) {
   if (!A || !b || !x) return LSDHIP_E_ARG;
   lsdm::ldlt6_solve(A, b, x);
diff --git a/lsd_slam_amd/csrc/lsdhip_internal.hpp b/lsd_slam_amd/csrc/lsdhip_internal.hpp
--- a/lsd_slam_amd/csrc/lsdhip_internal.hpp
+++ b/lsd_slam_amd/csrc/lsdhip_internal.hpp
@@ -121,6 +121,13 @@
   int ncand;
   int lastCand;
   int numLaunches;
+  int tag;
+};
+struct TrackSummary;
+struct TrackLink {
+  int curTag, nextTag;
+  TrackSummary* nextOut;
+  uint8_t* nextSide;
 };
 
 struct TrackSummary {
@@ -327,6 +334,26 @@
   long long dbgJobs = 0, dbgEnqueued = 0, dbgMisses = 0, dbgWaitNs = 0, dbgLaunchNs = 0;
   TrackSummary* h_summary = nullptr;
   TrackSummary* d_summary = nullptr;
+  bool linkJobs = true;
+  int linkFrom = 0;
+  int linkTail = 4;
+  lsdhip_link_hook linkHook = nullptr;
+  void* linkHookUser = nullptr;
+  TrackSummary* h_linkSummary = nullptr;
+  TrackSummary* d_linkSummary = nullptr;
+  int linkRecord = 0;
+  int linkParity = 0;
+  struct LinkedJob {
+    bool valid = false;
+    TrackJob job;
+    int tag = 0, maskSet = 0, record = 0;
+    lsdhip_frame* kf = nullptr; lsdhip_frame* frame = nullptr;
+    unsigned kfVersion = 0;
+    long long need = 0;
+    lsdm::SE3fH prevPose;
+    int ahead = 0;
+  } linked;
+  long long linkBegunEarly = 0, linkDescribed = 0, linkAlone = 0, linkAbandoned = 0;
   unsigned long long* d_trace = nullptr;
   int batch_capacity = 0;
   TrackJob* d_bjobs = nullptr;
diff --git a/lsd_slam_amd/csrc/pose_math.hpp b/lsd_slam_amd/csrc/pose_math.hpp
--- a/lsd_slam_amd/csrc/pose_math.hpp
+++ b/lsd_slam_amd/csrc/pose_math.hpp
@@ -77,6 +77,10 @@
   float nt[3] = {T.t[0] * -1.0f, T.t[1] * -1.0f, T.t[2] * -1.0f};
   q_rotate<Quatf, float>(r.q, nt, r.t);
   return r;
+}
+LSDM_HD SE3fH se3f_next_start(const SE3fH& referenceToFrame) {
+#pragma clang fp contract(off)
+  return se3f_from_d(se3d_inverse(se3d_from_f(se3f_inverse(referenceToFrame))));
 }
 LSDM_HD SE3fH se3f_mul(const SE3fH& a, const SE3fH& b) {
   SE3fH r = a;
diff --git a/lsd_slam_amd/csrc/tracker.hip b/lsd_slam_amd/csrc/tracker.hip
--- a/lsd_slam_amd/csrc/tracker.hip
+++ b/lsd_slam_amd/csrc/tracker.hip
@@ -41,10 +41,11 @@
 #endif
 
 enum { TS_FUSED = 0, TS_LM = 1, TS_EVAL = 2 };
-__device__ __forceinline__ void track_state_begin(TrackState& S, const TrackJob& job, const int tid) {
+__device__ __forceinline__ void track_state_begin(TrackState& S, const TrackJob& job, const int tid, const lsdm::SE3fH& T0, const int tag) {
   if (tid == 0) {
-    S.T = job.T0;
-    set_eval_pose(S, job.T0);
+    S.T = T0;
+    set_eval_pose(S, T0);
+    S.tag = tag;
     S.aff_a = job.aff_a0; S.aff_b = job.aff_b0; S.aff_a_lastIt = job.aff_a0; S.aff_b_lastIt = job.aff_b0;
     S.lastErr = 0; S.LM_lambda = 0; S.last_residual = 0;
     S.level = job.topLevel; S.iteration = 0; S.incTry = 0; S.phase = 0; S.pending = 0;
@@ -57,6 +58,7 @@
   if (tid < 36) S.A[tid] = 0;
   if (tid < 6) { S.b[tid] = 0; S.inc[tid] = 0; }
 }
+__device__ __forceinline__ void track_state_begin(TrackState& S, const TrackJob& job, const int tid) { track_state_begin(S, job, tid, job.T0, 0); }
 
 struct StepAddr {
   const float *sums_in, *topval_in;
@@ -559,20 +561,30 @@
 }
 #endif
 
+template <int JOBS = 1>
 __device__ __forceinline__ void warm_job_arguments() {
   typedef const unsigned __attribute__((address_space(4))) cuint;
   cuint* ka = (cuint*)__builtin_amdgcn_kernarg_segment_ptr();
   unsigned warm = 0;
 #pragma unroll
-  for (int i = 0; i < (int)(sizeof(TrackJob) / 4); i += 32) warm ^= ka[i];
+  for (int i = 0; i < (int)(JOBS * sizeof(TrackJob) / 4); i += 32) warm ^= ka[i];
   asm volatile("" ::"s"(warm));
 }
 
-template <int BLOCK, bool BATCH, int MODE>
+template <int BLOCK, bool BATCH, int MODE, bool LINK = false>
 __device__ __forceinline__ void track_step_impl(const TrackJob& jobv, const TrackJob* __restrict__ jobs, TrackState* __restrict__ st2,
-                                                TrackScratch sc, TrackSummary* __restrict__ out, int parity, int first, const TrackSpec& spec) {
-  const TrackJob& job = BATCH ? jobs[blockIdx.y] : jobv;
-  if (!BATCH) warm_job_arguments();
+                                                TrackScratch sc, TrackSummary* __restrict__ out, int parity, int first, const TrackSpec& spec,
+                                                const TrackJob& nextv, const TrackLink& link) {
+  static_assert(!LINK || (!BATCH && MODE == TS_FUSED), "only single jobs are linked");
+  static_assert(sizeof(TrackJob) % 8 == 0, "the second description follows the first without padding");
+  typedef const __attribute__((address_space(4))) TrackJob cjob;
+  cjob* const ka_ = (cjob*)__builtin_amdgcn_kernarg_segment_ptr();
+  const TrackJob* const curq = LINK ? (const TrackJob*)ka_ : &jobv;
+  const TrackJob* const nextq = LINK ? (const TrackJob*)(ka_ + 1) : &nextv;
+  const TrackJob* jq = BATCH ? &jobs[blockIdx.y] : curq;
+#define job (*jq)
+  bool onNext = false, began = false;
+  if (!BATCH) warm_job_arguments<LINK ? 2 : 1>();
   if (BATCH) { st2 += 2 * (size_t)blockIdx.y; out += blockIdx.y; }
   const StepAddr A = step_addr<BATCH, MODE>(sc, parity);
   constexpr int WAVES = BLOCK / 64, SUMW = WAVES - 1;
@@ -599,7 +611,12 @@
   unsigned long long* const tr_ = trace_open(sc.trace, trOn_ && tid == 0, &s_trp);
 #endif
   PHASE_MARK(0);
-  if (!BATCH && MODE == TS_FUSED && !first && !leader && st2[parity].done) return;
+  if (!LINK && !BATCH && MODE == TS_FUSED && !first && !leader && st2[parity].done) return;
+  if (LINK && !first && !leader) {
+    const TrackState* sp = st2 + parity;
+    const int d_ = sp->done, tg_ = sp->tag, dv_ = sp->diverged;
+    if (d_ && ((tg_ == link.curTag && (link.nextTag == 0 || dv_)) || (link.nextTag != 0 && tg_ == link.nextTag))) return;
+  }
   if (!BATCH && MODE == TS_FUSED && leader && tid == 0 && spec.seq != 0) out->seq = spec.seq;
   if (first) {
     track_state_begin(S, job, tid);
@@ -608,6 +625,23 @@
     if (SPEC_LM && A.cmax > 1 && tid < (int)(sizeof(s_rec) / 4)) ((float*)s_rec)[tid] = ((const float*)A.recs_in)[tid < (int)(sizeof(TrialRecord) / 4) * A.cmax ? tid : 0];
   }
   __syncthreads();
+  if (LINK && first) { if (tid == 0) S.tag = link.curTag; __syncthreads(); }
+  if (LINK && !first) {
+    const int tg_ = S.tag, d_ = S.done, dv_ = S.diverged;
+    const bool onCur = tg_ == link.curTag, onNxt = link.nextTag != 0 && tg_ == link.nextTag;
+    const bool beginNext = onCur && d_ && !dv_ && link.nextTag != 0, beginCur = !onCur && !onNxt;
+    onNext = onNxt || beginNext;
+    if (onNext) jq = nextq;
+    if (beginNext || beginCur) {
+      lsdm::SE3fH T0b = curq->T0;
+      if (beginNext && tid == 0) T0b = lsdm::se3f_next_start(S.T);
+      __syncthreads();
+      track_state_begin(S, job, tid, T0b, beginNext ? link.nextTag : link.curTag);
+      began = true;
+      __syncthreads();
+    }
+  }
+  if (LINK && onNext) out = link.nextOut;
   PHASE_MARK(1);
 #ifdef LSD_DEVTOOLS
   const int lvlIn_ = S.level, numLaunchesIn_ = S.numLaunches, pendingIn_ = S.pending, ncandIn_ = S.ncand;
@@ -618,8 +652,11 @@
     return;
   }
   const int lvlPending = S.level;
-  const int doneWord = (MODE == TS_FUSED && spec.seq != 0) ? (BATCH ? spec.seq : (spec.seq >> 12)) : 1;
+  int doneWord = (MODE == TS_FUSED && spec.seq != 0) ? (BATCH ? spec.seq : (spec.seq >> 12)) : 1;
+  if (LINK) doneWord = onNext ? link.nextTag : link.curTag;
   step_role<BATCH, MODE>(role, job, spec, S);
+  if (LINK && role.leaves && !onNext && link.nextTag != 0 && S.pending && lvlPending == job.lastLevel && (int)blockIdx.x < nextq->lv[nextq->topLevel].nblocks)
+    role.leaves = false;
   if (role.leaves) return;
   int cand = role.cand, bx = role.bx;
 
@@ -660,9 +697,19 @@
     if (S.done) {
       if (!BATCH && MODE == TS_FUSED && S.lastCand > 0 && spec.copyMask != 0 && job.lv[level].writeMask && cand == 0 && bx < nb)
         copy_side_mask<BLOCK>(job, S, spec, level, bx, nb, tid);
-      if (leader) copy_words<sizeof(TrackState) / 4>(next, &S, tid, BLOCK);
-      LAUNCH_LOG(2, pendingIn_, ncandIn_, S.lastCand);
-      return;
+      if (LINK && !onNext && link.nextTag != 0 && !S.diverged) {
+        lsdm::SE3fH T0b = curq->T0;
+        if (tid == 0) T0b = lsdm::se3f_next_start(S.T);
+        __syncthreads();
+        jq = nextq; onNext = true; began = true;
+        out = link.nextOut;
+        track_state_begin(S, job, tid, T0b, link.nextTag);
+        __syncthreads();
+      } else {
+        if (leader) copy_words<sizeof(TrackState) / 4>(next, &S, tid, BLOCK);
+        LAUNCH_LOG(2, pendingIn_, ncandIn_, S.lastCand);
+        return;
+      }
     }
     if (cand > 0 && bx == 0 && S.phase == 1 && cand < S.ncand && tid < TRIAL_RECORD_WORDS) ((float*)&A.recs_out[cand])[tid] = trial_record_word(S, tid);
   }
@@ -678,13 +725,13 @@
   const int level = S.level;
   const TrackLevel& L = job.lv[level];
   const int nb = L.nblocks;
-  if (MODE == TS_FUSED && level != lvlPending) { cand = 0; bx = (int)blockIdx.x; }
+  if (MODE == TS_FUSED && (level != lvlPending || (LINK && began))) { cand = 0; bx = (int)blockIdx.x; }
   if (bx >= nb || cand >= S.ncand) return;
   const int tile = xcd_tile(bx, nb);
   EvalCtx a;
   make_ctx_dev(job, S, level, a);
   if (BATCH && MODE == TS_EVAL && cand > 0) ctx_set_pose(a, A.recs_in[cand]);
-  gbyte* wasGood = (gbyte*)(L.writeMask ? (cand == 0 ? job.wasGood : spec.wasGoodSide + (size_t)(cand - 1) * spec.maskStride) : nullptr);
+  gbyte* wasGood = (gbyte*)(L.writeMask ? (cand == 0 ? job.wasGood : ((LINK && onNext) ? link.nextSide : spec.wasGoodSide) + (size_t)(cand - 1) * spec.maskStride) : nullptr);
   const int work = a.npts >= 0 ? a.npts : a.w * a.h;
   float acc[RS_END];
 #pragma unroll
@@ -703,10 +750,11 @@
   reduce_and_store<BLOCK, BATCH, MODE>(a, L, S, tile, acc, key0, key1, key2, s_red, s_sum, s_wtop, s_top, A.sums_out + (size_t)cand * RS_COLS * A.max_rows,
                                        A.topkey_out + (size_t)cand * A.max_rows, A.topval_out + (size_t)cand * A.max_rows * (TAIL_ROWS * TAIL_STRIDE), tid);
   if (MODE == TS_FUSED && leader) copy_words<sizeof(TrackState) / 4>(next, &S, tid, BLOCK);
-  if (MODE == TS_FUSED && leader && tid == 0 && spec.last != 0) out->exhausted = spec.seq;
+  if (MODE == TS_FUSED && leader && tid == 0 && spec.last != 0 && !(LINK && onNext)) out->exhausted = spec.seq;
   LAUNCH_LOG(3, pendingIn_, ncandIn_, S.lastCand);
   PHASE_MARK(6);
   TRACE_PUT(tr_, 0, 9, wall_clock64());
+#undef job
 }
 
 template <int BLOCK, bool BATCH, int MODE = TS_FUSED>
@@ -721,11 +769,17 @@
     }
   }
 #endif
-  track_step_impl<BLOCK, BATCH, MODE>(jobv, jobs, st2, sc, out, parity, first, spec);
+  track_step_impl<BLOCK, BATCH, MODE>(jobv, jobs, st2, sc, out, parity, first, spec, jobv, TrackLink{});
 #ifdef LSD_ORDER_CHECK
   __syncthreads();
   if (!BATCH && spec.dbgCounters && threadIdx.x == 0) __hip_atomic_fetch_add(&spec.dbgCounters[0], 1ull, __ATOMIC_RELEASE, __HIP_MEMORY_SCOPE_AGENT);
 #endif
+}
+
+template <int BLOCK>
+__global__ __launch_bounds__(BLOCK) void k_track_step_linked(TrackJob jobv, TrackJob nextv, TrackLink link, TrackState* __restrict__ st2, TrackScratch sc,
+                                                              TrackSummary* __restrict__ out, int parity, int first, TrackSpec spec) {
+  track_step_impl<BLOCK, false, TS_FUSED, true>(jobv, nullptr, st2, sc, out, parity, first, spec, nextv, link);
 }
 
 #define LSD_SOLO_TRIPS 9
@@ -1041,6 +1095,8 @@
   if (const char* e = getenv("LSDHIP_TRACK_BLOCK")) t->block = atoi(e);
   if (const char* e = getenv("LSDHIP_TRACK_CAP")) t->grid_cap = atoi(e);
   if (const char* e = getenv("LSDHIP_EVAL_BATCH")) t->evalBatch = atoi(e) != 0;
+  if (const char* e = getenv("LSDHIP_LINK_JOBS")) t->linkJobs = atoi(e) != 0;
+  if (const char* e = getenv("LSDHIP_LINK_TAIL")) { t->linkTail = atoi(e); if (t->linkTail < 1) t->linkTail = 1; }
   if (t->block != 256) { lsd_set_error("LSDHIP_TRACK_BLOCK must be 256"); delete t; return LSDHIP_E_ARG; }
   t->grid_cap = lsd_grid_cap(t->grid_cap, t->block, RS_END);
   t->max_blocks = t->grid_cap;
@@ -1152,6 +1208,7 @@
   (void)hipFree(t->d_log);
 #endif
   (void)hipHostFree(t->h_summary);
+  if (t->h_linkSummary) (void)hipHostFree(t->h_linkSummary);
   if (t->d_pts) (void)hipFree(t->d_pts);
   delete t;
 }
@@ -1507,9 +1564,11 @@
   eo->num_constraints = (double)num_constraints;
 }
 
+static int abandon_linked(lsdhip_tracker* t);
 static int evaluate_pose(lsdhip_tracker* t, TrackJob& job, const lsdm::SE3fH& T, int level, EvalOut* eo) {
   lsdhip_ctx* c = t->ctx;
   LSD_CTX_LOCK(c);
+  if (int rca = abandon_linked(t)) return rca;
   job.evalOnly = 1;
   job.lastLevel = level;
   job.topLevel = level;
@@ -1702,6 +1761,7 @@
 
 static int track_device(lsdhip_tracker* t, TrackJob& job, int topLevel, const lsdm::SE3fH& T0, lsdm::SE3fH* Tout) {
   lsdhip_ctx* c = t->ctx;
+  if (int rca = abandon_linked(t)) return rca;
   job.evalOnly = 0;
   job.topLevel = topLevel;
   job.T0 = T0;
@@ -1862,6 +1922,204 @@
   return LSDHIP_OK;
 }
 
+static TrackSummary* link_record(const lsdhip_tracker* t, int i) { return t->h_linkSummary + i; }
+static int link_reserve(lsdhip_tracker* t) {
+  if (t->h_linkSummary) return LSDHIP_OK;
+  HIPCHK(hipHostMalloc((void**)&t->h_linkSummary, 2 * sizeof(TrackSummary), hipHostMallocMapped));
+  HIPCHK(hipHostGetDevicePointer((void**)&t->d_linkSummary, t->h_linkSummary, 0));
+  memset(t->h_linkSummary, 0, 2 * sizeof(TrackSummary));
+  return LSDHIP_OK;
+}
+static long long trackframe_need(const lsdhip_frame* kf, const lsdhip_frame* frame) {
+  long long need = frame->readySeq > kf->readySeq ? frame->readySeq : kf->readySeq;
+  return kf->depthSeq > need ? kf->depthSeq : need;
+}
+static bool same_job_but_T0(const TrackJob& a, TrackJob b) {
+  b.T0 = a.T0;
+  return memcmp(&a, &b, sizeof(TrackJob)) == 0;
+}
+static bool same_pose_bits(const lsdm::SE3fH& a, const lsdm::SE3fH& b) { return memcmp(&a, &b, sizeof(a)) == 0; }
+static int abandon_linked(lsdhip_tracker* t) {
+  if (!t->linked.valid) return LSDHIP_OK;
+  lsdhip_ctx* c = t->ctx;
+  HIPCHK(hipStreamSynchronize(c->stream));
+  lsdhip_frame* f = t->linked.frame;
+  HIPCHK(hipMemsetAsync(f->d_wasGood, 0xFF, (size_t)c->wl[1] * c->hl[1], c->stream));
+  HIPCHK(hipStreamSynchronize(c->stream));
+  f->wasGoodValid = false;
+  f->wasGoodPristine = true;
+  t->linked.valid = false;
+  t->linkAbandoned++;
+  return LSDHIP_OK;
+}
+extern "C" int lsdhip_tracker_abandon_linked(lsdhip_tracker* t) {
+  if (!t) return LSDHIP_E_ARG;
+  LSD_CTX_LOCK(t->ctx);
+  HIPCHK(hipSetDevice(t->ctx->device));
+  return abandon_linked(t);
+}
+extern "C" int lsdhip_tracker_set_link_hook(lsdhip_tracker* t, lsdhip_link_hook fn, void* user) {
+  if (!t) return LSDHIP_E_ARG;
+  LSD_CTX_LOCK(t->ctx);
+  t->linkHook = fn;
+  t->linkHookUser = user;
+  return LSDHIP_OK;
+}
+extern "C" int lsdhip_tracker_set_link_jobs(lsdhip_tracker* t, int on) {
+  if (!t) return LSDHIP_E_ARG;
+  LSD_CTX_LOCK(t->ctx);
+  t->linkJobs = on != 0;
+  return LSDHIP_OK;
+}
+extern "C" int lsdhip_tracker_set_link_from(lsdhip_tracker* t, int launchIndex) {
+  if (!t || launchIndex < 0) return LSDHIP_E_ARG;
+  LSD_CTX_LOCK(t->ctx);
+  t->linkFrom = launchIndex;
+  return LSDHIP_OK;
+}
+extern "C" int lsdhip_tracker_link_stats(const lsdhip_tracker* t, long long out[4]) {
+  if (!t || !out) return LSDHIP_E_ARG;
+  out[0] = t->linkBegunEarly; out[1] = t->linkDescribed; out[2] = t->linkAlone; out[3] = t->linkAbandoned;
+  return LSDHIP_OK;
+}
+static bool link_mode(const lsdhip_tracker* t) { return t->linkJobs && t->linkHook && t->ctx->pipeline && t->spinWait && !t->hostLM; }
+static void launch_linked(lsdhip_tracker* t, const TrackJob& job, const TrackJob& next, const TrackLink& link, TrackSpec spec, int grid, TrackSummary* d_out, int first, int last) {
+  lsdhip_ctx* c = t->ctx;
+  TrackScratch sc = scratch_of(t);
+  t->launchOrdinal++;
+  spec.seq = (link.curTag << 12) | (t->launchOrdinal & 0xFFF);
+  spec.last = last;
+  hipLaunchKernelGGL((k_track_step_linked<256>), dim3(grid), dim3(256), 0, c->stream, job, next, link, t->d_state, sc, d_out, t->linkParity, first, spec);
+  t->linkParity ^= 1;
+}
+struct LinkedResult { TrackSummary* rec; int maskSet; };
+static int track_device_linked(lsdhip_tracker* t, TrackJob& job, lsdhip_frame* kf, lsdhip_frame* frame, const lsdm::SE3fH& T0, lsdm::SE3fH* Tout, LinkedResult* res) {
+  lsdhip_ctx* c = t->ctx;
+  if (int rc = link_reserve(t)) return rc;
+  job.evalOnly = 0;
+  job.topLevel = LSD_TRACK_MAX_LEVEL - 1;
+  job.T0 = T0;
+  job.aff_a0 = 1.0f; job.aff_b0 = 0.0f;
+  const SinglePlan plan = plan_job(t, job);
+  lsdhip_tracker::LinkedJob& N = t->linked;
+  bool cont = N.valid && N.kf == kf && N.frame == frame && N.kfVersion == kf->depthVersion && same_job_but_T0(job, N.job) &&
+              same_pose_bits(T0, lsdm::se3f_next_start(N.prevPose));
+  if (N.valid && !cont) { if (int rc = abandon_linked(t)) return rc; }
+  int tag, record, first, ahead;
+  if (cont) {
+    tag = N.tag; record = N.record; first = 0; ahead = N.ahead;
+    N.valid = false;
+    if (ahead > 0) t->linkBegunEarly++;
+  } else {
+    if (int rc = claim_side_planes(t)) return rc;
+    t->jobTag = (t->jobTag % 0x7FFFF) + 1;
+    tag = t->jobTag;
+    t->linkRecord ^= 1;
+    record = t->linkRecord;
+    link_record(t, record)->done = 0;
+    link_record(t, record)->exhausted = 0;
+    first = 1; ahead = 0;
+    t->linkAlone++;
+  }
+  const TrackSpec spec = job_spec(t, plan);
+  res->maskSet = t->maskSet;
+  TrackSummary* S = link_record(t, record);
+  res->rec = S;
+  TrackSummary* d_out = t->d_linkSummary + record;
+  volatile const int* done = &S->done;
+  volatile const int* exhausted = &S->exhausted;
+  const long long myEpoch = ++c->enqEpoch;
+  const bool sample = c->prof_on && ((c->prof_tick++ & 7) == 0);
+  dev_job_begins(t);
+  t->launchOrdinal = 0;
+  if (int rc = prof_collect(c)) return rc;
+  lsdhip_host_mark(2);
+  int budget = t->recent.budget(12, t->budgetExtra, t->budgetFixed);
+  if (budget < ahead + 1) budget = ahead + 1;
+  int from = t->linkFrom > 0 ? t->linkFrom : budget - (t->linkTail - 1);
+  if (from < 1) from = 1;
+  int queued = ahead, firstCarry = 0;
+  TrackLink link = {tag, 0, nullptr, nullptr};
+  TrackJob nextJob = job;
+  auto enqueue = [&](int upto, bool closes) {
+    const DevTime tl0 = dev_now();
+    const int before = queued;
+    while (queued < upto) {
+      queued++;
+      if (link.nextTag != 0 && firstCarry == 0) firstCarry = queued;
+      launch_linked(t, job, nextJob, link, spec, plan.grid, d_out, first, closes && queued == upto);
+      lsdhip_host_mark(20);
+      first = 0;
+    }
+    dev_launches_queued(t, queued - before, tl0);
+  };
+  if (sample) HIPCHK(hipEventRecord(c->ev_a, c->stream));
+  const int pre = from - 1 < budget ? from - 1 : budget;
+  enqueue(pre, pre == budget);
+  if (t->enqueueHook) t->enqueueHook(t->enqueueHookUser);
+  if (lsdhip_frame* nf = t->linkHook(t->linkHookUser)) {
+    if (!kf->hasIDepth) { lsd_set_error("linked job: keyframe %d has no depth", kf->id); return LSDHIP_E_STATE; }
+    const long long need = trackframe_need(kf, nf);
+    if (!lsd_m_done(c, need)) { if (int rcw = lsd_t_wait_m(c, need)) return rcw; }
+    if (int rcf = fill_trackframe_job(t, nextJob, BatchShape{}, kf, nf)) return rcf;
+    nextJob.evalOnly = 0;
+    nextJob.topLevel = LSD_TRACK_MAX_LEVEL - 1;
+    nextJob.aff_a0 = 1.0f; nextJob.aff_b0 = 0.0f;
+    (void)plan_job(t, nextJob);
+    if (int rc = claim_side_planes(t)) return rc;
+    t->jobTag = (t->jobTag % 0x7FFFF) + 1;
+    t->linkRecord ^= 1;
+    N.valid = true; N.job = nextJob; N.tag = t->jobTag; N.maskSet = t->maskSet; N.record = t->linkRecord;
+    N.kf = kf; N.frame = nf; N.kfVersion = kf->depthVersion; N.need = need; N.ahead = 0;
+    link_record(t, N.record)->done = 0;
+    link_record(t, N.record)->exhausted = 0;
+    link.nextTag = N.tag;
+    link.nextOut = t->d_linkSummary + N.record;
+    link.nextSide = side_planes(t);
+    t->linkDescribed++;
+  }
+  HIPCHK(hipGetLastError());
+  enqueue(budget, true);
+  if (sample) { HIPCHK(hipEventRecord(c->ev_b, c->stream)); c->prof_pending = true; }
+  HIPCHK(hipGetLastError());
+  lsdhip_host_mark(3);
+  for (int guard = 0; ; guard++) {
+    if (guard > 200) { lsd_set_error("tracking job (linked) did not terminate"); return LSDHIP_E_STATE; }
+    lsdhip_host_mark(4);
+    {
+      DevWaitClock waitClock_(t);
+      LsdCtxUnlocked unlocked_(c);
+      const int lastSeq = (tag << 12) | (t->launchOrdinal & 0xFFF);
+      if (int rc = lsd_spin_until(c, [=]() { return *done == tag || *exhausted == lastSeq; }, lsd_deadline(LSD_JOB_WAIT_S), LSD_WAIT_JOB)) return rc;
+    }
+    lsdhip_host_mark(5);
+    if (*done == tag) break;
+    dev_budget_missed(t);
+    HIPCHK(hipStreamSynchronize(c->stream));
+    if (*done == tag) break;
+    if (int rc = prof_collect(c)) return rc;
+    enqueue(queued + (t->budgetFixed > 0 ? t->budgetFixed : 6), true);
+    HIPCHK(hipGetLastError());
+  }
+  if (int rcs = summary_wait_consistent(t, tag, S)) return rcs;
+  if (sample) {
+    c->prof_bytes += S->bytes;
+    c->prof_launches += S->numLaunches;
+  }
+  if (myEpoch > c->doneEpoch) c->doneEpoch = myEpoch;
+  t->numLaunches = S->numLaunches;
+  t->recent.note(t->numLaunches);
+  for (int l = 0; l < LSD_LEVELS; l++) t->levelEvaluations[l] = S->levelEvals[l];
+  take_summary(t, S);
+  *Tout = pose_of(S);
+  if (N.valid) {
+    N.prevPose = *Tout;
+    const int fin = S->numLaunches + 1, begin = fin > firstCarry ? fin : firstCarry;
+    N.ahead = (S->diverged || firstCarry == 0 || queued < begin) ? 0 : queued - begin + 1;
+  }
+  return S->diverged ? LSDHIP_DIVERGED : LSDHIP_OK;
+}
+
 extern "C" int lsdhip_tracker_track(lsdhip_tracker* t, lsdhip_frame* kf, lsdhip_frame* frame, const double init[7],
                                     lsdhip_track_result* out) {
   if (!t || !kf || !frame || !init || !out) return LSDHIP_E_ARG;
@@ -1898,22 +2156,29 @@
     const TrackSummary S = host_lm_summary(t, referenceToFrame, last_residual);
     return finish_trackframe(t, &S, kf, frame, out);
   }
-  t->jobKf = kf;
-  t->jobKfVersion = kf->depthVersion;
   const lsdm::SE3fH T0 = referenceToFrame;
   dev_trace_launched(t, 26, frame);
-  rc = track_device(t, job, LSD_TRACK_MAX_LEVEL - 1, T0, &referenceToFrame);
-  if (rc == LSDHIP_OK || rc == LSDHIP_DIVERGED) rc = dev_replay_check(t, job, kf, frame, T0, &referenceToFrame, rc);
-  t->jobKf = nullptr;
+  LinkedResult res = {t->h_summary, 0};
+  if (link_mode(t)) {
+    rc = track_device_linked(t, job, kf, frame, T0, &referenceToFrame, &res);
+  } else {
+    if (int rca = abandon_linked(t)) return rca;
+    t->jobKf = kf;
+    t->jobKfVersion = kf->depthVersion;
+    rc = track_device(t, job, LSD_TRACK_MAX_LEVEL - 1, T0, &referenceToFrame);
+    if (rc == LSDHIP_OK || rc == LSDHIP_DIVERGED) rc = dev_replay_check(t, job, kf, frame, T0, &referenceToFrame, rc);
+    t->jobKf = nullptr;
+    res.maskSet = t->maskSet;
+  }
   if (rc != LSDHIP_OK && rc != LSDHIP_DIVERGED) return rc;
   lsdhip_host_mark(6);
   dev_trace_result(t, 20, frame);
-  if (c->pipeline && rc == LSDHIP_OK && t->h_summary->lastCand > 0 && t->h_summary->level == LSD_TRACK_MIN_LEVEL) {
-    const uint8_t* side = side_planes(t) + (size_t)(t->h_summary->lastCand - 1) * t->maskStride;
-    t->maskMergeSeq[t->maskSet] = -1;
-    c->pendingMerges.push_back({frame->d_wasGood, side, &t->maskMergeSeq[t->maskSet]});
-  }
-  rc = finish_trackframe(t, t->h_summary, kf, frame, out);
+  if (c->pipeline && rc == LSDHIP_OK && res.rec->lastCand > 0 && res.rec->level == LSD_TRACK_MIN_LEVEL) {
+    const uint8_t* side = t->d_maskSide + (size_t)res.maskSet * t->maskStride * (LSD_SPEC_MAX - 1) + (size_t)(res.rec->lastCand - 1) * t->maskStride;
+    t->maskMergeSeq[res.maskSet] = -1;
+    c->pendingMerges.push_back({frame->d_wasGood, side, &t->maskMergeSeq[res.maskSet]});
+  }
+  rc = finish_trackframe(t, res.rec, kf, frame, out);
   lsdhip_host_mark(7);
   return rc;
 }
diff --git a/lsd_slam_amd/driver.py b/lsd_slam_amd/driver.py
--- a/lsd_slam_amd/driver.py
+++ b/lsd_slam_amd/driver.py
@@ -18,7 +18,7 @@
 
 EXPORTED_SYMBOLS = ["lsdloop_create", "lsdloop_destroy", "lsdloop_run", "lsdloop_get_stats", "lsdloop_reset_stats",
                     "lsdloop_copy_keyframe_planes", "lsdloop_set_keyframe_ring", "lsdloop_keyframes_exported", "lsdloop_ctx",
-                    "lsdloop_last_error", "lsdloop_keep_keyframes", "lsdloop_keyframe_log", "lsdloop_set_live_queue", "lsdloop_set_pipeline", "lsdloop_enable_reactivation", "lsdloop_keyframe_changes", "lsdloop_reactivation_counts", "lsdloop_download_map", "lsdloop_set_speculation", "lsdloop_observe_time", "lsdloop_comm_unique_id", "lsdloop_comm_init", "lsdloop_comm_destroy",
+                    "lsdloop_last_error", "lsdloop_keep_keyframes", "lsdloop_keyframe_log", "lsdloop_set_live_queue", "lsdloop_set_pipeline", "lsdloop_enable_reactivation", "lsdloop_keyframe_changes", "lsdloop_reactivation_counts", "lsdloop_download_map", "lsdloop_set_speculation", "lsdloop_set_link_jobs", "lsdloop_link_stats", "lsdloop_keep_frame_log", "lsdloop_frame_log", "lsdloop_observe_time", "lsdloop_comm_unique_id", "lsdloop_comm_init", "lsdloop_comm_destroy",
                     "lsdloop_gather_keyframes", "lsdband_create", "lsdband_destroy", "lsdband_window_rows", "lsdband_layout", "lsdband_load",
                     "lsdband_get", "lsdband_comm_init", "lsdband_run", "lsdband_synchronize", "lsdband_halo_bytes_per_pass", "lsdband_set_packed_exchange", "lsdband_set_overlap", "lsdband_tile_runs", "lsdband_plan", "lsdband_ipc_init", "lsdband_ipc_connect", "lsdband_ipc_failed", "lsdloop_gather_counts", "lsdloop_ipc_init", "lsdloop_ipc_connect", "lsdloop_ipc_result", "lsdloop_observe_work",
                     "lsdloopbatch_create", "lsdloopbatch_destroy", "lsdloopbatch_run", "lsdloopbatch_get_stats", "lsdloopbatch_ctx", "lsdloopbatch_set_keyframe_phases", "lsdloopbatch_set_pipeline", "lsdloopbatch_set_coarse_min_jobs", "lsdloopbatch_dropped",
@@ -68,6 +68,14 @@
         L.lsdloop_set_pipeline.argtypes = [vp, i]
         L.lsdloop_set_speculation.restype = i
         L.lsdloop_set_speculation.argtypes = [vp, i, i]
+        L.lsdloop_set_link_jobs.restype = i
+        L.lsdloop_set_link_jobs.argtypes = [vp, i, i]
+        L.lsdloop_keep_frame_log.restype = i
+        L.lsdloop_keep_frame_log.argtypes = [vp, i]
+        L.lsdloop_frame_log.restype = i
+        L.lsdloop_frame_log.argtypes = [vp, i, vp]
+        L.lsdloop_link_stats.restype = i
+        L.lsdloop_link_stats.argtypes = [vp, vp]
         L.lsdloop_observe_time.restype = i
         L.lsdloop_observe_time.argtypes = [vp, vp, vp]
         L.lsdloop_observe_work.restype = i
@@ -312,6 +320,23 @@
     def set_speculation(self, trials, finest_level_workgroups=0):
         _check(self.L.lsdloop_set_speculation(self.h_, int(trials), int(finest_level_workgroups)))
 
+    def set_link_jobs(self, on=True, from_launch=0):
+        _check(self.L.lsdloop_set_link_jobs(self.h_, int(bool(on)), int(from_launch)))
+
+    def keep_frame_log(self, on=True):
+        _check(self.L.lsdloop_keep_frame_log(self.h_, int(bool(on))))
+
+    def frame_log(self):
+        n = self.L.lsdloop_frame_log(self.h_, 0, None)
+        buf = np.zeros((max(n, 1), 5), dtype=np.int32)
+        self.L.lsdloop_frame_log(self.h_, n, buf.ctypes.data)
+        return buf[:n].copy()
+
+    def link_stats(self):
+        out = (C.c_longlong * 4)()
+        _check(self.L.lsdloop_link_stats(self.h_, out))
+        return [int(x) for x in out]
+
     def set_pipeline(self, on=True):
         _check(self.L.lsdloop_set_pipeline(self.h_, int(bool(on))))
 
diff --git a/lsd_slam_amd/driver/slam_loop.cpp b/lsd_slam_amd/driver/slam_loop.cpp
--- a/lsd_slam_amd/driver/slam_loop.cpp
+++ b/lsd_slam_amd/driver/slam_loop.cpp
@@ -25,6 +25,8 @@
   NcclComm comm = nullptr;
   int comm_rank = 0, comm_world = 1;
   std::vector<int> last_counts;
+  std::vector<lsdloop_frame_record> frame_log;
+  bool keep_frame_log = false;
   int* counts_dev = nullptr;
   bool ipc = false;
   int ipc_root = 0;
@@ -308,6 +310,9 @@
       for (int k = 0; k < 5; k++) l->st.level_evaluations[k] += L.levelEvaluations[k] - lev0[k];
       if (L.newKeyframe) l->st.keyframes++;
       if (out7) est.to7(out7 + 7 * (size_t)i);
+      if (l->keep_frame_log)
+        l->frame_log.push_back(lsdloop_frame_record{L.tracker.numEvaluations, L.tracker.numWarpUpdates, L.tracker.numLaunches, L.tracker.lastResidual,
+                                                    L.tracker.pointUsage});
       done++;
       if (stop_at_keyframe && L.newKeyframe) break;
     }
@@ -434,6 +439,31 @@
   if (!l) return LSDHIP_E_ARG;
   try { l->loop->tracker.setSpeculation(trials, finest_level_workgroups); return LSDHIP_OK; }
   catch (const Error& e) { g_err = e.what(); return e.status; }
+}
+extern "C" int lsdloop_set_link_jobs(lsdloop* l, int on, int from_launch) {
+  if (!l || from_launch < 0) return LSDHIP_E_ARG;
+  try { l->loop->tracker.setLinkJobs(on != 0); l->loop->tracker.setLinkFrom(from_launch); return LSDHIP_OK; }
+  catch (const Error& e) { g_err = e.what(); return e.status; }
+}
+extern "C" int lsdloop_keep_frame_log(lsdloop* l, int on) {
+  if (!l) return LSDHIP_E_ARG;
+  l->keep_frame_log = on != 0;
+  l->frame_log.clear();
+  return LSDHIP_OK;
+}
+extern "C" int lsdloop_frame_log(lsdloop* l, int max, lsdloop_frame_record* out) {
+  if (!l || max < 0 || (max > 0 && !out)) return LSDHIP_E_ARG;
+  const int n = (int)l->frame_log.size() < max ? (int)l->frame_log.size() : max;
+  for (int i = 0; i < n; i++) out[i] = l->frame_log[(size_t)i];
+  return (int)l->frame_log.size();
+}
+extern "C" int lsdloop_link_stats(lsdloop* l, long long out4[4]) {
+  if (!l || !out4) return LSDHIP_E_ARG;
+  try {
+    const std::array<long long, 4> s = l->loop->tracker.linkStats();
+    for (int i = 0; i < 4; i++) out4[i] = s[(size_t)i];
+    return LSDHIP_OK;
+  } catch (const Error& e) { g_err = e.what(); return e.status; }
 }
 extern "C" int lsdloop_observe_time(lsdloop* l, double* ms_out, long long* calls_out) {
   if (!l) return LSDHIP_E_ARG;
```

Result: slower. 5558 (-2.2%).
